# vfmatzkin/ct-unet

Measured on AMD Instinct MI355X. Metric: voxels/sec fwd+bwd, 128^3 fp32 patch, higher is better.
Workload: dtype f32; 1 GPU; UNet() default (1 in, 2 out, i_size 8, 4 blocks), 128^3 patch, batch 1 per GPU, train step = fwd + Dice/CE loss + bwd + grad all-reduce + Adam(amsgrad); patch=128, per_gpu_batch=1, parallelism=dp1, launch=hipgraph

## Files before the change

### ct-unet_amd/csrc/upconv_fused.hip

```cpp
#include <type_traits>
#include "common.h"
#include "bn_tail.h"
#include "channel_sum.h"

namespace {

typedef float v2f __attribute__((ext_vector_type(2)));

struct UpP {
    const float* in;
    const float* in_scale;
    const float* in_shift;
    const float* wp;
    const float* beff;
    float* out;
    float* stats;
    int in_cs, rin_p, in_relu, out_cs, nout_p;
    int N, D, H, W;
    int tiles_d, tiles_h, tiles_w;
    ctu_bn_tail tail;
};

template <int PB, int NTP, bool PW = false>
__global__ __launch_bounds__(256, 2) void upconv_fused_fwd_kernel(UpP p, int ntiles, int tiles_per_block) {
    static_assert(PW ? (PB == 4 && NTP == 1) : ((PB * NTP == 8 || (PB == 4 && NTP == 1)) && (PB == 8 || PB == 4 || PB == 2)), "tile-parities per block");
    constexpr int NTW = PW ? 3 : 2, TAPS = 4 * NTW;
    constexpr int MT = 4, TD = 4, TH = 4, TW = 16;
    constexpr int HD = TD + 2, HH = TH + 2, HW = TW + 2, HV = HD * HH * HW;
    constexpr int NTHR = 256;
    constexpr int NTPT = NTP;
    constexpr int WFL = PB * TAPS * NTP * 128;
    constexpr int AITEMS = HV * 2, AITER = (AITEMS + NTHR - 1) / NTHR;
    constexpr int WITER = (WFL / 4 + NTHR - 1) / NTHR;
    constexpr int VS2 = 6;
    static_assert(WFL / 4 % NTHR == 0, "weight staging covers the stage exactly");

    __shared__ __attribute__((aligned(16))) v2f sA2[HV * VS2];
    __shared__ __attribute__((aligned(16))) v2f sW2[WFL / 2];
    typedef const volatile __attribute__((address_space(3))) v2f* lds_v2f_ptr;
    __shared__ float sRed[4 * NTP * 16 * 2];

    const int tid = threadIdx.x, lane = tid & 63, wave = tid >> 6;
    const int m = lane & 15, kq = lane >> 4;
    const int by = blockIdx.y;
    const int nchunk = p.rin_p >> 3;
    const int half = tid & 1;
    const bool has_xf = p.in_scale != nullptr;
    const int pd0 = PW ? 0 : ((by * PB) >> 2) & 1, ph0 = PW ? 0 : ((by * PB) >> 1) & 1;

    lds_v2f_ptr vA = (lds_v2f_ptr)sA2 + (((wave + pd0) * HH + ph0) * HW + m) * VS2 + kq;
    lds_v2f_ptr vW = (lds_v2f_ptr)sW2 + (kq * 16 + m);

    unsigned hoff[AITER];
    constexpr int FPW = 5, NFW = (AITER + FPW - 1) / FPW;
    unsigned fw[NFW];
#pragma unroll
    for (int q = 0; q < NFW; ++q) fw[q] = 0;
#pragma unroll
    for (int it = 0; it < AITER; ++it) {
        const int i = tid + it * NTHR;
        const int v = (i < AITEMS) ? (i >> 1) : 0;
        const int pw = v % HW, t2 = v / HW, ph = t2 % HH, pd = t2 / HH;
        hoff[it] = (unsigned)(((pd * p.H + ph) * p.W + pw) * p.in_cs + half * 4) * 4u;
        const unsigned face = (pd == 0 ? 1u : 0u) | (pd == HD - 1 ? 2u : 0u) | (ph == 0 ? 4u : 0u) | (ph == HH - 1 ? 8u : 0u) |
                              (pw == 0 ? 16u : 0u) | (pw == HW - 1 ? 32u : 0u);
        fw[it / FPW] |= face << (6 * (it % FPW));
    }
    const unsigned safe_off = (unsigned)(((p.H + 1) * p.W + 1) * p.in_cs + half * 4) * 4u;

    f32x4 acc[PB][MT][NTP];
    float s1[NTP][4], s2[NTP][4];
#pragma unroll
    for (int nt = 0; nt < NTP; ++nt) {
#pragma unroll
        for (int pi = 0; pi < PB; ++pi)
#pragma unroll
            for (int mt = 0; mt < MT; ++mt) acc[pi][mt][nt] = f32x4{0.f, 0.f, 0.f, 0.f};
#pragma unroll
        for (int r = 0; r < 4; ++r) { s1[nt][r] = 0.f; s2[nt][r] = 0.f; }
    }

    int tile = blockIdx.x * tiles_per_block;
    const int tile_end = min(ntiles, tile + tiles_per_block);
    int c = 0;
    float4 va[AITER];
    typedef typename std::conditional<PW, f32x4, float4>::type wv_t;
    wv_t vw[WITER];
    float4 sc = make_float4(1.f, 1.f, 1.f, 1.f), sh = make_float4(0.f, 0.f, 0.f, 0.f);
    unsigned vmask = 0;

    struct Box { int tx, ty, tz, n; };
    Box box;
    {
        int t = tile;
        box.tx = t % p.tiles_w; t /= p.tiles_w;
        box.ty = t % p.tiles_h; t /= p.tiles_h;
        box.tz = t % p.tiles_d; box.n = t / p.tiles_d;
    }
    auto box_next = [&](Box b) {
        if (++b.tx == p.tiles_w) { b.tx = 0; if (++b.ty == p.tiles_h) { b.ty = 0; if (++b.tz == p.tiles_d) { b.tz = 0; ++b.n; } } }
        return b;
    };
    bool a_interior = false;
    auto load_a = [&](Box b, int cc) {
        const int d0 = b.tz * TD, h0 = b.ty * TH, w0 = b.tx * TW;
        if (has_xf) {
            sc = *reinterpret_cast<const float4*>(p.in_scale + cc * 8 + half * 4);
            sh = *reinterpret_cast<const float4*>(p.in_shift + cc * 8 + half * 4);
        }
        const long long org = (((long long)b.n * p.D + d0) * p.H + h0) * p.W + w0 - ((long long)p.H * p.W + p.W + 1);
        const char* base = reinterpret_cast<const char*>(p.in + org * p.in_cs + cc * 8);
        a_interior = d0 >= 1 && h0 >= 1 && w0 >= 1 && d0 + TD < p.D && h0 + TH < p.H && w0 + TW < p.W;
        if (a_interior) {
#pragma unroll
            for (int it = 0; it < AITER; ++it) {
                if ((it + 1) * NTHR <= AITEMS || tid + it * NTHR < AITEMS)
                    va[it] = *reinterpret_cast<const float4*>(base + hoff[it]);
                else
                    va[it] = make_float4(0.f, 0.f, 0.f, 0.f);
            }
            return;
        }
        vmask = 0;
        if (d0 + TD <= p.D && h0 + TH <= p.H && w0 + TW <= p.W) {
            const unsigned bface = (d0 == 0 ? 1u : 0u) | (d0 + TD == p.D ? 2u : 0u) | (h0 == 0 ? 4u : 0u) |
                                   (h0 + TH == p.H ? 8u : 0u) | (w0 == 0 ? 16u : 0u) | (w0 + TW == p.W ? 32u : 0u);
#pragma unroll
            for (int it = 0; it < AITER; ++it) {
                const bool ok = (fw[it / FPW] & (bface << (6 * (it % FPW)))) == 0u;
                va[it] = *reinterpret_cast<const float4*>(base + (ok ? hoff[it] : safe_off));
                vmask |= ok ? (1u << it) : 0u;
            }
            return;
        }
#pragma unroll
        for (int it = 0; it < AITER; ++it) {
            const int i = tid + it * NTHR, v = i >> 1;
            const int pw = v % HW, t2 = v / HW, ph = t2 % HH, pd = t2 / HH;
            const int gd = d0 + pd - 1, gh = h0 + ph - 1, gw = w0 + pw - 1;
            const bool ok = i < AITEMS && (unsigned)gd < (unsigned)p.D && (unsigned)gh < (unsigned)p.H && (unsigned)gw < (unsigned)p.W;
            float4 val = make_float4(0.f, 0.f, 0.f, 0.f);
            if (ok) {
                val = *reinterpret_cast<const float4*>(base + hoff[it]);
                vmask |= 1u << it;
            }
            va[it] = val;
        }
    };
    auto load_w = [&](int cc) {
        const char* wsrc = reinterpret_cast<const char*>(PW ? p.wp + (size_t)cc * 4 * TAPS * 128
                                                            : p.wp + ((size_t)cc * 8 + (size_t)by * PB) * 8 * NTPT * 128);
#pragma unroll
        for (int it = 0; it < WITER; ++it) vw[it] = *reinterpret_cast<const wv_t*>(wsrc + (unsigned)(tid + it * NTHR) * 16u);
    };
    if (tile >= tile_end) return;
    load_a(box, 0);
    load_w(0);

    while (true) {
        CTU_SETPRIO(CTU_PRIO_STAGE);
        __syncthreads();
        {
            auto put = [&](int it, float4 val) {
                const int i = tid + it * NTHR;
                if ((it + 1) * NTHR <= AITEMS || i < AITEMS) *reinterpret_cast<float4*>(&sA2[(i >> 1) * VS2 + half * 2]) = val;
            };
            if (a_interior) {
#pragma unroll
                for (int it = 0; it < AITER; ++it) put(it, has_xf ? xform4(va[it], sc, sh, p.in_relu) : va[it]);
            } else {
#pragma unroll
                for (int it = 0; it < AITER; ++it) {
                    const float4 t = has_xf ? xform4(va[it], sc, sh, p.in_relu) : va[it];
                    const bool ok = (vmask >> it) & 1u;
                    put(it, make_float4(ok ? t.x : 0.f, ok ? t.y : 0.f, ok ? t.z : 0.f, ok ? t.w : 0.f));
                }
            }
#pragma unroll
            for (int it = 0; it < WITER; ++it) *reinterpret_cast<wv_t*>(&sW2[(tid + it * NTHR) * 2]) = vw[it];
        }
        __syncthreads();
        int ntile = tile, nc = c + 1;
        Box nbox = box;
        if (nc == nchunk) { nc = 0; ntile = tile + 1; nbox = box_next(box); }
        const bool has_next = ntile < tile_end;
        if (has_next) {
            load_a(nbox, nc);
            load_w(nc);
        }
        CTU_SETPRIO(0);
        {
            constexpr int NG = PB * 2 * NTW;
            v2f ar[2][5], br[2][2][NTP];
            auto load_group = [&](int g, v2f (&aa)[5], v2f (&bb)[2][NTP]) {
                const int pi = g / (2 * NTW), dz = (g / NTW) & 1, dx = g % NTW;
                const int pid = PW ? (pi >> 1) : ((PB == 8) ? (pi >> 2) : 0), pih = PW ? (pi & 1) : ((PB >= 4) ? ((pi >> 1) & 1) : 0),
                          piw = PW ? 0 : (pi & 1);
#pragma unroll
                for (int r = 0; r < 5; ++r) aa[r] = vA[(((pid + dz) * HH + r + pih) * HW + piw + dx) * VS2];
#pragma unroll
                for (int dy = 0; dy < 2; ++dy)
#pragma unroll
                    for (int nt = 0; nt < NTP; ++nt) bb[dy][nt] = vW[((pi * TAPS + (dz * 2 + dy) * NTW + dx) * NTP + nt) * 64];
            };
            load_group(0, ar[0], br[0]);
            constexpr bool PIN = CTU_PIN_FWD && PB * NTP <= 4;
            if constexpr (PIN) __builtin_amdgcn_sched_barrier(0);
#pragma unroll
            for (int g = 0; g < NG; ++g) {
                if (g + 1 < NG) load_group(g + 1, ar[(g + 1) & 1], br[(g + 1) & 1]);
                const int pi = g / (2 * NTW);
                v2f (&aa)[5] = ar[g & 1];
                v2f (&bb)[2][NTP] = br[g & 1];
#pragma unroll
                for (int dy = 0; dy < 2; ++dy) {
#pragma unroll
                    for (int nt = 0; nt < NTP; ++nt)
#pragma unroll
                        for (int mt = 0; mt < MT; ++mt)
                            acc[pi][mt][nt] = __builtin_amdgcn_mfma_f32_16x16x4f32(bb[dy][nt].x, aa[mt + dy].x, acc[pi][mt][nt], 0, 0, 0);
#pragma unroll
                    for (int nt = 0; nt < NTP; ++nt)
#pragma unroll
                        for (int mt = 0; mt < MT; ++mt)
                            acc[pi][mt][nt] = __builtin_amdgcn_mfma_f32_16x16x4f32(bb[dy][nt].y, aa[mt + dy].y, acc[pi][mt][nt], 0, 0, 0);
                }
                if constexpr (PIN) {
#pragma unroll
                    for (int q = 0; q < 4 * MT * NTP; ++q) {
                        __builtin_amdgcn_sched_group_barrier(0x008, 1, 0);
                        if (g + 1 < NG && q < 5 + 2 * NTP) __builtin_amdgcn_sched_group_barrier(0x100, 1, 0);
                    }
                }
            }
        }
        CTU_SETPRIO(CTU_PRIO_STAGE);
        if (c == nchunk - 1) {
            const int d0 = box.tz * TD, h0 = box.ty * TH, w0 = box.tx * TW;
            const int Df = 2 * p.D, Hf = 2 * p.H, Wf = 2 * p.W;
            const int cd = d0 + wave, cw = w0 + m;
            const bool touches = d0 == 0 || h0 == 0 || w0 == 0 || d0 + TD >= p.D || h0 + TH >= p.H || w0 + TW >= p.W;
#pragma unroll
            for (int nt = 0; nt < NTP; ++nt) {
                const int co = PW ? (kq & 1) * 4 : nt * 16 + kq * 4;
                const bool cok = co < p.nout_p;
                float4 b0 = make_float4(0.f, 0.f, 0.f, 0.f);
                if (cok) b0 = *reinterpret_cast<const float4*>(p.beff + co);
#pragma unroll
                for (int pi = 0; pi < PB; ++pi) {
                    const int pd = PW ? (pi >> 1) : pd0 + ((PB == 8) ? (pi >> 2) : 0), ph = PW ? (pi & 1) : ph0 + ((PB >= 4) ? ((pi >> 1) & 1) : 0),
                              pw = PW ? (kq >> 1) : (pi & 1);
                    const int fz = 2 * cd + pd, fx = 2 * cw + pw;
#pragma unroll
                    for (int mt = 0; mt < MT; ++mt) {
                        const int ch = h0 + mt, fy = 2 * ch + ph;
                        if (cok && cd < p.D && ch < p.H && cw < p.W) {
                            float4 bv = b0;
                            if (touches) {
                                const int cz = fz == 0 ? 1 : (fz == Df - 1 ? 2 : 0), cy = fy == 0 ? 1 : (fy == Hf - 1 ? 2 : 0),
                                          cx = fx == 0 ? 1 : (fx == Wf - 1 ? 2 : 0);
                                bv = *reinterpret_cast<const float4*>(p.beff + (size_t)((cz * 3 + cy) * 3 + cx) * p.nout_p + co);
                            }
                            float4 o;
                            o.x = acc[pi][mt][nt][0] + bv.x; o.y = acc[pi][mt][nt][1] + bv.y;
                            o.z = acc[pi][mt][nt][2] + bv.z; o.w = acc[pi][mt][nt][3] + bv.w;
                            const size_t fv = (((size_t)box.n * Df + fz) * Hf + fy) * Wf + fx;
                            *reinterpret_cast<float4*>(p.out + fv * p.out_cs + co) = o;
                            s1[nt][0] += o.x; s1[nt][1] += o.y; s1[nt][2] += o.z; s1[nt][3] += o.w;
                            s2[nt][0] += o.x * o.x; s2[nt][1] += o.y * o.y; s2[nt][2] += o.z * o.z; s2[nt][3] += o.w * o.w;
                        }
                        acc[pi][mt][nt] = f32x4{0.f, 0.f, 0.f, 0.f};
                    }
                }
            }
        }
        if (!has_next) break;
        tile = ntile; c = nc; box = nbox;
    }
    if (p.stats) {
        __syncthreads();
#pragma unroll
        for (int nt = 0; nt < NTP; ++nt)
#pragma unroll
            for (int r = 0; r < 4; ++r) {
                float a1 = s1[nt][r], a2 = s2[nt][r];
#pragma unroll
                for (int o = 1; o < 16; o <<= 1) { a1 += __shfl_xor(a1, o); a2 += __shfl_xor(a2, o); }
                if (PW) { a1 += __shfl_xor(a1, 32); a2 += __shfl_xor(a2, 32); }
                const int ch = PW ? (kq & 1) * 4 + r : nt * 16 + kq * 4 + r;
                if (m == 0 && (!PW || kq < 2)) {
                    sRed[(wave * NTP * 16 + ch) * 2 + 0] = a1;
                    sRed[(wave * NTP * 16 + ch) * 2 + 1] = a2;
                }
            }
        __syncthreads();
        float* row = p.stats + ((size_t)blockIdx.y * gridDim.x + blockIdx.x) * 2 * p.nout_p;
        for (int ch = tid; ch < p.nout_p; ch += NTHR) {
            float a1 = 0.f, a2 = 0.f;
#pragma unroll
            for (int w = 0; w < 4; ++w) {
                a1 += sRed[(w * NTP * 16 + ch) * 2 + 0];
                a2 += sRed[(w * NTP * 16 + ch) * 2 + 1];
            }
            st_row(p.tail.counter != nullptr, row + ch, a1);
            st_row(p.tail.counter != nullptr, row + p.nout_p + ch, a2);
        }
        if (p.tail.counter) bn_fwd_tail(p.tail, p.stats, gridDim.x * gridDim.y, p.nout_p, gridDim.x * gridDim.y);
    }
}

struct UpDP {
    const float* g;
    const float* wp;
    float* out;
    int g_cs, nout_p, out_cs, cin_p;
    int N, D, H, W;
    int tiles_d, tiles_h, tiles_w, n16;
};

template <int NT>
__global__ __launch_bounds__(256, 2) void upconv_fused_bwd_data_kernel(UpDP p, int ntiles, int tiles_per_block) {
    constexpr int MT = 4, TD = 4, TH = 4, TW = 16;
    constexpr int HD = TD + 2, HH = TH + 2, HW = TW + 2, HV = HD * HH * HW;
    constexpr int NTHR = 256;
    constexpr int WFL = 8 * NT * 128;
    constexpr int AITEMS = HV * 2, AITER = (AITEMS + NTHR - 1) / NTHR;
    constexpr int WITER = (WFL / 4 + NTHR - 1) / NTHR;
    constexpr int VS2 = 6;
    static_assert(WFL / 4 % NTHR == 0, "weight staging covers the stage exactly");

    __shared__ __attribute__((aligned(16))) v2f sA2[HV * VS2];
    __shared__ __attribute__((aligned(16))) v2f sW2[WFL / 2];
    typedef const volatile __attribute__((address_space(3))) v2f* lds_v2f_ptr;

    const int tid = threadIdx.x, lane = tid & 63, wave = tid >> 6;
    const int m = lane & 15, kq = lane >> 4;
    const int by = blockIdx.y;
    const int qc = p.nout_p >> 3;
    const int nchunk = 8 * qc;
    const int half = tid & 1;
    const int Hf = 2 * p.H, Wf = 2 * p.W;

    lds_v2f_ptr vA0 = (lds_v2f_ptr)sA2 + ((wave * HH) * HW + m) * VS2 + kq;
    lds_v2f_ptr vW = (lds_v2f_ptr)sW2 + (kq * 16 + m);

    unsigned hoff[AITER];
    constexpr int FPW = 5, NFW = (AITER + FPW - 1) / FPW;
    unsigned fw[NFW];
#pragma unroll
    for (int q = 0; q < NFW; ++q) fw[q] = 0;
#pragma unroll
    for (int it = 0; it < AITER; ++it) {
        const int i = tid + it * NTHR;
        const int v = (i < AITEMS) ? (i >> 1) : 0;
        const int pw = v % HW, t2 = v / HW, ph = t2 % HH, pd = t2 / HH;
        hoff[it] = (unsigned)(((2 * pd * Hf + 2 * ph) * Wf + 2 * pw) * p.g_cs + half * 4) * 4u;
        const unsigned face = (pd == 0 ? 1u : 0u) | (pd == HD - 1 ? 2u : 0u) | (ph == 0 ? 4u : 0u) | (ph == HH - 1 ? 8u : 0u) |
                              (pw == 0 ? 16u : 0u) | (pw == HW - 1 ? 32u : 0u);
        fw[it / FPW] |= face << (6 * (it % FPW));
    }
    const unsigned safe_off = (unsigned)(((2 * Hf + 2) * Wf + 2) * p.g_cs + half * 4) * 4u;

    f32x4 acc[MT][NT];
#pragma unroll
    for (int nt = 0; nt < NT; ++nt)
#pragma unroll
        for (int mt = 0; mt < MT; ++mt) acc[mt][nt] = f32x4{0.f, 0.f, 0.f, 0.f};

    int tile = blockIdx.x * tiles_per_block;
    const int tile_end = min(ntiles, tile + tiles_per_block);
    if (tile >= tile_end) return;
    int c = 0;
    float4 va[AITER], vw[WITER];
    unsigned vmask = 0;

    struct Box { int tx, ty, tz, n; };
    Box box;
    {
        int t = tile;
        box.tx = t % p.tiles_w; t /= p.tiles_w;
        box.ty = t % p.tiles_h; t /= p.tiles_h;
        box.tz = t % p.tiles_d; box.n = t / p.tiles_d;
    }
    auto box_next = [&](Box b) {
        if (++b.tx == p.tiles_w) { b.tx = 0; if (++b.ty == p.tiles_h) { b.ty = 0; if (++b.tz == p.tiles_d) { b.tz = 0; ++b.n; } } }
        return b;
    };
    bool a_interior = false;
    auto load_a = [&](Box b, int cc) {
        const int d0 = b.tz * TD, h0 = b.ty * TH, w0 = b.tx * TW;
        const int par = cc / qc, q = cc % qc;
        const int pz = (par >> 2) & 1, py = (par >> 1) & 1, px = par & 1;
        const long long org = (((long long)b.n * 2 * p.D + 2 * (d0 - 1) + pz) * Hf + 2 * (h0 - 1) + py) * Wf + 2 * (w0 - 1) + px;
        const char* base = reinterpret_cast<const char*>(p.g + org * p.g_cs + q * 8);
        a_interior = d0 >= 1 && h0 >= 1 && w0 >= 1 && d0 + TD < p.D && h0 + TH < p.H && w0 + TW < p.W;
        if (a_interior) {
#pragma unroll
            for (int it = 0; it < AITER; ++it) {
                if ((it + 1) * NTHR <= AITEMS || tid + it * NTHR < AITEMS)
                    va[it] = *reinterpret_cast<const float4*>(base + hoff[it]);
                else
                    va[it] = make_float4(0.f, 0.f, 0.f, 0.f);
            }
            return;
        }
        vmask = 0;
        if (d0 + TD <= p.D && h0 + TH <= p.H && w0 + TW <= p.W) {
            const unsigned bface = (d0 == 0 ? 1u : 0u) | (d0 + TD == p.D ? 2u : 0u) | (h0 == 0 ? 4u : 0u) |
                                   (h0 + TH == p.H ? 8u : 0u) | (w0 == 0 ? 16u : 0u) | (w0 + TW == p.W ? 32u : 0u);
#pragma unroll
            for (int it = 0; it < AITER; ++it) {
                const bool ok = (fw[it / FPW] & (bface << (6 * (it % FPW)))) == 0u;
                va[it] = *reinterpret_cast<const float4*>(base + (ok ? hoff[it] : safe_off));
                vmask |= ok ? (1u << it) : 0u;
            }
            return;
        }
#pragma unroll
        for (int it = 0; it < AITER; ++it) {
            const int i = tid + it * NTHR, v = i >> 1;
            const int pw = v % HW, t2 = v / HW, ph = t2 % HH, pd = t2 / HH;
            const int gd = d0 + pd - 1, gh = h0 + ph - 1, gw = w0 + pw - 1;
            const bool ok = i < AITEMS && (unsigned)gd < (unsigned)p.D && (unsigned)gh < (unsigned)p.H && (unsigned)gw < (unsigned)p.W;
            float4 val = make_float4(0.f, 0.f, 0.f, 0.f);
            if (ok) {
                val = *reinterpret_cast<const float4*>(base + hoff[it]);
                vmask |= 1u << it;
            }
            va[it] = val;
        }
    };
    const bool w_full = (by + 1) * NT <= p.n16;
    auto load_w = [&](int cc) {
        const float* wsrc = p.wp + ((size_t)cc * 8 * p.n16 + (size_t)by * NT) * 128;
#pragma unroll
        for (int it = 0; it < WITER; ++it) {
            const int i = (tid + it * NTHR) * 4;
            const int ts = i / (NT * 128), r = i % (NT * 128);
            float4 v = make_float4(0.f, 0.f, 0.f, 0.f);
            if (w_full || by * NT * 128 + r < p.n16 * 128)
                v = *reinterpret_cast<const float4*>(reinterpret_cast<const char*>(wsrc) + (unsigned)(ts * p.n16 * 128 + r) * 4u);
            vw[it] = v;
        }
    };
    load_a(box, 0);
    load_w(0);

    while (true) {
        CTU_SETPRIO(CTU_PRIO_STAGE);
        __syncthreads();
        {
            auto put = [&](int it, float4 val) {
                const int i = tid + it * NTHR;
                if ((it + 1) * NTHR <= AITEMS || i < AITEMS) *reinterpret_cast<float4*>(&sA2[(i >> 1) * VS2 + half * 2]) = val;
            };
            if (a_interior) {
#pragma unroll
                for (int it = 0; it < AITER; ++it) put(it, va[it]);
            } else {
#pragma unroll
                for (int it = 0; it < AITER; ++it) {
                    const bool ok = (vmask >> it) & 1u;
                    put(it, make_float4(ok ? va[it].x : 0.f, ok ? va[it].y : 0.f, ok ? va[it].z : 0.f, ok ? va[it].w : 0.f));
                }
            }
#pragma unroll
            for (int it = 0; it < WITER; ++it) *reinterpret_cast<float4*>(&sW2[(tid + it * NTHR) * 2]) = vw[it];
        }
        __syncthreads();
        const int par = c / qc;
        lds_v2f_ptr vA = vA0 + (((1 - ((par >> 2) & 1)) * HH + (1 - ((par >> 1) & 1))) * HW + (1 - (par & 1))) * VS2;
        int ntile = tile, nc = c + 1;
        Box nbox = box;
        if (nc == nchunk) { nc = 0; ntile = tile + 1; nbox = box_next(box); }
        const bool has_next = ntile < tile_end;
        if (has_next) {
            load_a(nbox, nc);
            load_w(nc);
        }
        CTU_SETPRIO(0);
        {
            v2f ar[2][5], br[2][2][NT];
            auto load_group = [&](int g, v2f (&aa)[5], v2f (&bb)[2][NT]) {
                const int ez = (g >> 1) & 1, ex = g & 1;
#pragma unroll
                for (int r = 0; r < 5; ++r) aa[r] = vA[((ez * HH + r) * HW + ex) * VS2];
#pragma unroll
                for (int ey = 0; ey < 2; ++ey)
#pragma unroll
                    for (int nt = 0; nt < NT; ++nt) bb[ey][nt] = vW[(((ez * 2 + ey) * 2 + ex) * NT + nt) * 64];
            };
            load_group(0, ar[0], br[0]);
#if CTU_PIN_FWD
            __builtin_amdgcn_sched_barrier(0);
#endif
#pragma unroll
            for (int g = 0; g < 4; ++g) {
                if (g + 1 < 4) load_group(g + 1, ar[(g + 1) & 1], br[(g + 1) & 1]);
                v2f (&aa)[5] = ar[g & 1];
                v2f (&bb)[2][NT] = br[g & 1];
#pragma unroll
                for (int ey = 0; ey < 2; ++ey) {
#pragma unroll
                    for (int nt = 0; nt < NT; ++nt)
#pragma unroll
                        for (int mt = 0; mt < MT; ++mt)
                            acc[mt][nt] = __builtin_amdgcn_mfma_f32_16x16x4f32(bb[ey][nt].x, aa[mt + ey].x, acc[mt][nt], 0, 0, 0);
#pragma unroll
                    for (int nt = 0; nt < NT; ++nt)
#pragma unroll
                        for (int mt = 0; mt < MT; ++mt)
                            acc[mt][nt] = __builtin_amdgcn_mfma_f32_16x16x4f32(bb[ey][nt].y, aa[mt + ey].y, acc[mt][nt], 0, 0, 0);
                }
#if CTU_PIN_FWD
#pragma unroll
                for (int q = 0; q < 4 * MT * NT; ++q) {
                    __builtin_amdgcn_sched_group_barrier(0x008, 1, 0);
                    if (g + 1 < 4 && q < 5 + 2 * NT) __builtin_amdgcn_sched_group_barrier(0x100, 1, 0);
                }
#endif
            }
        }
        CTU_SETPRIO(CTU_PRIO_STAGE);
        if (c == nchunk - 1) {
            const int d0 = box.tz * TD, h0 = box.ty * TH, w0 = box.tx * TW;
            const int gw = w0 + m;
            float* obase = p.out + ((((size_t)box.n * p.D + d0 + wave) * p.H + h0) * p.W + gw) * p.out_cs;
            const int orow = p.W * p.out_cs;
#pragma unroll
            for (int nt = 0; nt < NT; ++nt) {
                const int co = (by * NT + nt) * 16 + kq * 4;
#pragma unroll
                for (int mt = 0; mt < MT; ++mt) {
                    if (co < p.cin_p && d0 + wave < p.D && h0 + mt < p.H && gw < p.W) {
                        float4 o;
                        o.x = acc[mt][nt][0]; o.y = acc[mt][nt][1]; o.z = acc[mt][nt][2]; o.w = acc[mt][nt][3];
                        *reinterpret_cast<float4*>(obase + mt * orow + co) = o;
                    }
                    acc[mt][nt] = f32x4{0.f, 0.f, 0.f, 0.f};
                }
            }
        }
        if (!has_next) break;
        tile = ntile; c = nc; box = nbox;
    }
}

__device__ __forceinline__ float upconv_pack_bwd_value(const float* __restrict__ wp, int idx, int cin_p, int nout_p) {
    const int n16 = (cin_p + 15) >> 4, qc = nout_p >> 3, ntpt = (nout_p + 15) >> 4;
    int r = idx;
    const int j = r & 1; r >>= 1;
    const int n = r & 15; r >>= 4;
    const int kq = r & 3; r >>= 2;
    const int nt = r % n16; r /= n16;
    const int e = r & 7; r >>= 3;
    const int q = r % qc;
    const int par = r / qc;
    const int pos = nt * 16 + n, co = q * 8 + kq * 2 + j;
    float v = 0.f;
    if (pos < cin_p) {
        const int cf = pos >> 3, kqf = (pos & 7) >> 1, jf = pos & 1;
        v = wp[((((size_t)cf * 8 + par) * 8 + (e ^ 7)) * ntpt + (co >> 4)) * 128 + kqf * 32 + (co & 15) * 2 + jf];
    }
    return v;
}

__device__ __forceinline__ int axis_pairs(int pbit, int jbit, int (&t)[2], int (&a)[2]) {
    if (pbit == 0) {
        if (jbit == 0) { t[0] = 0; a[0] = 1; return 1; }
        t[0] = 1; a[0] = 0; t[1] = 2; a[1] = 1; return 2;
    }
    if (jbit == 0) { t[0] = 0; a[0] = 0; t[1] = 1; a[1] = 1; return 2; }
    t[0] = 2; a[0] = 0; return 1;
}

__global__ void upconv_transpose_kernel(const float* __restrict__ wt, const float* __restrict__ w3, float* __restrict__ wtt,
                                        float* __restrict__ w3t, int C, int Co, int nout_p) {
    const int idx = blockIdx.x * blockDim.x + threadIdx.x;
    const int n3 = 27 * C * nout_p, nt = 8 * C * C;
    if (idx < n3) {
        const int co = idx % nout_p, cm = (idx / nout_p) % C, t = idx / (nout_p * C);
        w3t[idx] = co < Co ? w3[((size_t)co * C + cm) * 27 + t] : 0.f;
    } else if (idx < n3 + nt) {
        const int k = idx - n3;
        const int cm = k % C, ci = (k / C) % C, a = k / (C * C);
        wtt[k] = wt[((size_t)ci * C + cm) * 8 + a];
    }
}

constexpr int WS_WAVES = 8, WS_BLOCK = WS_WAVES * 64;
__device__ __forceinline__ void upconv_pack_block(const float* __restrict__ wtt, const float* __restrict__ w3t, float* __restrict__ wp,
                                                  int C, int nout_p, const int32_t* __restrict__ cinv, int nchunk, int ntpt,
                                                  int bid, float4 (*part)[64]) {
    const int pr = threadIdx.x >> 6, lane = threadIdx.x & 63, sub = lane & 7;
    const int idx = bid * 8 + (lane >> 3);
    const int ncol4 = ntpt * 4;
    const bool valid = idx < nchunk * 8 * 8 * 8 * ncol4;
    int r = valid ? idx : 0;
    const int co = (r % ncol4) * 4; r /= ncol4;
    const int r8 = r & 7; r >>= 3;
    const int tap = r & 7; r >>= 3;
    const int par = r & 7; r >>= 3;
    const int c = r;
    const int rp = c * 8 + r8;
    const int ci = cinv ? cinv[rp] : (rp < C ? rp : -1);
    int np = 0;
    float4 s = make_float4(0.f, 0.f, 0.f, 0.f);
    if (valid && ci >= 0 && co < nout_p) {
        int tz[2], az[2], ty[2], ay[2], tx[2], ax[2];
        const int nz = axis_pairs((par >> 2) & 1, (tap >> 2) & 1, tz, az);
        const int ny = axis_pairs((par >> 1) & 1, (tap >> 1) & 1, ty, ay);
        const int nx = axis_pairs(par & 1, tap & 1, tx, ax);
        np = nz * ny * nx;
        const int ix = pr % nx, iy = (pr / nx) % ny, iz = pr / (nx * ny);
        if (iz < nz) {
            const float* a = wtt + ((size_t)((az[iz] * 2 + ay[iy]) * 2 + ax[ix]) * C + ci) * C;
            const float* b = w3t + (size_t)((tz[iz] * 3 + ty[iy]) * 3 + tx[ix]) * C * nout_p + co;
#pragma unroll 4
            for (int cm = sub; cm < C; cm += 8) {
                const float av = a[cm];
                const float4 bv = *reinterpret_cast<const float4*>(b + (size_t)cm * nout_p);
                s.x = fmaf(av, bv.x, s.x); s.y = fmaf(av, bv.y, s.y); s.z = fmaf(av, bv.z, s.z); s.w = fmaf(av, bv.w, s.w);
            }
        }
    }
    part[pr][lane] = s;
    __syncthreads();
    if (pr != 0) return;
    float4 v = make_float4(0.f, 0.f, 0.f, 0.f);
    for (int p = 0; p < np; ++p) {
        const float4 t = part[p][lane];
        v.x += t.x; v.y += t.y; v.z += t.z; v.w += t.w;
    }
    float vv[4] = {v.x, v.y, v.z, v.w};
#pragma unroll
    for (int q = 0; q < 4; ++q) { vv[q] += __shfl_xor(vv[q], 1); vv[q] += __shfl_xor(vv[q], 2); vv[q] += __shfl_xor(vv[q], 4); }
    if (valid && sub == 0) {
        const int nt = co >> 4, n = co & 15, kq = r8 >> 1, j = r8 & 1;
        float* dst = wp + ((((size_t)c * 8 + par) * 8 + tap) * ntpt + nt) * 128 + kq * 32 + n * 2 + j;
#pragma unroll
        for (int q = 0; q < 4; ++q) dst[q * 2] = vv[q];
    }
}

__device__ __forceinline__ float upconv_pack_pw_value(const float* __restrict__ wp, int idx) {
    int r = idx;
    const int j = r & 1; r >>= 1;
    const int n = r & 15; r >>= 4;
    const int kq = r & 3; r >>= 2;
    const int tap = r % 12; r /= 12;
    const int par4 = r & 3;
    const int c = r >> 2;
    const int px = n >> 3, co = n & 7, dxx = tap % 3, dzy = tap / 3, jx = dxx - px;
    float v = 0.f;
    if (jx == 0 || jx == 1) v = wp[((size_t)(c * 8 + par4 * 2 + px) * 8 + dzy * 2 + jx) * 128 + kq * 32 + co * 2 + j];
    return v;
}

__global__ void upconv_pack_gather_kernel(const float* __restrict__ wp, float* __restrict__ wpw, int npw, float* __restrict__ wpd,
                                          int nwpd, int cin_p, int nout_p) {
    const int idx = blockIdx.x * blockDim.x + threadIdx.x;
    if (idx < npw) wpw[idx] = upconv_pack_pw_value(wp, idx);
    else if (idx - npw < nwpd) wpd[idx - npw] = upconv_pack_bwd_value(wp, idx - npw, cin_p, nout_p);
}

constexpr int BEFF_CO = 8;
__device__ __forceinline__ void upconv_beff_block(const float* __restrict__ bt, const float* __restrict__ w3t, float* __restrict__ beff,
                                                  int C, int nout_p, int co0, float* S) {
    for (int i = threadIdx.x; i < 27 * BEFF_CO; i += blockDim.x) {
        const int co = co0 + i % BEFF_CO, t = i / BEFF_CO;
        const float* b = w3t + (size_t)t * C * nout_p + co;
        float s = 0.f;
#pragma unroll 16
        for (int cm = 0; cm < C; ++cm) s = fmaf(bt[cm], b[(size_t)cm * nout_p], s);
        S[i] = s;
    }
    __syncthreads();
    for (int i = threadIdx.x; i < 27 * BEFF_CO; i += blockDim.x) {
        const int col = i % BEFF_CO, cls = i / BEFF_CO;
        const int cz = cls / 9, cy = (cls / 3) % 3, cx = cls % 3;
        float v = 0.f;
        for (int t = 0; t < 27; ++t) {
            const int tz = t / 9, ty = (t / 3) % 3, tx = t % 3;
            if ((cz == 1 && tz == 0) || (cz == 2 && tz == 2) || (cy == 1 && ty == 0) || (cy == 2 && ty == 2) ||
                (cx == 1 && tx == 0) || (cx == 2 && tx == 2))
                continue;
            v += S[t * BEFF_CO + col];
        }
        beff[cls * nout_p + co0 + col] = v;
    }
}

__global__ __launch_bounds__(WS_BLOCK) void upconv_pack_beff_kernel(const float* __restrict__ wtt, const float* __restrict__ w3t,
                                                                    float* __restrict__ wp, int C, int nout_p,
                                                                    const int32_t* __restrict__ cinv, int nchunk, int ntpt,
                                                                    const float* __restrict__ bt, float* __restrict__ beff) {
    __shared__ float4 part[WS_WAVES][64];
    static_assert(27 * BEFF_CO <= WS_WAVES * 64 * 4, "b_eff's S fits the pack's LDS");
    const int nbeff = nout_p / BEFF_CO;
    if ((int)blockIdx.x < nbeff) {
        upconv_beff_block(bt, w3t, beff, C, nout_p, (int)blockIdx.x * BEFF_CO, reinterpret_cast<float*>(part));
        return;
    }
    upconv_pack_block(wtt, w3t, wp, C, nout_p, cinv, nchunk, ntpt, (int)blockIdx.x - nbeff, part);
}

constexpr int FS_SPLIT = 16;

template <class T>
__device__ __forceinline__ void upconv_face_sums_block(const T* __restrict__ dy, int cs, int cp, int N, int Df, int Hf, int Wf,
                                                       float* __restrict__ tpart, int sel, int split, float4* red) {
    const int sz = sel / 9, sy = (sel / 3) % 3, sx = sel % 3;
    const int nz = sz ? 1 : Df, ny = sy ? 1 : Hf, nx = sx ? 1 : Wf;
    const int z0 = sz == 2 ? Df - 1 : 0, y0 = sy == 2 ? Hf - 1 : 0, x0 = sx == 2 ? Wf - 1 : 0;
    const int nq = cp >> 2;
    const int qd = threadIdx.x % nq;
    const int64_t nvox = (int64_t)N * nz * ny * nx;
    float4 acc = make_float4(0.f, 0.f, 0.f, 0.f);
    for (int64_t v = (int64_t)split * (256 / nq) + threadIdx.x / nq; v < nvox; v += (int64_t)FS_SPLIT * (256 / nq)) {
        int64_t r = v;
        const int x = x0 + (int)(r % nx); r /= nx;
        const int y = y0 + (int)(r % ny); r /= ny;
        const int z = z0 + (int)(r % nz);
        const int n = (int)(r / nz);
        const float4 g = ld4<T>(dy + ((((size_t)n * Df + z) * Hf + y) * Wf + x) * cs + qd * 4);
        acc.x += g.x; acc.y += g.y; acc.z += g.z; acc.w += g.w;
    }
    red[threadIdx.x] = acc;
    __syncthreads();
    for (int o = 128; o >= nq; o >>= 1) {
        if (threadIdx.x < o) {
            float4 b = red[threadIdx.x + o];
            float4& a = red[threadIdx.x];
            a.x += b.x; a.y += b.y; a.z += b.z; a.w += b.w;
        }
        __syncthreads();
    }
    if (threadIdx.x < nq)
        *reinterpret_cast<float4*>(tpart + ((size_t)sel * FS_SPLIT + split) * cp + threadIdx.x * 4) = red[threadIdx.x];
}

template <class T>
__global__ __launch_bounds__(256) void upconv_sums_kernel(const T* __restrict__ dy, int cs, int cp, int N, int Df, int Hf, int Wf,
                                                          int64_t fvox, float* __restrict__ csp, int nb, float* __restrict__ tpart) {
    static_assert(CSUM_BLOCK == 256, "one block size for both ranges");
    __shared__ float4 red[256];
    if ((int)blockIdx.x < nb) {
        channel_sum_partial_block<T>(dy, cs, cp, fvox, csp, blockIdx.x, nb, reinterpret_cast<float*>(red));
        return;
    }
    const int b = (int)blockIdx.x - nb;
    upconv_face_sums_block<T>(dy, cs, cp, N, Df, Hf, Wf, tpart, b / FS_SPLIT + 1, b % FS_SPLIT, red);
}

__global__ __launch_bounds__(256) void upconv_tall_v_kernel(const float* __restrict__ csp, int nb, const float* __restrict__ tpart,
                                                            int cp, float* __restrict__ tall, float* __restrict__ V) {
    __shared__ double r[CSUM_BLOCK];
    const int co = blockIdx.x;
    const float ta = channel_sum_final_block(csp, nb, cp, co, r);
    if (threadIdx.x == 0) tall[co] = ta;
    if (threadIdx.x >= 27) return;
    const int t = threadIdx.x, idx = t * cp + co;
    const int tz = t / 9, ty = (t / 3) % 3, tx = t % 3;
    float v = 0.f;
    for (int iz = 0; iz < (tz == 1 ? 1 : 2); ++iz)
        for (int iy = 0; iy < (ty == 1 ? 1 : 2); ++iy)
            for (int ix = 0; ix < (tx == 1 ? 1 : 2); ++ix) {
                const int sz = iz == 0 ? 0 : (tz == 0 ? 1 : 2), sy = iy == 0 ? 0 : (ty == 0 ? 1 : 2), sx = ix == 0 ? 0 : (tx == 0 ? 1 : 2);
                const float sign = ((iz + iy + ix) & 1) ? -1.f : 1.f;
                const int sel = (sz * 3 + sy) * 3 + sx;
                float s = 0.f;
                if (sel == 0) {
                    s = ta;
                } else {
                    const float* src = tpart + (size_t)sel * FS_SPLIT * cp + co;
                    for (int b = 0; b < FS_SPLIT; ++b) s += src[(size_t)b * cp];
                }
                v += sign * s;
            }
    V[idx] = v;
}

__device__ __forceinline__ void axis_pd(int t, int a, int& pbit, int& jbit) {
    if (a == 1) { pbit = (t == 1) ? 1 : 0; jbit = (t == 2) ? 1 : 0; }
    else { pbit = (t == 1) ? 0 : 1; jbit = (t == 0) ? 0 : 1; }
}
__device__ __forceinline__ int weff_index(int t, int a) {
    int pz, jz, py, jy, px, jx;
    axis_pd(t / 9, (a >> 2) & 1, pz, jz);
    axis_pd((t / 3) % 3, (a >> 1) & 1, py, jy);
    axis_pd(t % 3, a & 1, px, jx);
    return ((pz * 4 + py * 2 + px) * 8) + (jz * 4 + jy * 2 + jx);
}

__global__ __launch_bounds__(WS_BLOCK) void upconv_project_kernel(const float* __restrict__ dweff, const float* __restrict__ V,
                                                                  const float* __restrict__ wtt, const float* __restrict__ w3t,
                                                                  const float* __restrict__ bt, const int32_t* __restrict__ imap,
                                                                  int C, int Co, int cin_p, int nout_p, int nb1,
                                                                  float* __restrict__ dwt, float* __restrict__ dw3,
                                                                  float* __restrict__ dbt) {
    const int coq = (Co + 3) >> 2;
    const int n1 = C * C * 8, n2 = coq * C * 27, n3 = C;
    if ((int)blockIdx.x >= nb1) {
        __shared__ float4 part[WS_WAVES][64];
        const int a = threadIdx.x >> 6, lane = threadIdx.x & 63, sub = lane & 7;
        const int k = ((int)blockIdx.x - nb1) * 8 + (lane >> 3);
        const bool valid = k < n2;
        const int kk = valid ? k : 0;
        const int co = (kk % coq) * 4, cm = (kk / coq) % C, t = kk / (coq * C);
        float4 s = make_float4(0.f, 0.f, 0.f, 0.f);
        if (valid) {
            const float* g = dweff + (size_t)weff_index(t, a) * cin_p * nout_p + co;
            const float* w = wtt + (size_t)a * C * C + cm;
#pragma unroll 4
            for (int ci = sub; ci < C; ci += 8) {
                const float4 gv = *reinterpret_cast<const float4*>(g + (size_t)(imap ? imap[ci] : ci) * nout_p);
                const float wv = w[(size_t)ci * C];
                s.x = fmaf(gv.x, wv, s.x); s.y = fmaf(gv.y, wv, s.y); s.z = fmaf(gv.z, wv, s.z); s.w = fmaf(gv.w, wv, s.w);
            }
        }
        part[a][lane] = s;
        __syncthreads();
        if (a != 0) return;
        float4 acc = make_float4(0.f, 0.f, 0.f, 0.f);
#pragma unroll
        for (int aa = 0; aa < 8; ++aa) {
            const float4 p = part[aa][lane];
            acc.x += p.x; acc.y += p.y; acc.z += p.z; acc.w += p.w;
        }
        float av[4] = {acc.x, acc.y, acc.z, acc.w};
#pragma unroll
        for (int q = 0; q < 4; ++q) {
            if (sub == 0 && co + q < Co) av[q] = fmaf(V[t * nout_p + co + q], bt[cm], av[q]);
            av[q] += __shfl_xor(av[q], 1); av[q] += __shfl_xor(av[q], 2); av[q] += __shfl_xor(av[q], 4);
            if (valid && sub == 0 && co + q < Co) dw3[((size_t)(co + q) * C + cm) * 27 + t] = av[q];
        }
        return;
    }
    const int gidx = blockIdx.x * blockDim.x + threadIdx.x;
    const int sub = gidx & 7;
    const int idx = gidx >> 3;
    if (idx >= n1 + n3) return;
    float v = 0.f;
    float* dst;
    if (idx < n1) {
        const int a = idx & 7, cm = (idx >> 3) % C, ci = idx / (8 * C);
        const int pos = imap ? imap[ci] : ci;
#pragma unroll
        for (int k = 0; k < 4; ++k) {
            const int t = sub + 8 * k;
            if (t < 27) {
                const float4* g = reinterpret_cast<const float4*>(dweff + ((size_t)weff_index(t, a) * cin_p + pos) * nout_p);
                const float4* w = reinterpret_cast<const float4*>(w3t + ((size_t)t * C + cm) * nout_p);
                float s = 0.f;
                for (int c4 = 0; c4 * 4 < Co; ++c4) {
                    const float4 gv = g[c4], wv = w[c4];
                    const int co = c4 * 4;
                    s = fmaf(gv.x, wv.x, s);
                    if (co + 1 < Co) s = fmaf(gv.y, wv.y, s);
                    if (co + 2 < Co) s = fmaf(gv.z, wv.z, s);
                    if (co + 3 < Co) s = fmaf(gv.w, wv.w, s);
                }
                v += s;
            }
        }
        dst = dwt + idx;
    } else {
        const int cm = idx - n1;
        for (int t = sub; t < 27; t += 8) {
            const float* w = w3t + ((size_t)t * C + cm) * nout_p;
#pragma unroll 8
            for (int co = 0; co < Co; ++co) v = fmaf(V[t * nout_p + co], w[co], v);
        }
        dst = dbt + cm;
    }
    v += __shfl_xor(v, 1); v += __shfl_xor(v, 2); v += __shfl_xor(v, 4);
    if (sub == 0) *dst = v;
}

struct UpPlan { int tiles_d, tiles_h, tiles_w, ntiles, nt, ny; Grid grid; };
static UpPlan up_plan(int N, int D, int H, int W, int nout_p, int bwd_n16) {
    UpPlan r;
    r.tiles_d = ceil_div(D, 4); r.tiles_h = ceil_div(H, 4); r.tiles_w = ceil_div(W, 16);
    r.ntiles = N * r.tiles_d * r.tiles_h * r.tiles_w;
    if (bwd_n16) {
        r.nt = bwd_n16 >= 4 ? 4 : (bwd_n16 >= 2 ? 2 : 1);
        while (r.nt > 1 && (long)r.ntiles * ceil_div(bwd_n16, r.nt) < 256) r.nt >>= 1;
        r.ny = ceil_div(bwd_n16, r.nt);
    } else {
        r.nt = 0;
        r.ny = (nout_p == 16 && r.ntiles < 256) ? 2 : (nout_p <= 16 ? 1 : (nout_p <= 32 ? 2 : 4));
    }
    r.grid = persist_grid(r.ntiles, 512 / r.ny);
    return r;
}

}

extern "C" int ctu_upconv_fused_supported(int k, int D, int H, int W, int cin_p, int nout_p) {
    return k == 3 && W >= 16 && D >= 1 && H >= 1 && cin_p % 8 == 0 && cin_p >= 8 && nout_p % 8 == 0 && nout_p >= 8 && nout_p <= 64;
}

static size_t up_std_packed(int cin_p, int nout_p) { return (size_t)(cin_p / 8) * 8 * 8 * ceil_div(nout_p, 16) * 128; }

extern "C" size_t ctu_upconv_fused_packed_floats(int cin_p, int nout_p) {
    return up_std_packed(cin_p, nout_p) + (nout_p == 8 ? (size_t)(cin_p / 8) * 4 * 12 * 128 : 0);
}

extern "C" int ctu_upconv_fused_num_blocks(int N, int D, int H, int W, int nout_p) {
    const UpPlan r = up_plan(N, D, H, W, nout_p, 0);
    return r.grid.gx * r.ny;
}

extern "C" size_t ctu_upconv_fused_pack_ws_floats(int C, int nout_p) { return (size_t)27 * C * nout_p + (size_t)8 * C * C; }

static int upconv_pack_gather(const float* wp, int cin_p, int nout_p, float* wpw, float* wpd, hipStream_t st) {
    const int npw = wpw ? (cin_p / 8) * 4 * 12 * 128 : 0;
    const int nwpd = wpd ? (int)ctu_upconv_fused_bwd_packed_floats(cin_p, nout_p) : 0;
    if (npw + nwpd == 0) return CTU_OK;
    upconv_pack_gather_kernel<<<ceil_div(npw + nwpd, 256), 256, 0, st>>>(wp, wpw, npw, wpd, nwpd, cin_p, nout_p);
    CTU_CHECK_LAUNCH("upconv_fused_pack_gather");
    return CTU_OK;
}

extern "C" int ctu_upconv_fused_pack_all(const float* wt, const float* bt, const float* w3, int C, int Co, const int32_t* cinv,
                                         int cin_p, int nout_p, float* wp, float* beff, float* ws, float* wpd, void* stream) {
    CTU_REQUIRE(wt && bt && w3 && wp && beff && ws, "upconv_fused_pack: null pointer");
    CTU_REQUIRE(C > 0 && Co > 0 && Co <= nout_p && cin_p % 8 == 0 && nout_p % 8 == 0 && (cinv || C <= cin_p),
                "upconv_fused_pack: C=%d Co=%d cin_p=%d nout_p=%d", C, Co, cin_p, nout_p);
    hipStream_t st = (hipStream_t)stream;
    const int ntpt = ceil_div(nout_p, 16);
    CTU_REQUIRE(((uintptr_t)ws & 15) == 0, "upconv_fused_pack: ws must be 16-byte aligned");
    float* w3t = ws;
    float* wtt = ws + (size_t)27 * C * nout_p;
    const int ntr = 27 * C * nout_p + 8 * C * C;
    upconv_transpose_kernel<<<ceil_div(ntr, 256), 256, 0, st>>>(wt, w3, wtt, w3t, C, Co, nout_p);
    CTU_CHECK_LAUNCH("upconv_fused_transpose");
    const int quads = (cin_p / 8) * 8 * 8 * 8 * ntpt * 4;
    upconv_pack_beff_kernel<<<nout_p / BEFF_CO + ceil_div(quads, 8), WS_BLOCK, 0, st>>>(wtt, w3t, wp, C, nout_p, cinv, cin_p / 8,
                                                                                         ntpt, bt, beff);
    CTU_CHECK_LAUNCH("upconv_fused_pack");
    return upconv_pack_gather(wp, cin_p, nout_p, nout_p == 8 ? wp + up_std_packed(cin_p, nout_p) : nullptr, wpd, st);
}

extern "C" int ctu_upconv_fused_pack(const float* wt, const float* bt, const float* w3, int C, int Co, const int32_t* cinv,
                                     int cin_p, int nout_p, float* wp, float* beff, float* ws, void* stream) {
    return ctu_upconv_fused_pack_all(wt, bt, w3, C, Co, cinv, cin_p, nout_p, wp, beff, ws, nullptr, stream);
}

extern "C" int ctu_upconv_fused_fwd(const float* in, int in_cs, int cin_p, const float* in_scale, const float* in_shift,
                                    int in_relu, const float* wp, const float* beff, float* out, int out_cs, int nout_p,
                                    float* stats, int N, int D, int H, int W, const ctu_bn_tail* tail, void* stream) {
    CTU_REQUIRE(in && wp && beff && out, "upconv_fused_fwd: null pointer");
    CTU_REQUIRE(ctu_upconv_fused_supported(3, D, H, W, cin_p, nout_p), "upconv_fused_fwd: unsupported geometry (W=%d cin_p=%d nout_p=%d)",
                W, cin_p, nout_p);
    CTU_REQUIRE(in_cs >= cin_p && in_cs % 4 == 0 && out_cs >= nout_p && out_cs % 4 == 0, "upconv_fused_fwd: bad stride");
    CTU_REQUIRE((in_scale == nullptr) == (in_shift == nullptr), "upconv_fused_fwd: scale/shift must come together");
    CTU_REQUIRE(((uintptr_t)in & 15) == 0 && ((uintptr_t)out & 15) == 0 && ((uintptr_t)wp & 15) == 0 && ((uintptr_t)beff & 15) == 0,
                "upconv_fused_fwd: 16-byte alignment");
    CTU_REQUIRE((int64_t)N * D * H * W * 8 < (int64_t)1 << 31 && (int64_t)(2 * H * W + 2 * W + 2) * in_cs * 4 < (int64_t)1 << 31,
                "upconv_fused_fwd: volume too large for 32-bit offsets");
    UpP p;
    p.in = in; p.in_scale = in_scale; p.in_shift = in_shift; p.wp = wp; p.beff = beff; p.out = out; p.stats = stats;
    CTU_REQUIRE(!tail || (stats && tail->counter && tail->gamma && tail->beta && tail->scale && tail->shift && tail->mean &&
                          tail->invstd && tail->C > 0 && tail->C <= nout_p && tail->count > 0),
                "upconv_fused_fwd: incomplete BatchNorm tail");
    p.tail = tail_or_off(tail);
    p.in_cs = in_cs; p.rin_p = cin_p; p.in_relu = in_relu; p.out_cs = out_cs; p.nout_p = nout_p;
    p.N = N; p.D = D; p.H = H; p.W = W;
    const UpPlan r = up_plan(N, D, H, W, nout_p, 0);
    p.tiles_d = r.tiles_d; p.tiles_h = r.tiles_h; p.tiles_w = r.tiles_w;
    const int ny = r.ny, gx = r.grid.gx, tpb = r.grid.tpb, ntiles = r.ntiles;
    hipStream_t st = (hipStream_t)stream;
    if (nout_p == 16 && ny == 2) {
        upconv_fused_fwd_kernel<4, 1><<<dim3(gx, 2), 256, 0, st>>>(p, ntiles, tpb);
    } else if (nout_p == 8) {
        p.wp = wp + up_std_packed(cin_p, nout_p);
        upconv_fused_fwd_kernel<4, 1, true><<<dim3(gx, 1), 256, 0, st>>>(p, ntiles, tpb);
    } else if (ny == 1) upconv_fused_fwd_kernel<8, 1><<<dim3(gx, 1), 256, 0, st>>>(p, ntiles, tpb);
    else if (ny == 2) upconv_fused_fwd_kernel<4, 2><<<dim3(gx, 2), 256, 0, st>>>(p, ntiles, tpb);
    else upconv_fused_fwd_kernel<2, 4><<<dim3(gx, 4), 256, 0, st>>>(p, ntiles, tpb);
    CTU_CHECK_LAUNCH("upconv_fused_fwd");
    return CTU_OK;
}

extern "C" int ctu_channel_sum_num_blocks(int64_t nvox);

extern "C" size_t ctu_upconv_fused_project_ws_floats(int nout_p, int64_t fine_nvox) {
    return (size_t)27 * FS_SPLIT * nout_p + (size_t)27 * nout_p + nout_p + (size_t)ctu_channel_sum_num_blocks(fine_nvox) * nout_p;
}

static int upconv_project_impl(int dtype, const float* dweff, const void* gout, int g_cs, int nout_p, int N, int D, int H, int W,
                               const float* bt, const float* pack_ws, const int32_t* imap, int C, int Co, int cin_p,
                               float* dwt, float* dbt, float* dw3, float* ws, void* stream) {
    CTU_REQUIRE(dweff && gout && bt && pack_ws && dwt && dbt && dw3 && ws, "upconv_fused_project: null pointer");
    CTU_REQUIRE(nout_p == 8 || nout_p == 16 || nout_p == 32 || nout_p == 64, "upconv_fused_project: nout_p=%d", nout_p);
    CTU_REQUIRE(C > 0 && Co > 0 && Co <= nout_p && g_cs >= nout_p && g_cs % 4 == 0, "upconv_fused_project: bad channels");
    CTU_REQUIRE(((uintptr_t)dweff & 15) == 0 && ((uintptr_t)pack_ws & 15) == 0, "upconv_fused_project: dweff / pack_ws must be 16-byte aligned");
    hipStream_t st = (hipStream_t)stream;
    float* tpart = ws;
    float* V = ws + (size_t)27 * FS_SPLIT * nout_p;
    float* tall = V + (size_t)27 * nout_p;
    float* csp = tall + nout_p;
    const int64_t fvox = (int64_t)N * 8 * D * H * W;
    const int nb = ctu_channel_sum_num_blocks(fvox);
    const int nsum = nb + 26 * FS_SPLIT;
    if (dtype == 0) {
        upconv_sums_kernel<float><<<nsum, 256, 0, st>>>((const float*)gout, g_cs, nout_p, N, 2 * D, 2 * H, 2 * W, fvox, csp, nb, tpart);
    } else {
        CTU_DISPATCH_LP(dtype, upconv_sums_kernel<T><<<nsum, 256, 0, st>>>((const T*)gout, g_cs, nout_p, N, 2 * D, 2 * H, 2 * W, fvox, csp, nb, tpart));
    }
    CTU_CHECK_LAUNCH("upconv_sums");
    upconv_tall_v_kernel<<<nout_p, 256, 0, st>>>(csp, nb, tpart, nout_p, tall, V);
    CTU_CHECK_LAUNCH("upconv_tall_v");
    const float* w3t = pack_ws;
    const float* wtt = pack_ws + (size_t)27 * C * nout_p;
    const int nb1 = ceil_div((C * C * 8 + C) * 8, WS_BLOCK);
    const int nb2 = ceil_div(((Co + 3) / 4) * C * 27, 8);
    upconv_project_kernel<<<nb1 + nb2, WS_BLOCK, 0, st>>>(dweff, V, wtt, w3t, bt, imap, C, Co, cin_p, nout_p, nb1, dwt, dw3, dbt);
    CTU_CHECK_LAUNCH("upconv_project");
    return CTU_OK;
}

extern "C" int ctu_upconv_fused_project(const float* dweff, const float* gout, int g_cs, int nout_p, int N, int D, int H, int W,
                                        const float* bt, const float* pack_ws, const int32_t* imap, int C, int Co, int cin_p,
                                        float* dwt, float* dbt, float* dw3, float* ws, void* stream) {
    return upconv_project_impl(0, dweff, gout, g_cs, nout_p, N, D, H, W, bt, pack_ws, imap, C, Co, cin_p, dwt, dbt, dw3, ws, stream);
}
extern "C" int ctu_lp_upconv_fused_project(int dtype, const float* dweff, const void* gout, int g_cs, int nout_p, int N, int D, int H,
                                           int W, const float* bt, const float* pack_ws, const int32_t* imap, int C, int Co, int cin_p,
                                           float* dwt, float* dbt, float* dw3, float* ws, void* stream) {
    CTU_REQUIRE(dtype == CTU_BF16 || dtype == CTU_F16, "lp_upconv_fused_project: dtype %d", dtype);
    return upconv_project_impl(dtype, dweff, gout, g_cs, nout_p, N, D, H, W, bt, pack_ws, imap, C, Co, cin_p, dwt, dbt, dw3, ws, stream);
}

extern "C" size_t ctu_upconv_fused_bwd_packed_floats(int cin_p, int nout_p) {
    return (size_t)8 * (nout_p / 8) * 8 * ceil_div(cin_p, 16) * 128;
}

extern "C" int ctu_upconv_fused_pack_bwd(const float* wp, int cin_p, int nout_p, float* wpd, void* stream) {
    CTU_REQUIRE(wp && wpd && cin_p % 8 == 0 && nout_p % 8 == 0, "upconv_fused_pack_bwd: bad argument");
    return upconv_pack_gather(wp, cin_p, nout_p, nullptr, wpd, (hipStream_t)stream);
}

extern "C" int ctu_upconv_fused_bwd_data(const float* gout, int g_cs, int nout_p, const float* wpd, float* gin, int gin_cs,
                                         int cin_p, int N, int D, int H, int W, void* stream) {
    CTU_REQUIRE(gout && wpd && gin, "upconv_fused_bwd_data: null pointer");
    CTU_REQUIRE(ctu_upconv_fused_supported(3, D, H, W, cin_p, nout_p), "upconv_fused_bwd_data: unsupported geometry");
    CTU_REQUIRE(g_cs >= nout_p && g_cs % 4 == 0 && gin_cs >= cin_p && gin_cs % 4 == 0, "upconv_fused_bwd_data: bad stride");
    CTU_REQUIRE(((uintptr_t)gout & 15) == 0 && ((uintptr_t)gin & 15) == 0 && ((uintptr_t)wpd & 15) == 0, "upconv_fused_bwd_data: alignment");
    CTU_REQUIRE((int64_t)(12 * 2 * H + 12) * 2 * W * g_cs * 4 + 64 < (int64_t)1 << 31, "upconv_fused_bwd_data: volume too large for 32-bit offsets");
    UpDP p;
    p.g = gout; p.wp = wpd; p.out = gin; p.g_cs = g_cs; p.nout_p = nout_p; p.out_cs = gin_cs; p.cin_p = cin_p;
    p.N = N; p.D = D; p.H = H; p.W = W;
    p.n16 = ceil_div(cin_p, 16);
    const UpPlan r = up_plan(N, D, H, W, nout_p, p.n16);
    p.tiles_d = r.tiles_d; p.tiles_h = r.tiles_h; p.tiles_w = r.tiles_w;
    const int NT = r.nt, ny = r.ny, gx = r.grid.gx, tpb = r.grid.tpb, ntiles = r.ntiles;
    hipStream_t st = (hipStream_t)stream;
    if (NT == 4) upconv_fused_bwd_data_kernel<4><<<dim3(gx, ny), 256, 0, st>>>(p, ntiles, tpb);
    else if (NT == 2) upconv_fused_bwd_data_kernel<2><<<dim3(gx, ny), 256, 0, st>>>(p, ntiles, tpb);
    else upconv_fused_bwd_data_kernel<1><<<dim3(gx, ny), 256, 0, st>>>(p, ntiles, tpb);
    CTU_CHECK_LAUNCH("upconv_fused_bwd_data");
    return CTU_OK;
}
```

### ct-unet_amd/ctunet_amd/_lib.py

```python
from __future__ import annotations

import ctypes as C
import os

import torch

_HERE = os.path.dirname(os.path.abspath(__file__))
LIB_PATH = os.environ.get("CTUNET_HIP_LIB") or os.path.join(_HERE, "libctunet_hip.so")

P = C.c_void_p
I = C.c_int
L = C.c_int64
F = C.c_float
D = C.c_double
Z = C.c_size_t
U = C.c_uint64

class PackJob(C.Structure):
    _fields_ = [("w", C.c_void_p), ("wp", C.c_void_p), ("cinv", C.c_void_p), ("kind", C.c_int), ("Co", C.c_int),
                ("Ci", C.c_int), ("k", C.c_int), ("rin_p", C.c_int), ("nout_p", C.c_int), ("mode", C.c_int),
                ("layout", C.c_int)]


class BnTail(C.Structure):
    _fields_ = [("gamma", C.c_void_p), ("beta", C.c_void_p), ("running_mean", C.c_void_p), ("running_var", C.c_void_p),
                ("scale", C.c_void_p), ("shift", C.c_void_p), ("mean", C.c_void_p), ("invstd", C.c_void_p),
                ("num_batches_tracked", C.c_void_p), ("counter", C.c_void_p), ("count", C.c_double),
                ("momentum", C.c_float), ("eps", C.c_float), ("C", C.c_int), ("n_updates", C.c_int)]


class BnBwdTail(C.Structure):
    _fields_ = [("gamma", C.c_void_p), ("invstd", C.c_void_p), ("dgamma", C.c_void_p), ("dbeta", C.c_void_p),
                ("coef", C.c_void_p), ("mean", C.c_void_p), ("running_mean", C.c_void_p), ("running_var", C.c_void_p),
                ("num_batches_tracked", C.c_void_p), ("counter", C.c_void_p), ("count", C.c_double),
                ("momentum", C.c_float), ("eps", C.c_float), ("C", C.c_int)]


class WgradJob(C.Structure):
    _fields_ = [("ws", C.c_void_p), ("dw", C.c_void_p), ("db", C.c_void_p), ("cinv", C.c_void_p), ("kind", C.c_int),
                ("Co", C.c_int), ("Ci", C.c_int), ("cin_p", C.c_int), ("n_ci_g", C.c_int), ("gx", C.c_int),
                ("pairs", C.c_int), ("nmf", C.c_int)]


WGRAD_JOBS_MAX = 4

SIGNATURES = {
    "ctu_last_error": (C.c_char_p, []),
    "ctu_abi_version": (I, []),
    "ctu_arch": (C.c_char_p, []),
    "ctu_ncdhw_to_ndhwc": (I, [P, P, I, I, I, I, I, I, I, P]),
    "ctu_ndhwc_to_ncdhw": (I, [P, P, I, I, I, I, I, I, P]),
    "ctu_conv3d_layout": (I, [I, I, I]),
    "ctu_conv3d_fwd_kernel_name": (C.c_char_p, [I, I, I, I, I, I, I]),
    "ctu_conv3d_wgrad_kernel_name": (C.c_char_p, [I, I, I, I]),
    "ctu_conv3d_packed_floats": (Z, [I, I, I, I]),
    "ctu_conv3d_num_blocks": (I, [I, I, I, I, I, I, I]),
    "ctu_pack_conv3d_weight": (I, [P, P, I, I, I, P, I, I, I, I, P]),
    "ctu_pack_batch": (I, [P, I, P]),
    "ctu_conv3d_fwd": (I, [P, I, I, P, P, I, P, P, I, P, I, I, P, I, I, I, I, I, I, P, P]),
    "ctu_conv3d_wgrad_ws_floats": (Z, [I, I, I, I, I, I, I]),
    "ctu_conv3d_wgrad": (I, [P, I, I, P, P, I, P, I, I, P, P, I, I, P, P, I, I, I, I, I, P]),
    "ctu_conv3d_wgrad_bn_supported": (I, [I, I, I, I, I, I, I]),
    "ctu_conv3d_wgrad_bn": (I, [P, I, I, P, P, I, P, I, I, P, P, P, P, P, P, I, I, P, P, I, I, I, I, I, P]),
    "ctu_conv3d_first_supported": (I, [I, I, I, I]),
    "ctu_conv3d_first_num_blocks": (I, [I, I, I, I]),
    "ctu_conv3d_first_fwd": (I, [P, I, P, P, I, P, I, I, P, I, I, I, I, P, P]),
    "ctu_conv3d_first_bwd_data": (I, [P, I, P, I, I, P, I, I, I, I, P]),
    "ctu_conv3d_first_wgrad_ws_floats": (Z, [I, I, I, I, I]),
    "ctu_conv3d_first_wgrad": (I, [P, I, P, I, P, I, P, I, I, I, I, P]),
    "ctu_conv3d_first_wgrad_bn": (I, [P, I, P, I, P, P, P, P, P, P, I, P, I, I, I, I, P]),
    "ctu_bn_finalize": (I, [P, I, I, I, D, P, P, P, P, F, F, I, P, P, P, P, P, P]),
    "ctu_bn_eval_affine": (I, [P, P, P, P, F, I, I, P, P, P]),
    "ctu_bn_bwd_num_blocks": (I, [L]),
    "ctu_bn_relu_bwd_reduce": (I, [P, I, P, I, I, P, P, P, P, L, P, P, P]),
    "ctu_bn_bwd_finalize": (I, [P, I, I, I, D, P, P, P, P, P, P, P, P, F, F, P, P]),
    "ctu_bn_relu_bwd_apply": (I, [P, I, P, I, I, P, P, P, P, P, L, P]),
    "ctu_conv3d_wgrad_slabs": (I, [P, I, I, P, P, I, P, I, I, P, P, I, I, P, P, I, I, I, I, I, P, P]),
    "ctu_conv3d_wgrad_bn_slabs": (I, [P, I, I, P, P, I, P, I, I, P, P, P, P, P, P, I, I, P, P, I, I, I, I, I, P, P]),
    "ctu_conv3d_first_wgrad_slabs": (I, [P, I, P, I, P, I, P, I, I, I, I, P, P]),
    "ctu_conv3d_first_wgrad_bn_slabs": (I, [P, I, P, I, P, P, P, P, P, P, I, P, I, I, I, I, P, P]),
    "ctu_convt2_wgrad_slabs": (I, [P, I, I, P, P, I, P, I, I, P, P, I, I, P, P, I, I, I, I, P, P]),
    "ctu_bn_bwd_finalize_jobs": (I, [P, I, I, I, D, P, P, P, P, P, P, P, P, F, F, P, P, I, P]),
    "ctu_wgrad_reduce_jobs": (I, [P, I, P]),
    "ctu_maxpool2_fwd": (I, [P, I, I, P, P, I, P, I, I, I, I, I, P]),
    "ctu_maxpool2_bwd": (I, [P, I, I, P, P, I, P, I, P, I, I, I, I, I, I, P]),
    "ctu_maxpool2_bwd_bn_num_blocks": (I, [I, I, I, I, I]),
    "ctu_maxpool2_bwd_bn": (I, [P, I, I, P, P, P, P, P, I, P, I, I, I, I, I, I, P, P, P]),
    "ctu_convt_packed_floats": (Z, [I, I]),
    "ctu_pack_convt_weight": (I, [P, P, I, I, P, I, I, I, P]),
    "ctu_convt2_fwd": (I, [P, I, I, P, P, I, P, P, I, P, I, I, I, I, I, I, P]),
    "ctu_convt2_bwd_data": (I, [P, I, I, P, P, I, I, I, I, I, I, P]),
    "ctu_convt2_wgrad_ws_floats": (Z, [I, I, I, I, I, I]),
    "ctu_convt2_wgrad": (I, [P, I, I, P, P, I, P, I, I, P, P, I, I, P, P, I, I, I, I, P]),
    "ctu_convt2_plan": (C.c_char_p, [I, I, I, I, I, I, I, P]),
    "ctu_convt2_wgrad_plan": (C.c_char_p, [I, I, I, I, I, I, P]),
    "ctu_head_fwd": (I, [P, I, I, P, P, I, P, P, P, I, I, I, I, P, P, I, L, P]),
    "ctu_head_bwd_ws_floats": (Z, [I, L, I, I]),
    "ctu_head_bwd": (I, [P, I, I, P, P, I, P, P, P, I, I, I, I, P, P, P, I, P, P, P, I, L, P]),
    "ctu_head_bwd_num_blocks": (I, [I, L]),
    "ctu_head_bwd_bn": (I, [P, I, I, P, P, I, P, P, P, I, I, I, I, P, P, P, I, P, P, P, I, L, P, P, I, P, P, P]),
    "ctu_loss_ws_floats": (Z, [I, L]),
    "ctu_loss_fwd": (I, [P, P, I, L, F, F, I, P, P, P]),
    "ctu_loss_bwd": (I, [P, P, I, L, F, F, I, P, P, P, P, I, P]),
    "ctu_skip_add": (I, [P, I, P, P, I, P, I, P, P, I, P, I, I, L, P]),
    "ctu_upconv_fused_supported": (I, [I, I, I, I, I, I]),
    "ctu_upconv_fused_packed_floats": (Z, [I, I]),
    "ctu_upconv_fused_num_blocks": (I, [I, I, I, I, I]),
    "ctu_upconv_fused_pack_ws_floats": (Z, [I, I]),
    "ctu_upconv_fused_pack": (I, [P, P, P, I, I, P, I, I, P, P, P, P]),
    "ctu_upconv_fused_pack_all": (I, [P, P, P, I, I, P, I, I, P, P, P, P, P]),
    "ctu_upconv_fused_fwd": (I, [P, I, I, P, P, I, P, P, P, I, I, P, I, I, I, I, P, P]),
    "ctu_upconv_fused_wgrad_ws_floats": (Z, [I, I, I, I, I, I]),
    "ctu_upconv_fused_wgrad": (I, [P, I, I, P, P, I, P, I, I, P, P, I, I, I, I, P]),
    "ctu_upconv_fused_wgrad_bn_supported": (I, [I, I, I, I, I, I]),
    "ctu_upconv_fused_wgrad_bn": (I, [P, I, I, P, P, I, P, I, I, P, P, P, P, P, P, P, I, I, I, I, P]),
    "ctu_upconv_fused_project_ws_floats": (Z, [I, L]),
    "ctu_upconv_fused_project": (I, [P, P, I, I, I, I, I, I, P, P, P, I, I, I, P, P, P, P, P]),
    "ctu_upconv_fused_bwd_packed_floats": (Z, [I, I]),
    "ctu_upconv_fused_pack_bwd": (I, [P, I, I, P, P]),
    "ctu_upconv_fused_bwd_data": (I, [P, I, I, P, P, I, I, I, I, I, I, P]),
    "ctu_hard_segm": (I, [P, I, I, L, P, P]),
    "ctu_one_hot": (I, [P, I, I, L, P, P]),
    "ctu_hard_dice_ws_doubles": (Z, [I]),
    "ctu_hard_dice_counts": (I, [P, P, I, I, L, P, P, P]),
    "ctu_hausdorff_ws_bytes": (Z, [I, I, I, I, I]),
    "ctu_hausdorff": (I, [P, P, I, I, I, I, I, P, P, P]),
    "ctu_surface_ws_bytes": (Z, [I, I, I, I, I]),
    "ctu_surface_metrics": (I, [P, I, I, P, I, I, I, I, I, I, I, I, I, P, P, D, P, P, P]),
    "ctu_components_ws_bytes": (Z, [I, I, I, I]),
    "ctu_label_components": (I, [P, I, I, I, I, I, I, P, I, P, P, P, P]),
    "ctu_filter_components": (I, [P, I, I, I, I, I, I, P, I, I, I, P, P, P]),
    "ctu_morphology_ws_bytes": (Z, [I, I, I, I, I]),
    "ctu_binary_morphology": (I, [P, I, I, I, I, I, I, C.c_uint32, I, I, I, L, P, P, P]),
    "ctu_fill_holes": (I, [P, I, I, I, I, I, I, I, L, P, P, P]),
    "ctu_implant_mask": (I, [P, I, P, I, I, I, I, I, C.c_uint32, I, I, I, I, P, P, P]),
    "ctu_distance_ws_bytes": (Z, [I, I, I, I, I, I]),
    "ctu_distance_transform": (I, [P, I, I, I, I, I, I, L, I, I, P, I, P, P, F, P, P]),
    "ctu_resample": (I, [P, I, I, I, L, I, I, I, I, I, I, P, P, P, P, P]),
    "ctu_affine_resample": (I, [P, I, I, I, L, I, I, I, I, I, I, P, P, P, P, P, D, P, P]),
    "ctu_registration_ws_bytes": (Z, [L]),
    "ctu_registration_init": (I, [P, L, P, P, P]),
    "ctu_registration_accumulate": (I, [P, L, P, I, I, I, P, P, D, P, P]),
    "ctu_registration_update": (I, [L, I, P, P, P, I, P, P]),
    "ctu_mesh_ws_bytes": (Z, [I, I, I]),
    "ctu_mesh_count": (I, [P, I, I, I, I, I, L, F, P, P]),
    "ctu_mesh_emit": (I, [P, I, I, I, I, F, F, P, P, L, L, P, P, P, P]),
    "ctu_mesh_measure": (I, [P, L, P, L, P, P, P, P]),
    "ctu_mesh_adjacency_ws_bytes": (Z, [L, L]),
    "ctu_mesh_adjacency_build": (I, [P, L, L, P, P, P]),
    "ctu_mesh_adjacency_emit": (I, [L, L, L, P, P, P, P]),
    "ctu_mesh_smooth_ws_bytes": (Z, [L]),
    "ctu_mesh_smooth": (I, [P, L, P, P, L, P, I, F, I, F, P, P, P]),
    "ctu_mesh_voxelize_ws_bytes": (Z, [I, I, I]),
    "ctu_mesh_voxelize": (I, [P, L, P, L, I, I, I, P, P, I, P, P, P]),
    "ctu_mesh_grid_ws_bytes": (Z, [L, L]),
    "ctu_mesh_grid_build": (I, [P, L, P, L, F, L, P, P, P]),
    "ctu_mesh_grid_emit": (I, [P, L, L, L, L, P, P, P, P]),
    "ctu_mesh_distance": (I, [P, L, P, P, L, P, I, I, I, P, L, I, I, I, P, P, F, F, P, P, P, P]),
    "ctu_mesh_decimate_ws_bytes": (Z, [L, L, L]),
    "ctu_mesh_decimate_bounds": (I, [P, L, P, L, P, P]),
    "ctu_mesh_decimate_build": (I, [P, L, P, L, P, P, P, L, I, P, P]),
    "ctu_mesh_decimate_emit": (I, [P, L, L, L, L, P, P, P, P, P, P, P]),
    "ctu_gaussian_ws_bytes": (Z, [L, I, I, I, I]),
    "ctu_gaussian_filter": (I, [P, I, L, I, I, I, P, P, I, F, P, P, P]),
    "ctu_minmax_ws_bytes": (Z, [L]),
    "ctu_finite_minmax": (I, [P, I, L, P, P, P]),
    "ctu_histogram": (I, [P, I, L, I, P, D, D, P, P]),
    "ctu_threshold_otsu": (I, [P, I, P, D, D, P, P, P]),
    "ctu_binarize": (I, [P, I, L, P, D, P, D, P, P]),
    "ctu_extract_patches": (I, [P, P, I, I, I, I, I, I, I, I, P, P]),
    "ctu_stitch_patches": (I, [P, P, I, I, I, I, I, I, I, I, P, P]),
    "ctu_window_accumulate": (I, [P, P, P, P, I, I, I, I, I, I, I, I, P, P, P, F, I, I, I, P, P, P]),
    "ctu_window_finalize": (I, [P, P, I, L, P, P, P]),
    "ctu_flap_count": (I, [P, I, I, L, P, P]),
    "ctu_flap_draw": (I, [P, I, I, I, I, I, P, I, P, U, F, I, I, I, P, P, U, F, F, I, P, P]),
    "ctu_flap_apply": (I, [P, I, P, I, I, I, I, P, I, P, P, P, U, I, P, I, P, P, P]),
    "ctu_spatial_draw": (I, [I, I, I, I, P, P, U, I, D, D, D, P, I, I, I, I, P, P, P]),
    "ctu_spatial_warp": (I, [P, I, I, I, I, I, I, P, I, I, I, P, P, P, P, P]),
    "ctu_lp_upconv_fused_supported": (I, [I, I, I, I, I, I]),
    "ctu_lp_upconv_fused_packed_elems": (Z, [I]),
    "ctu_lp_upconv_fused_num_blocks": (I, [I, I, I, I]),
    "ctu_lp_upconv_fused_pack": (I, [I, P, I, P, P]),
    "ctu_lp_upconv_fused_fwd": (I, [I, P, I, I, P, P, I, P, P, P, I, P, I, I, I, I, P]),
    "ctu_lp_upconv_fused_wgrad_ws_floats": (Z, [I, I, I, I, I]),
    "ctu_lp_upconv_fused_wgrad": (I, [I, P, I, I, P, P, I, P, I, P, P, I, I, I, I, P]),
    "ctu_lp_upconv_fused_wgrad_bn_supported": (I, [I, I, I, I, I]),
    "ctu_lp_upconv_fused_wgrad_bn": (I, [I, P, I, I, P, P, I, P, I, P, P, P, P, P, P, P, I, I, I, I, P]),
    "ctu_lp_conv3d_wgrad_bn_supported": (I, [I, I, I, I, I, I, I]),
    "ctu_lp_conv3d_wgrad_bn": (I, [I, P, I, I, P, P, I, P, I, I, P, P, P, P, P, P, I, I, P, P, I, I, I, I, I, P]),
    "ctu_lp_upconv_fused_project": (I, [I, P, P, I, I, I, I, I, I, P, P, P, I, I, I, P, P, P, P, P]),
    "ctu_lp_upconv_fused_bwd_data": (I, [I, P, I, P, P, I, I, I, I, I, I, P]),
    "ctu_lp_conv3d_layout": (I, [I, I, I, I]),
    "ctu_lp_conv3d_packed_elems": (Z, [I, I, I]),
    "ctu_lp_conv3d_num_blocks": (I, [I, I, I, I, I, I, I, I]),
    "ctu_lp_pack_conv3d_weight": (I, [I, P, P, I, I, I, P, I, I, I, I, P]),
    "ctu_lp_pack_batch": (I, [I, P, I, P]),
    "ctu_lp_conv3d_fwd": (I, [I, P, I, I, P, P, I, P, P, I, P, I, I, P, I, I, I, I, I, I, P, P]),
    "ctu_lp_conv3d_wgrad_ws_floats": (Z, [I, I, I, I, I, I, I]),
    "ctu_lp_conv3d_wgrad": (I, [I, P, I, I, P, P, I, P, I, I, P, I, I, P, P, I, I, I, I, I, P]),
    "ctu_lp_conv3d_first_fwd": (I, [I, P, I, P, P, I, P, I, I, P, I, I, I, I, P, P]),
    "ctu_lp_conv3d_first_bwd_data": (I, [I, P, I, P, I, I, P, I, I, I, I, P]),
    "ctu_lp_conv3d_first_bwd_data_pair_supported": (I, [I, I]),
    "ctu_lp_conv3d_fwd_kernel_name": (C.c_char_p, [I, I, I, I, I, I, I, I]),
    "ctu_lp_conv3d_wgrad_kernel_name": (C.c_char_p, [I, I, I, I, I, I]),
    "ctu_lp_conv3d_first_bwd_data_pair": (I, [I, P, I, P, I, P, I, I, I, I, P]),
    "ctu_lp_conv3d_first_wgrad": (I, [I, P, I, P, I, P, I, P, I, I, I, I, P]),
    "ctu_lp_convt_packed_elems": (Z, [I, I, I]),
    "ctu_lp_pack_convt_weight": (I, [I, P, P, I, I, P, I, I, I, P]),
    "ctu_lp_convt2_fwd": (I, [I, P, I, I, P, P, I, P, P, I, P, I, I, I, I, I, I, P]),
    "ctu_lp_convt2_bwd_data": (I, [I, P, I, I, P, P, I, I, I, I, I, I, P]),
    "ctu_lp_convt2_wgrad_ws_floats": (Z, [I, I, I, I, I, I]),
    "ctu_lp_convt2_wgrad": (I, [I, P, I, I, P, P, I, P, I, I, P, I, I, P, P, I, I, I, I, P]),
    "ctu_lp_convt2_plan": (C.c_char_p, [I, I, I, I, I, I, I, P]),
    "ctu_lp_convt2_wgrad_plan": (C.c_char_p, [I, I, I, I, I, I, P]),
    "ctu_lp_ncdhw_to_ndhwc": (I, [I, P, P, I, I, I, I, I, I, I, P]),
    "ctu_lp_ndhwc_to_ncdhw": (I, [I, P, P, I, I, I, I, I, I, P]),
    "ctu_lp_bn_relu_bwd_reduce": (I, [I, P, I, P, I, I, P, P, P, P, L, P, P, P]),
    "ctu_lp_bn_relu_bwd_apply": (I, [I, P, I, P, I, I, P, P, P, P, P, L, P]),
    "ctu_lp_maxpool2_fwd": (I, [I, P, I, I, P, P, I, P, I, I, I, I, I, P]),
    "ctu_lp_maxpool2_bwd": (I, [I, P, I, I, P, P, I, P, I, P, I, I, I, I, I, I, P]),
    "ctu_lp_maxpool2_bwd_bn": (I, [I, P, I, I, P, P, P, P, P, I, P, I, I, I, I, I, I, P, P, P]),
    "ctu_lp_skip_add": (I, [I, P, I, P, P, I, P, I, P, P, I, P, I, I, L, P]),
    "ctu_lp_channel_sum": (I, [I, P, I, I, L, P, P, I, P]),
    "ctu_lp_head_fwd": (I, [I, P, I, I, P, P, I, P, P, P, I, I, I, I, P, P, I, L, P]),
    "ctu_lp_head_bwd_bn": (I, [I, P, I, I, P, P, I, P, P, P, I, I, I, I, P, P, P, I, P, P, P, I, L, P, P, I, P, P, F, P]),
    "ctu_lp_head_bwd_bn_dscale": (I, [I, P, I, I, P, P, I, P, P, P, I, I, I, I, P, P, P, I, P, P, P, I, L, P, P, I, P, P, P, P]),
    "ctu_scale_tensors": (I, [P, P, I, F, P, P]),
    "ctu_unscale_tensors": (I, [P, P, I, P, P, P]),
    "ctu_loss_scale_update": (I, [P, P, P, P, F, F, I, P]),
    "ctu_comm_available": (I, []),
    "ctu_comm_unique_id": (I, [P]),
    "ctu_comm_init": (I, [C.POINTER(C.c_void_p), I, I, P]),
    "ctu_comm_allreduce_f32": (I, [P, P, P, Z, I, P]),
    "ctu_comm_destroy": (I, [P]),
    "ctu_channel_sum_num_blocks": (I, [L]),
    "ctu_channel_sum": (I, [P, I, I, L, P, P, I, P]),
    "ctu_adam_amsgrad": (I, [P, P, I, P, D, D, D, D, D, I, P, P]),
    "ctu_adam_amsgrad_dev": (I, [P, P, I, P, P, D, D, D, D, I, P, P, P]),
    "ctu_grad_norm_num_blocks": (I, [P, I]),
    "ctu_grad_clip_coef": (I, [P, P, I, F, P, P, P, P]),
    "ctu_plateau_update": (I, [P, P, P, P, I, I, D, I, D, I, D, D, P]),
    "ctu_sgd": (I, [P, P, I, P, P, D, D, D, D, I, I, P, P, P]),
    "ctu_rmsprop": (I, [P, P, I, P, P, D, D, D, D, D, I, I, P, P, P]),
}

_lib = None
ABI_VERSION = 8


class CtuError(RuntimeError):
    """A libctunet_hip.so entry point returned a non-zero status."""


def load() -> C.CDLL:
    global _lib
    if _lib is not None:
        return _lib
    if not os.path.exists(LIB_PATH):
        raise ImportError(
            f"{LIB_PATH} not found: the MI355X kernels are not built. Run `python __graft_entry__.py` "
            "(or `make -C ct-unet_amd/csrc`). There is no CPU fallback for this path.")
    lib = C.CDLL(LIB_PATH)
    for name, (res, args) in SIGNATURES.items():
        try:
            fn = getattr(lib, name)
        except AttributeError as e:
            raise ImportError(f"{LIB_PATH} does not export {name}; rebuild the library") from e
        fn.restype = res
        fn.argtypes = args
    if lib.ctu_abi_version() != ABI_VERSION:
        raise ImportError(f"{LIB_PATH} is ABI v{lib.ctu_abi_version()}, this package binds v{ABI_VERSION}: "
                          "a stale build -- run `python __graft_entry__.py` (or `make -C ct-unet_amd/csrc`)")
    _lib = lib
# ... 53 lines not shown
```

### ct-unet_amd/ctunet_amd/engine.py

```python
from __future__ import annotations

import os
from dataclasses import dataclass
from typing import Dict, List, Optional, Tuple

import torch

from . import ops
from .ops import CL, pad8

BN_EPS = 1e-5
FUSE_UP = os.environ.get("CTUNET_FUSE_UP", "1") != "0"
FUSE_UP_MAX_CO = int(os.environ.get("CTUNET_FUSE_UP_MAXCO", "16"))
POOL_BN = os.environ.get("CTUNET_POOL_BN", "1") != "0"
LP_FUSE_UP = os.environ.get("CTUNET_LP_FUSE_UP", "1") != "0"
BN_MOMENTUM = 0.1
LAZY_BN = os.environ.get("CTUNET_LAZY_BN", "1") != "0"
LAZY_BN_LP = os.environ.get("CTUNET_LAZY_BN_LP", "0") != "0"
BN_TAIL = os.environ.get("CTUNET_BN_TAIL", "0") != "0"
DEFER_WGRAD_REDUCE = os.environ.get("CTUNET_DEFER_WGRAD_REDUCE", "1") != "0"


@dataclass
class BlockPlan:
    prefix: str
    first: int
    cin: int
    cout: int


@dataclass
class NetPlan:
    k: int
    conv_bias: bool
    in_ch: int
    out_ch: int
    enc: List[BlockPlan]
    center: BlockPlan
    center_live: bool
    dec: List[BlockPlan]
    head: str
    act: int
    head_mode: int
    skip: str = "cat"


@dataclass(slots=True)
class _ConvRec:
    x: Optional[CL]
    y: CL
    vec: torch.Tensor
    stats: Optional[torch.Tensor]
    nblk: int
    conv: str
    bn: str
    cin: int
    cout: int
    imap: Optional[torch.Tensor]
    bias: bool
    first: Optional[torch.Tensor] = None


class _WgradWs:

    def __init__(self, floats: int, device, defer: bool):
        self.jobs = ops.WgradJobs() if defer else None
        self.bufs = [torch.empty(floats, dtype=torch.float32, device=device) for _ in range(2 if defer else 1)]
        self.i = 0

    def take(self) -> torch.Tensor:
        self.i = (self.i + 1) % len(self.bufs)
        ws = self.bufs[self.i]
        if self.jobs is not None:
            if self.jobs.uses(ws):
                self.jobs.flush()
            assert not self.jobs.uses(ws)
        return ws

    def flush(self) -> None:
        if self.jobs is not None:
            self.jobs.flush()


class UNetEngine:
    def __init__(self, plan: NetPlan, dtype: torch.dtype = torch.float32, loss_scale: Optional[float] = None):
        if dtype not in ops.ACT_DTYPES:
            raise ValueError(f"ctunet_amd: activation dtype {dtype} not supported (float32, bfloat16, float16)")
        self.plan = plan
        self.dtype = dtype
        self.loss_scale = loss_scale
        self.scaler = None
        self._pack_cache: Dict[Tuple, Tuple[int, torch.Tensor]] = {}
        self._replay_stats = False
        self._up_cache: Dict[str, Tuple] = {}
        self._imaps: Dict[Tuple, torch.Tensor] = {}
        self._tail_words: Dict[str, torch.Tensor] = {}
        self._tail_slots: Dict[Tuple[str, str], int] = {}
        self._overflow: Dict[str, torch.Tensor] = {}
        self._gy_bufs: Dict[int, Tuple[torch.Tensor, torch.Tensor]] = {}

    def overflow_flag(self, device) -> torch.Tensor:
        f = self._overflow.get(str(device))
        if f is None:
            f = self._overflow[str(device)] = torch.zeros(1, dtype=torch.float32, device=device)
        return f

    def _counter(self, layer: str, direction: str, device) -> Optional[torch.Tensor]:
        if not BN_TAIL:
            return None
        words = self._tail_words.get(str(device))
        if words is None:
            words = self._tail_words[str(device)] = torch.zeros(1024, dtype=torch.int32, device=device)
        slot = self._tail_slots.setdefault((layer, direction), len(self._tail_slots))
        if slot >= words.numel():
            raise RuntimeError("ctunet_amd: more than 1024 BatchNorm tails in one engine")
        return words[slot:slot + 1]

    def _maps(self, segs: Tuple[Tuple[int, int], ...], cp: int, device):
        idx: List[int] = []
        for n, start in segs:
            idx += list(range(start, start + n))
        if idx == list(range(len(idx))):
            return None, None
        key = (segs, cp, str(device))
        t = self._imaps.get(key)
        if t is None:
            inv = [-1] * cp
            for logical, pos in enumerate(idx):
                inv[pos] = logical
            t = (torch.tensor(idx, dtype=torch.int32, device=device), torch.tensor(inv, dtype=torch.int32, device=device))
            self._imaps[key] = t
        return t

    def _packed(self, name: str, w: torch.Tensor, kind: str, imap, rin_p: int, nout_p: int, mode: int,
                layout: int = 0) -> torch.Tensor:
        key = (name, kind, mode, rin_p, nout_p, layout, self.dtype)
        hit = self._pack_cache.get(key)
        ver = (w._version, w.data_ptr())
        if hit is not None and hit[0] == ver:
            return hit[1]
        wd = w.detach()
        if self.dtype != torch.float32:
            wp = self._pack_lp(kind, wd, imap, rin_p, nout_p, mode, hit[1] if hit is not None else None, layout)
        else:
            wp = hit[1] if hit is not None else torch.empty(ops.packed_floats(kind, w.shape[2], rin_p, nout_p, layout),
                                                            dtype=torch.float32, device=w.device)
            ops.pack_batch([(kind, wd.contiguous(), wp, imap, rin_p, nout_p, mode, layout)], self.dtype)
        self._pack_cache[key] = (ver, wp, imap)
        return wp

    def _pack_lp(self, kind, wd, imap, rin_p, nout_p, mode, into, layout=0):
        if kind == "conv":
            return ops.pack_conv_w_lp(wd, imap, rin_p, nout_p, mode, self.dtype, into, layout)
        return ops.pack_convt_w_lp(wd, imap, rin_p, nout_p, mode, self.dtype, into)

    def refresh_packs(self, P: Dict[str, torch.Tensor]) -> None:
        force = P and next(iter(P.values())).is_cuda and torch.cuda.is_current_stream_capturing()
        jobs = []
        for key, ent in self._pack_cache.items():
            name, kind, mode, rin_p, nout_p, layout, dt = key
            w = P.get(name + ".weight")
            if w is None or w.device != ent[1].device or dt != self.dtype:
                continue
            ver = (w._version, w.data_ptr())
            if force or ent[0] != ver:
                jobs.append((kind, w.detach().contiguous(), ent[1], ent[2], rin_p, nout_p, mode, layout))
                self._pack_cache[key] = (ver, ent[1], ent[2])
        ops.pack_batch(jobs, self.dtype)

    def invalidate_packs(self) -> None:
        for key, ent in self._pack_cache.items():
            self._pack_cache[key] = (None,) + tuple(ent[1:])
        for prefix, hit in self._up_cache.items():
            self._up_cache[prefix] = (None,) + tuple(hit[1:])

    def _fwd_tail(self, P, bn: str, c: int, nvox: int, n_upd: int, vec4: torch.Tensor, device):
        counter = self._counter(bn, "fwd", device)
        if counter is None:
            return None
        return ops.make_bn_tail(c, nvox, P[bn + ".weight"], P[bn + ".bias"], P[bn + ".running_mean"], P[bn + ".running_var"],
                                BN_MOMENTUM, BN_EPS, n_upd, vec4, P.get(bn + ".num_batches_tracked") if n_upd else None,
                                counter)

    def _bn_stage(self, P, bn: str, out: CL, vec4: torch.Tensor, nvox: int, c: int, training: bool, n_upd: int, nblk: int,
                  launch, tail_ok: bool = True) -> Tuple[CL, Optional[torch.Tensor]]:
        wb = (P[bn + ".weight"], P[bn + ".bias"], P[bn + ".running_mean"], P[bn + ".running_var"])
        if training:
            stats = torch.empty((nblk, 2, out.cp), dtype=torch.float32, device=out.buf.device)
            tail = self._fwd_tail(P, bn, c, nvox, n_upd, vec4, out.buf.device) if tail_ok else None
            launch(stats, tail)
            if tail is None:
                ops.bn_finalize_into(stats, nblk, c, out.cp, nvox, *wb, BN_MOMENTUM, BN_EPS, n_upd, vec4,
                                     P.get(bn + ".num_batches_tracked") if n_upd else None)
        else:
            stats = None
            launch(None, None)
            ops.bn_eval_affine_into(*wb, BN_EPS, c, out.cp, vec4)
        return out.with_xf(vec4[0], vec4[1], True), stats

    def _conv_bn(self, P, x: CL, conv: str, bn: str, cin: int, cout: int, imap, out: CL, vec4: torch.Tensor,
                 training: bool, n_upd: int, save: bool) -> Tuple[CL, Optional[_ConvRec]]:
        k = self.plan.k
        w = P[conv + ".weight"]
        bias = P.get(conv + ".bias")
        lay = ops.conv_layout(k, out.cp, x.dims[3], self.dtype, x.cp)
        if bias is not None and self.dtype != torch.float32:
            lay = 0
        wp = self._packed(conv, w, "conv", imap, x.cp, out.cp, 0, lay)
        bias_p = None if bias is None else bias.detach()
        nblk = ops.conv_num_blocks(x.dims, out.cp, lay, k, self.dtype, x.cp) if training else 0
        y, stats = self._bn_stage(P, bn, out, vec4, x.nvox, cout, training, n_upd, nblk,
                                  lambda stats, tail: ops.conv3d_fwd(x, wp, bias_p, out, k, stats, (cin, cout), lay, tail))
        rec = _ConvRec(x, out.raw(), vec4, stats, nblk, conv, bn, cin, cout, imap, bias is not None) if save else None
        return y, rec

    def _fuse_up(self, x: CL, nout_p: int) -> bool:
        if not (self.plan.k == 3 and not self.plan.conv_bias and nout_p <= FUSE_UP_MAX_CO and FUSE_UP):
            return False
        if self.dtype == torch.float32:
            return ops.upconv_fused_supported(x.dims, 3, x.cp, nout_p)
        return LP_FUSE_UP and ops.lp_upconv_fused_supported(x.dims, 3, x.cp, nout_p)

    def _upconv_bn(self, P, x: CL, prefix: str, ct: int, cout: int, cinv, out: CL, vec4: torch.Tensor, training: bool,
                   n_upd: int, save: bool) -> Tuple[CL, Optional[_ConvRec]]:
        conv, bn = f"{prefix}.1", f"{prefix}.2"
        wt, bt, w3 = P[f"{prefix}.0.weight"], P[f"{prefix}.0.bias"], P[conv + ".weight"]
        lp = bool(x.lp)
        ver = tuple((t._version, t.data_ptr()) for t in (wt, bt, w3))
        hit = self._up_cache.get(prefix)
        if hit is None or hit[0] != ver or hit[3] != (x.cp, out.cp, self.dtype) or torch.cuda.is_current_stream_capturing():
            same = hit is not None and hit[3] == (x.cp, out.cp, self.dtype)
            if lp:
                wp, beff, pws = ops.upconv_fused_pack(wt, bt, w3, cinv, x.cp, out.cp, (hit[1], hit[2], hit[4]) if same else None)
                wpd = ops.lp_upconv_fused_pack(wp, x.cp, self.dtype, hit[5] if same else None)
            else:
                wp, beff, pws, wpd = ops.upconv_fused_pack_all(wt, bt, w3, cinv, x.cp, out.cp,
                                                               (hit[1], hit[2], hit[4], hit[5]) if same else None)
            self._up_cache[prefix] = (ver, wp, beff, (x.cp, out.cp, self.dtype), pws, wpd)
        else:
            wp, beff, wpd = hit[1], hit[2], hit[5]
        if lp:
            nblk = ops.lp_upconv_fused_num_blocks(x.dims) if training else 0
            launch = lambda stats, tail: ops.lp_upconv_fused_fwd(x, wpd, beff, out, stats, (ct, cout))
        else:
            nblk = ops.upconv_fused_num_blocks(x.dims, out.cp) if training else 0
            launch = lambda stats, tail: ops.upconv_fused_fwd(x, wp, beff, out, stats, (ct, cout), tail)
        y, stats = self._bn_stage(P, bn, out, vec4, 8 * x.nvox, cout, training, n_upd, nblk, launch, tail_ok=not lp)
        rec = _ConvRec(None, out.raw(), vec4, stats, nblk, conv, bn, ct, cout, None, False) if save else None
        return y, rec

    def _first_conv_bn(self, P, x: torch.Tensor, conv: str, bn: str, cin: int, cout: int, out: CL, vec4: torch.Tensor,
                       training: bool, n_upd: int, save: bool):
        w = P[conv + ".weight"].detach()
        bias = P.get(conv + ".bias")
        bias_p = None if bias is None else bias.detach()
        nblk = ops.conv_first_num_blocks(out.dims) if training else 0
        y, stats = self._bn_stage(P, bn, out, vec4, out.nvox, cout, training, n_upd, nblk,
                                  lambda stats, tail: ops.conv_first_fwd(x, w, bias_p, out, stats, tail))
        rec = _ConvRec(None, out.raw(), vec4, stats, nblk, conv, bn, cin, cout, None, bias is not None, x) if save else None
        return y, rec

    def forward(self, P: Dict[str, torch.Tensor], x: torch.Tensor, training: bool, save: bool, chk: bool):
        plan = self.plan
        dev = x.device
        n, cin, d, h, w = x.shape
        nlev = len(plan.enc)
        if cin != plan.in_ch:
            raise RuntimeError(f"ctunet_amd: expected {plan.in_ch} input channels, got {cin}")
        if any(s % (1 << nlev) for s in (d, h, w)):
            raise RuntimeError(f"ctunet_amd: spatial size {(d, h, w)} must be divisible by {1 << nlev}")
        if training and n * (d >> nlev) * (h >> nlev) * (w >> nlev) <= 1:
            raise ValueError("Expected more than 1 value per channel when training (centre block)")
        ctx = {"recs": {}, "levels": [], "training": training, "chk": chk} if save else None
        n_upd = 1 if training else 0
        self.refresh_packs(P)

        x = x.contiguous()
        e0 = plan.enc[0]
        first_direct = plan.conv_bias is False and ops.conv_first_supported(plan.k, cin, pad8(e0.cout), w)
        adt = self.dtype
        cur = None if first_direct else ops.ncdhw_to_cl(x, dtype=adt)
        x_cl = cur
        cat: List[torch.Tensor] = []
        xf: List[torch.Tensor] = []
        pooled: List[CL] = []
        dskip: List[CL] = []
        dd, hh, ww = d, h, w
        recs = {}
        xf_sizes = [8 * pad8(blk.cout) for blk in plan.enc]
        xf_all = torch.zeros(sum(xf_sizes), dtype=torch.float32, device=dev)
        xf_off = 0
        for i, blk in enumerate(plan.enc):
            cp = pad8(blk.cout)
            cat.append(torch.empty((n, dd, hh, ww, 2 * cp), dtype=adt, device=dev))
            xf.append(xf_all[xf_off:xf_off + 8 * cp].view(4, 2 * cp))
            xf_off += 8 * cp
            t1 = CL(torch.empty((n, dd, hh, ww, cp), dtype=adt, device=dev), 0, cp)
            v1 = torch.empty((4, cp), dtype=torch.float32, device=dev)
            imap = None
            if i == 0 and first_direct:
                a1, recs[(blk.prefix, 1)] = self._first_conv_bn(P, x, f"{blk.prefix}.{blk.first}",
                                                                f"{blk.prefix}.{blk.first + 1}", blk.cin, blk.cout, t1,
                                                                v1, training, n_upd, save)
            else:
                a1, recs[(blk.prefix, 1)] = self._conv_bn(P, cur, f"{blk.prefix}.{blk.first}",
                                                          f"{blk.prefix}.{blk.first + 1}", blk.cin, blk.cout, imap, t1,
                                                          v1, training, n_upd, save)
            a2, recs[(blk.prefix, 2)] = self._conv_bn(P, a1, f"{blk.prefix}.{blk.first + 3}", f"{blk.prefix}.{blk.first + 4}",
                                                      blk.cout, blk.cout, None, CL(cat[i], cp, cp), xf[i][:, cp:],
                                                      training, n_upd, save)
            dskip.append(a2)
            dd, hh, ww = dd // 2, hh // 2, ww // 2
            pl = CL(torch.empty((n, dd, hh, ww, cp), dtype=adt, device=dev), 0, cp)
            ops.maxpool_fwd(a2, pl)
            pooled.append(pl)
            cur = pl
        cb = plan.center
        cpc = pad8(cb.cout)
        center_out = None
        if plan.center_live or training:
            live = plan.center_live
            c1 = CL(torch.empty((n, dd, hh, ww, cpc), dtype=adt, device=dev), 0, cpc)
            c2 = CL(torch.empty((n, dd, hh, ww, cpc), dtype=adt, device=dev), 0, cpc)
            v1 = torch.empty((4, cpc), dtype=torch.float32, device=dev)
            v2 = torch.empty((4, cpc), dtype=torch.float32, device=dev)
            a1, r1 = self._conv_bn(P, cur, f"{cb.prefix}.{cb.first}", f"{cb.prefix}.{cb.first + 1}", cb.cin, cb.cout,
                                   None, c1, v1, training, n_upd, save and live)
            a2, r2 = self._conv_bn(P, a1, f"{cb.prefix}.{cb.first + 3}", f"{cb.prefix}.{cb.first + 4}", cb.cout, cb.cout,
                                   None, c2, v2, training, n_upd, save and live)
            if live:
                recs[(cb.prefix, 1)], recs[(cb.prefix, 2)] = r1, r2
                center_out = a2
        cur = center_out if plan.center_live else pooled[-1]
        cur_segs = ((cb.cout if plan.center_live else plan.enc[-1].cout, 0),)
        dec_in: List[CL] = []
        ups: List[CL] = []
        for j, blk in enumerate(plan.dec):
            i = nlev - 1 - j
            cp = pad8(blk.cout)
            dd, hh, ww = dd * 2, hh * 2, ww * 2
            ct = blk.cin
            ctp = pad8(ct)
            imap_t, cinv_t = self._maps(cur_segs, cur.cp, dev)
            wt = P[f"{blk.prefix}.0.weight"]
            dec_in.append(cur)
            t1 = CL(torch.empty((n, dd, hh, ww, cp), dtype=adt, device=dev), 0, cp)
            v1 = torch.empty((4, cp), dtype=torch.float32, device=dev)
            if self._fuse_up(cur, cp):
                ups.append(None)
                a1, recs[(blk.prefix, 1)] = self._upconv_bn(P, cur, blk.prefix, ct, blk.cout, cinv_t, t1, v1, training,
                                                            n_upd, save)
            else:
                up = CL(torch.empty((n, dd, hh, ww, ctp), dtype=adt, device=dev), 0, ctp)
                wpt = self._packed(f"{blk.prefix}.0", wt, "convt", cinv_t, cur.cp, ctp, 0)
                ops.convt_fwd(cur, wpt, P[f"{blk.prefix}.0.bias"].detach(), up)
                ups.append(up)
                a1, recs[(blk.prefix, 1)] = self._conv_bn(P, up, f"{blk.prefix}.1", f"{blk.prefix}.2", ct, blk.cout, None,
                                                          t1, v1, training, n_upd, save)
            a2, recs[(blk.prefix, 2)] = self._conv_bn(P, a1, f"{blk.prefix}.4", f"{blk.prefix}.5", blk.cout, blk.cout, None,
                                                      CL(cat[i], 0, cp), xf[i][:, :cp], training, n_upd, save)
            if plan.skip == "cat":
                cur = CL(cat[i], 0, 2 * cp, xf[i][0], xf[i][1], True)
                cur_segs = ((blk.cout, 0), (blk.cout, cp))
            elif plan.skip == "none":
                cur = CL(cat[i], 0, cp, xf[i][0][:cp], xf[i][1][:cp], True)
                cur_segs = ((blk.cout, 0),)
            else:
                cur = CL(torch.empty((n, dd, hh, ww, cp), dtype=adt, device=dev), 0, cp)
                ops.skip_add(CL(cat[i], 0, cp, xf[i][0][:cp], xf[i][1][:cp], True),
                             CL(cat[i], cp, cp, xf[i][0][cp:], xf[i][1][cp:], True), cur)
                cur_segs = ((blk.cout, 0),)
        imap_h, _ = self._maps(cur_segs, cur.cp, dev)
        wl, bl = P[plan.head + ".weight"], P[plan.head + ".bias"]
        w2 = wl.detach().reshape(wl.shape[0], wl.shape[1])
        out0, out1 = ops.head_fwd(cur, w2, bl.detach(), imap_h, plan.act, plan.head_mode)
        if save:
            ctx.update(recs=recs, x_cl=x_cl, cat=cat, xf=xf, pooled=pooled, dskip=dskip, dec_in=dec_in, ups=ups,
                       head_in=cur, imap_h=imap_h, center_out=center_out, dims=(n, d, h, w))
        return out0, out1, ctx

    def _replay(self, P, rec: _ConvRec):
        return ((P[rec.bn + ".running_mean"], P[rec.bn + ".running_var"], BN_MOMENTUM, BN_EPS,
                 P.get(rec.bn + ".num_batches_tracked")) if self._replay_stats else None)

    def _bwd_fin(self, P, rec: _ConvRec, device):
        counter = self._counter(rec.bn, "bwd", device)
        return None if counter is None else (P[rec.bn + ".weight"].detach(), rec.cout, self._replay(P, rec), counter)

    def _gy_like(self, ga: CL) -> CL:
        ent = self._gy_bufs.get(id(ga.buf))
        if ent is None:
            ent = self._gy_bufs[id(ga.buf)] = (ga.buf, torch.empty_like(ga.buf))
        return CL(ent[1], ga.c0, ga.cp)

    def _conv_bn_bwd(self, P, rec: _ConvRec, ga: CL, gin: Optional[CL], grads: Dict[str, torch.Tensor], ws: _WgradWs, part,
                     pre_reduced: Optional[int] = None, finalized=None, up_in: Optional[CL] = None):
        k = self.plan.k
        can = LAZY_BN and ga.cs == rec.y.cs and (not ga.lp or LAZY_BN_LP)
        if up_in is not None:
            lazy = can and (ops.lp_upconv_fused_wgrad_bn_supported(up_in.dims, up_in.cp) if ga.lp else
# ... 6 lines not shown
        res = ops.bn_relu_bwd(rec.y, ga, rec.vec, P[rec.bn + ".weight"].detach(), rec.cout, part, self._replay(P, rec),
                              pre_reduced, self._counter(rec.bn, "bwd", ga.buf.device), finalized, lazy, jobs)
        grads[rec.bn + ".weight"], grads[rec.bn + ".bias"] = res[0], res[1]
        if up_in is not None:
            return (rec.y, rec.vec, res[2], self._gy_like(ga)) if lazy else None
        if rec.first is not None:
            if lazy:
                gy = self._gy_like(ga)
                grads[rec.conv + ".weight"] = ops.conv_first_wgrad_bn(rec.first, ga, rec.y, rec.vec, res[2], gy, rec.cout,
                                                                      ws.take(), jobs)
                ga = gy
            else:
                grads[rec.conv + ".weight"] = ops.conv_first_wgrad(rec.first, ga, rec.cout, ws.take(), jobs)
            return ops.conv_first_bwd_data(ga, P[rec.conv + ".weight"].detach(), rec.cin) if gin is not None else None
        if lazy:
            gy = self._gy_like(ga)
            grads[rec.conv + ".weight"] = ops.conv3d_wgrad_bn(rec.x, ga, rec.y, rec.vec, res[2], gy, rec.cout, rec.cin, k,
                                                             rec.imap, ws.take(), jobs)
            ga = gy
        elif rec.x is not None:
            dw, dbias = ops.conv3d_wgrad(rec.x, ga, rec.cout, rec.cin, k, rec.imap, ws.take(), rec.bias, jobs)
            grads[rec.conv + ".weight"] = dw
            if rec.bias:
                grads[rec.conv + ".bias"] = dbias
        if gin is not None:
            lay = ops.conv_layout(k, gin.cp, ga.dims[3], self.dtype, ga.cp)
            wpd = self._packed(rec.conv, P[rec.conv + ".weight"], "conv", rec.imap, ga.cp, gin.cp, 1, lay)
            ops.conv3d_fwd(ga, wpd, None, gin, k, None, (rec.cout, rec.cin), lay)

    def backward(self, P: Dict[str, torch.Tensor], ctx, g0: torch.Tensor, g1: Optional[torch.Tensor],
                 need_dx: bool, sync=None):
        plan = self.plan
        recs = ctx["recs"]
        n, d, h, w = ctx["dims"]
        dev = g0.device
        nlev = len(plan.enc)
        gs = 1.0
        flag = None
        dyn = self.scaler if self.dtype == torch.float16 else None
        if dyn is not None:
            dyn.prepare(dev, n * d * h * w)
            flag = dyn.found_inf
        elif self.dtype == torch.float16:
            gs = self.loss_scale if self.loss_scale else float(2 ** max(0, (n * d * h * w).bit_length() - 5))
            flag = self.overflow_flag(dev)
            flag.zero_()
        grads: Dict[str, torch.Tensor] = {}
        emitted: set = set()
        self._gy_bufs = {}

        def unscale(tensors):
            if dyn is not None:
                ops.unscale_tensors(tensors, dyn.scale, flag)
            elif gs != 1.0:
                ops.scale_tensors(tensors, 1.0 / gs, flag)

        def emit():
            new = [(nm, g) for nm, g in grads.items() if nm not in emitted and g is not None]
            emitted.update(nm for nm, _ in new)
            if sync is not None or dyn is not None or gs != 1.0:
                ws.flush()
            unscale([g for _, g in new])
            if sync is not None:
                sync.push(new)
        k = plan.k
        ws_n, part_n = 1, 1
        for r in recs.values():
            if r is None:
                continue
            if r.first is not None:
                ws_n = max(ws_n, ops.conv_first_wgrad_ws(r.y.dims, r.cin))
                part_n = max(part_n, ops.bn_bwd_partials_floats(r.y.nvox, r.y.cp))
                continue
            ws_n = max(ws_n, ops.conv3d_wgrad_ws(r.y.dims, k, r.x.cp if r.x is not None else pad8(r.cin), r.y.cp, self.dtype))
            part_n = max(part_n, ops.bn_bwd_partials_floats(r.y.nvox, r.y.cp))
        for x_in, blk in zip(ctx["dec_in"], plan.dec):
            ws_n = max(ws_n, ops.convt_wgrad_ws(x_in.dims, x_in.cp, pad8(blk.cin), self.dtype))
        for dsk in ctx["dskip"]:
            part_n = max(part_n, ops.maxpool_bwd_bn_blocks(dsk.dims, dsk.cp) * 2 * dsk.cp)
        part_n = max(part_n, ops.head_bwd_blocks(ctx["head_in"].dims) * 2 * pad8(plan.dec[-1].cout))
        ws = _WgradWs(ws_n, dev, DEFER_WGRAD_REDUCE and self.dtype == torch.float32 and ops.TIMER is None)
        part = torch.empty(part_n, dtype=torch.float32, device=dev)

        self._replay_stats = bool(ctx["training"] and ctx["chk"])

        cat, head_in = ctx["cat"], ctx["head_in"]
        gcat = [torch.empty_like(c) for c in cat]
        wl, bl = P[plan.head + ".weight"], P[plan.head + ".bias"]
        w2 = wl.detach().reshape(wl.shape[0], wl.shape[1])
        gsd = None if dyn is None else dyn.scale
        def g_skip_target(level: int) -> CL:
            full = gcat[level].shape[-1]
            return CL(gcat[level], 0, full if plan.skip == "cat" else full // 2)

        def g_skip_fanout(level: int):
            if plan.skip == "add":
                half = gcat[level].shape[-1] // 2
                ops.skip_add(CL(gcat[level], 0, half), None, CL(gcat[level], half, half))

        r_last = recs[(plan.dec[-1].prefix, 2)]
        head_rows, head_fin = None, None
        if (POOL_BN and head_in.scale is not None and head_in.relu and head_in.scale.data_ptr() == r_last.vec[0].data_ptr()
                and head_in.c0 == r_last.y.c0 and head_in.buf is r_last.y.buf):
            fin = self._bwd_fin(P, r_last, head_in.buf.device)
            res = ops.head_bwd(head_in, w2, bl.detach(), ctx["imap_h"], plan.act, plan.head_mode, g0.contiguous(),
                               None if g1 is None else g1.contiguous(), g_skip_target(0), (r_last.vec, part), fin, gscale=gs,
                               gscale_dev=gsd)
            dwl, dbl, head_rows = res[:3]
            head_fin = res[3] if fin is not None else None
        else:
            dwl, dbl = ops.head_bwd(head_in, w2, bl.detach(), ctx["imap_h"], plan.act, plan.head_mode, g0.contiguous(),
                                    None if g1 is None else g1.contiguous(), g_skip_target(0), gscale=gs,
                                    gscale_dev=gsd)
        g_skip_fanout(0)
        grads[plan.head + ".weight"], grads[plan.head + ".bias"] = dwl.reshape(wl.shape), dbl
        emit()

        g_deep: Optional[CL] = None
        for j in range(nlev - 1, -1, -1):
            blk = plan.dec[j]
            i = nlev - 1 - j
            cp = pad8(blk.cout)
            r1, r2 = recs[(blk.prefix, 1)], recs[(blk.prefix, 2)]
            g_u2 = CL(gcat[i], 0, cp)
            g_u1 = CL(torch.empty_like(r1.y.buf), 0, cp)
            self._conv_bn_bwd(P, r2, g_u2, g_u1, grads, ws, part, head_rows if j == nlev - 1 else None,
                              head_fin if j == nlev - 1 else None)
            x_in = ctx["dec_in"][j]
            ct = blk.cin
            if j > 0 and plan.skip == "cat":
                segs = ((plan.dec[j - 1].cout, 0), (plan.dec[j - 1].cout, pad8(plan.dec[j - 1].cout)))
            else:
                segs = ((ct, 0),)
            imap_t, cinv_t = self._maps(segs, x_in.cp, dev)
            wt = P[f"{blk.prefix}.0.weight"]
            up = ctx["ups"][j]
            if j > 0:
                gin = g_skip_target(i + 1)
            else:
                gin = CL(torch.empty_like(x_in.buf), 0, x_in.cp)
                g_deep = gin
            if up is None:
                lz = self._conv_bn_bwd(P, r1, g_u1, None, grads, ws, part, up_in=x_in)
                gq = g_u1
                up_wgrad = ops.lp_upconv_fused_wgrad if g_u1.lp else ops.upconv_fused_wgrad
                dwt, dbt, dw3 = up_wgrad(x_in, gq, ct, blk.cout, P[f"{blk.prefix}.0.bias"], self._up_cache[blk.prefix][4], imap_t, lz)
                if lz is not None:
                    gq = lz[3]
                grads[f"{blk.prefix}.1.weight"] = dw3
                grads[f"{blk.prefix}.0.weight"], grads[f"{blk.prefix}.0.bias"] = dwt, dbt
                if g_u1.lp:
                    ops.lp_upconv_fused_bwd_data(gq, self._up_cache[blk.prefix][5], gin, (ct, blk.cout))
                else:
                    ops.upconv_fused_bwd_data(gq, self._up_cache[blk.prefix][5], gin, (ct, blk.cout))
            else:
                g_up = CL(torch.empty_like(up.buf), 0, up.cp)
                self._conv_bn_bwd(P, r1, g_u1, g_up, grads, ws, part)
                dwt, dbt = ops.convt_wgrad(x_in, g_up, ct, ct, imap_t, ws.take(), ws.jobs)
                grads[f"{blk.prefix}.0.weight"], grads[f"{blk.prefix}.0.bias"] = dwt, dbt
                wpd = self._packed(f"{blk.prefix}.0", wt, "convt", cinv_t, g_up.cp, x_in.cp, 1)
                ops.convt_bwd_data(g_up, wpd, gin)
            if j > 0:
                g_skip_fanout(i + 1)
            emit()
        g_pool = g_deep
        if plan.center_live:
            cb = plan.center
            r1, r2 = recs[(cb.prefix, 1)], recs[(cb.prefix, 2)]
            g_c1 = CL(torch.empty_like(r1.y.buf), 0, r1.y.cp)
            self._conv_bn_bwd(P, r2, g_deep, g_c1, grads, ws, part)
            g_pool = CL(torch.empty_like(ctx["pooled"][-1].buf), 0, ctx["pooled"][-1].cp)
            self._conv_bn_bwd(P, r1, g_c1, g_pool, grads, ws, part)
            emit()
        dx = None
        for i in range(nlev - 1, -1, -1):
            blk = plan.enc[i]
            cp = pad8(blk.cout)
            r1, r2 = recs[(blk.prefix, 1)], recs[(blk.prefix, 2)]
            g_d2 = CL(gcat[i], cp, cp)
            dsk = ctx["dskip"][i]
            fuse = (POOL_BN and dsk.scale is not None and dsk.relu and dsk.scale.data_ptr() == r2.vec[0].data_ptr()
                    and ops.maxpool_bwd_bn_blocks(dsk.dims, dsk.cp) > 0)
            fin = self._bwd_fin(P, r2, dsk.buf.device) if fuse else None
            nb = ops.maxpool_bwd(dsk, g_pool, g_d2, plan.skip != "none", (r2.vec, part) if fuse else None, fin)
            nb, done = nb if fin is not None else (nb, None)
            g_d1 = CL(torch.empty_like(r1.y.buf), 0, cp)
            self._conv_bn_bwd(P, r2, g_d2, g_d1, grads, ws, part, nb, done)
            if i > 0:
                g_pool = CL(torch.empty_like(ctx["pooled"][i - 1].buf), 0, ctx["pooled"][i - 1].cp)
                self._conv_bn_bwd(P, r1, g_d1, g_pool, grads, ws, part)
            elif need_dx and r1.first is not None:
                dx = self._conv_bn_bwd(P, r1, g_d1, True, grads, ws, part)
            elif need_dx:
                g_x = CL(torch.empty_like(ctx["x_cl"].buf), 0, ctx["x_cl"].cp)
                self._conv_bn_bwd(P, r1, g_d1, g_x, grads, ws, part)
                dx = ops.cl_to_ncdhw(g_x, plan.in_ch)
            else:
                self._conv_bn_bwd(P, r1, g_d1, None, grads, ws, part)
            emit()
        ws.flush()
        emit()
        unscale([dx])
        if sync is not None:
            if flag is not None:
                sync.push([("__overflow__", flag.clone())])
            grads.update(sync.finish())
            red = grads.pop("__overflow__", None)
            if red is not None:
                flag.copy_(red.reshape(1))
        self._gy_bufs = {}
        return grads, dx


class _UNetFn(torch.autograd.Function):
    @staticmethod
    def forward(fctx, module, engine, names, x_req, x, *params):
        P = _tensor_dict(module)
        out0, out1, ctx = engine.forward(P, x, module.training, True, bool(getattr(module, "chk", False)))
        fctx.engine, fctx.module, fctx.names, fctx.ctx = engine, module, names, ctx
        fctx.two = out1 is not None
        fctx.x_req = x_req
        fctx.versions = _versions(P, names)
        if out1 is None:
            return out0
        return out0, out1

    @staticmethod
    def backward(fctx, *gouts):
        if fctx.ctx is None:
            raise RuntimeError("ctunet_amd: backward through the same forward twice is not supported")
        g0 = gouts[0]
        g1 = gouts[1] if fctx.two else None
        ctx = fctx.ctx
        if g0 is None:
            g0 = torch.zeros(_out_shape(ctx, fctx, 0), device=ctx["cat"][0].device)
        if fctx.two and g1 is None:
            g1 = torch.zeros_like(g0)
        P = _tensor_dict(fctx.module)
        for nm, then, now in zip(fctx.names, fctx.versions, _versions(P, fctx.names)):
            if then != now:
                raise RuntimeError(f"ctunet_amd: parameter {nm} needed for gradient computation has been modified since the "
                                   f"forward pass (version {then[0]} then, {now[0]} now): run backward before changing weights")
        from .parallel import make_sync
        with torch.no_grad():
            grads, dx = fctx.engine.backward(P, ctx, g0, g1, fctx.x_req, make_sync(fctx.module))
        fctx.ctx = None
        return (None, None, None, None, dx) + tuple(grads.get(nm) for nm in fctx.names)


def _out_shape(ctx, fctx, idx):
    n, d, h, w = ctx["dims"]
    c = 2 if fctx.two else fctx.engine.plan.out_ch
    return (n, c, d, h, w)


def _versions(P: Dict[str, torch.Tensor], names) -> Tuple[Tuple[int, int], ...]:
    return tuple((P[nm]._version, P[nm].data_ptr()) for nm in names)


def _tensor_dict(module) -> Dict[str, torch.Tensor]:
    P = dict(module.named_parameters())
    P.update(dict(module.named_buffers()))
    return P


def check_input(module, x: torch.Tensor) -> None:
    if not isinstance(x, torch.Tensor) or x.dim() != 5:
        raise RuntimeError("ctunet_amd: expected a [N, C, D, H, W] tensor")
    if not x.is_cuda:
        raise RuntimeError("ctunet_amd: this model runs on the MI355X only (input is on %s); there is no CPU path"
                           % x.device)
    if x.dtype != torch.float32:
        raise RuntimeError(f"ctunet_amd: fp32 input expected, got {x.dtype}")
    for p in module.parameters():
        if p.device != x.device:
            raise RuntimeError("ctunet_amd: module parameters and input must be on the same GPU (call .to(device))")


def run_network(module, engine: UNetEngine, x: torch.Tensor):
    check_input(module, x)
    names, params = zip(*module.named_parameters())
    need_grad = torch.is_grad_enabled() and (x.requires_grad or any(p.requires_grad for p in params))
    if not need_grad:
        with torch.no_grad():
            out0, out1, _ = engine.forward(_tensor_dict(module), x, module.training, False, False)
        return out0 if out1 is None else (out0, out1)
    return _UNetFn.apply(module, engine, names, x.requires_grad, x, *params)
```

### ct-unet_amd/ctunet_amd/ops.py

```python
from __future__ import annotations

import contextlib
import ctypes
import gc
import os

from dataclasses import dataclass
from typing import Optional, Tuple

import torch

from . import _lib


def pad8(c: int) -> int:
    return (c + 7) // 8 * 8


LP_CODE = {torch.bfloat16: 1, torch.float16: 2}
ACT_DTYPES = (torch.float32, torch.bfloat16, torch.float16)


def _need_cuda(t: torch.Tensor, name: str) -> None:
    if not t.is_cuda:
# ... 693 lines not shown
    return dw, db


def convt_wgrad_ws(dims, cin_p, cout_p, dtype=torch.float32) -> int:
    n, d, h, w = dims
    return _query(lp(dtype), "convt2_wgrad_ws_floats", n, d, h, w, cin_p, cout_p)


def head_fwd(x: CL, w: torch.Tensor, b: torch.Tensor, imap, act: int, head_mode: int):
    n, d, h, w_ = x.dims
    co, ci = w.shape[0], w.shape[1]
    v = d * h * w_
    dev = x.buf.device
    if head_mode == 0:
        out0 = torch.empty((n, co, d, h, w_), dtype=torch.float32, device=dev)
        out1 = None
    else:
        out0 = torch.empty((n, 2, d, h, w_), dtype=torch.float32, device=dev)
        out1 = torch.empty((n, 2, d, h, w_), dtype=torch.float32, device=dev)
    _dual(x.lp, "head_fwd", x.ptr, x.cs, x.cp, _ptr(x.scale), _ptr(x.shift), int(x.relu), w.data_ptr(), b.data_ptr(),
          _ptr(imap), ci, co, act, head_mode, out0.data_ptr(), _ptr(out1), n, v, _stream())
    return out0, out1


def head_bwd(x: CL, w: torch.Tensor, b: torch.Tensor, imap, act: int, head_mode: int, g0: torch.Tensor,
             g1: Optional[torch.Tensor], gin: CL, bn=None, fin=None, gscale: float = 1.0,
             gscale_dev: Optional[torch.Tensor] = None):
    assert gscale == 1.0 or x.lp, "gscale is the 16-bit path's loss scale"
    assert gscale_dev is None or (x.lp and gscale_dev.is_cuda and gscale_dev.dtype == torch.float32), \
        "gscale_dev is the 16-bit path's device loss scale"
    n, d, h, w_ = x.dims
    co, ci = w.shape[0], w.shape[1]
    v = d * h * w_
    dev = x.buf.device
    lib = _lib.load()
    ws = torch.empty(lib.ctu_head_bwd_ws_floats(n, v, x.cp, co), dtype=torch.float32, device=dev)
    dw = torch.empty_like(w)
    db = torch.empty_like(b)
    bn_args, tail, done = (None, None, 0, None), None, None
    if bn is not None:
        vec, partials = bn
        bn_cp = vec.shape[1]
        rows = lib.ctu_head_bwd_num_blocks(n, v)
        assert x.scale is not None and x.relu and vec[0].data_ptr() == x.scale.data_ptr() and partials.numel() >= rows * 2 * bn_cp
        bn_args = (vec[2].data_ptr(), vec[3].data_ptr(), bn_cp, partials.data_ptr())
        if fin is not None:
            gamma, c, replay = fin[:3]
            tail, done = _bn_bwd_outputs(c, bn_cp, n * v, gamma, vec, replay, None, dev)
    entry, scale = "head_bwd_bn", ((float(gscale),) if x.lp else ())
    if gscale_dev is not None:
        entry, scale = "head_bwd_bn_dscale", (gscale_dev.data_ptr(),)
    _dual(x.lp, entry, x.ptr, x.cs, x.cp, _ptr(x.scale), _ptr(x.shift), int(x.relu), w.data_ptr(), b.data_ptr(), _ptr(imap),
          ci, co, act, head_mode, g0.data_ptr(), _ptr(g1), gin.ptr, gin.cs, dw.data_ptr(), db.data_ptr(), ws.data_ptr(), n, v,
          *bn_args, _tail_arg(tail), *scale, _stream())
    if bn is None:
        return dw, db
    return (dw, db, rows) if fin is None else (dw, db, rows, done)


def head_bwd_blocks(dims) -> int:
    n, d, h, w_ = dims
    return _lib.load().ctu_head_bwd_num_blocks(n, d * h * w_)


def loss_fwd(pred: torch.Tensor, target: torch.Tensor, ce_lambda: float, dice_lambda: float, dice_softmax: bool):
    _need_cuda(pred, "prediction")
    _need_cuda(target, "target")
    assert pred.shape == target.shape and pred.shape[1] == 2, "loss kernel handles 2-channel maps"
    pred, target = pred.contiguous(), target.contiguous()
    n = pred.shape[0]
    v = pred[0, 0].numel()
    lib = _lib.load()
    ws = torch.empty(lib.ctu_loss_ws_floats(n, v), dtype=torch.float32, device=pred.device)
    terms = torch.empty(2, dtype=torch.float32, device=pred.device)
    _lib.check(lib.ctu_loss_fwd(pred.data_ptr(), target.data_ptr(), n, v, ce_lambda, dice_lambda, int(dice_softmax),
                                terms.data_ptr(), ws.data_ptr(), _stream()), "loss_fwd")
    return terms, ws


def loss_bwd(pred, target, ce_lambda, dice_lambda, dice_softmax, ws, g_ce: Optional[torch.Tensor],
             g_dice: Optional[torch.Tensor], out: Optional[torch.Tensor] = None, accumulate: bool = False) -> torch.Tensor:
    pred, target = pred.contiguous(), target.contiguous()
    for g_ in (g_ce, g_dice):
        assert g_ is None or (g_.is_cuda and g_.dtype == torch.float32 and g_.numel() == 1)
    n = pred.shape[0]
    v = pred[0, 0].numel()
    g = out if out is not None else torch.empty_like(pred)
    lib = _lib.load()
    _lib.check(lib.ctu_loss_bwd(pred.data_ptr(), target.data_ptr(), n, v, ce_lambda, dice_lambda, int(dice_softmax),
                                ws.data_ptr(), _ptr(g_ce), _ptr(g_dice), g.data_ptr(), int(accumulate), _stream()),
               "loss_bwd")
    return g



def skip_add(a: CL, b: Optional[CL], out: CL) -> None:
    assert out.dims == a.dims and out.cp == a.cp and (b is None or (b.dims == a.dims and b.cp == a.cp))
    assert out.dtype == a.dtype and (b is None or b.dtype == a.dtype)
    _dual(a.lp, "skip_add", a.ptr, a.cs, _ptr(a.scale), _ptr(a.shift), int(a.relu), 0 if b is None else b.ptr,
          0 if b is None else b.cs, _ptr(b.scale) if b is not None else 0, _ptr(b.shift) if b is not None else 0,
          int(b.relu) if b is not None else 0, out.ptr, out.cs, out.cp, a.nvox, _stream())


def channel_sum(x: CL, c: int) -> torch.Tensor:
    lib = _lib.load()
    nb = lib.ctu_channel_sum_num_blocks(x.nvox)
    part = torch.empty(nb * x.cp, dtype=torch.float32, device=x.buf.device)
    out = torch.empty(c, dtype=torch.float32, device=x.buf.device)
    _dual(x.lp, "channel_sum", x.ptr, x.cs, x.cp, x.nvox, part.data_ptr(), out.data_ptr(), c, _stream())
    return out


def upconv_fused_supported(dims, k: int, cin_p: int, nout_p: int) -> bool:
    n, d, h, w = dims
    return bool(_lib.load().ctu_upconv_fused_supported(k, d, h, w, cin_p, nout_p))


def upconv_fused_pack(wt: torch.Tensor, bt: torch.Tensor, w3: torch.Tensor, cinv, cin_p: int, nout_p: int,
                      into=None):
    return _upconv_pack(wt, bt, w3, cinv, cin_p, nout_p, into, False)


def upconv_fused_pack_all(wt: torch.Tensor, bt: torch.Tensor, w3: torch.Tensor, cinv, cin_p: int, nout_p: int,
                          into=None):
    return _upconv_pack(wt, bt, w3, cinv, cin_p, nout_p, into, True)


def _upconv_pack(wt, bt, w3, cinv, cin_p, nout_p, into, with_wpd: bool):
    lib = _lib.load()
    c, co = wt.shape[0], w3.shape[0]
    assert wt.shape == (c, c, 2, 2, 2) and w3.shape == (co, c, 3, 3, 3) and bt.shape == (c,)
    if into is not None:
        bufs = tuple(into)
        assert len(bufs) == 3 + with_wpd
    else:
        new = lambda n: torch.empty(n, dtype=torch.float32, device=wt.device)
        bufs = (new(lib.ctu_upconv_fused_packed_floats(cin_p, nout_p)), new((27, nout_p)),
                new(lib.ctu_upconv_fused_pack_ws_floats(c, nout_p)))
        if with_wpd:
            bufs += (new(lib.ctu_upconv_fused_bwd_packed_floats(cin_p, nout_p)),)
    wp, beff, ws = bufs[:3]
    _lib.check(lib.ctu_upconv_fused_pack_all(wt.detach().contiguous().data_ptr(), bt.detach().contiguous().data_ptr(),
                                             w3.detach().contiguous().data_ptr(), c, co, _ptr(cinv), cin_p, nout_p, wp.data_ptr(),
                                             beff.data_ptr(), ws.data_ptr(), bufs[3].data_ptr() if with_wpd else None, _stream()),
               "upconv_fused_pack")
    return bufs


def upconv_fused_num_blocks(dims, nout_p: int) -> int:
    n, d, h, w = dims
    return _lib.load().ctu_upconv_fused_num_blocks(n, d, h, w, nout_p)


def upconv_fused_fwd(x: CL, wp: torch.Tensor, beff: torch.Tensor, out: CL, stats: Optional[torch.Tensor],
                     algo_ch: Optional[Tuple[int, int]] = None, tail=None) -> None:
    n, d, h, w = x.dims
    assert out.dims == (n, 2 * d, 2 * h, 2 * w)
    ci, co = algo_ch if algo_ch is not None else (x.cp, out.cp)
    vox = n * d * h * w
    with _timed(lambda: (f"upconv_fused_fwd_kernel<{out.cp}>", vox * (16.0 * ci * ci + 8 * 54.0 * ci * co),
                         4.0 * vox * (ci + 8 * co), (w, x.cp, out.cp))):
        _lib.check(_lib.load().ctu_upconv_fused_fwd(x.ptr, x.cs, x.cp, _ptr(x.scale), _ptr(x.shift), int(x.relu),
                                                    wp.data_ptr(), beff.data_ptr(), out.ptr, out.cs, out.cp, _ptr(stats),
                                                    n, d, h, w, _tail_arg(tail), _stream()), "upconv_fused_fwd")


def upconv_fused_wgrad_bn_supported(dims, cin_p: int, nout_p: int, dtype=torch.float32) -> bool:
    n, d, h, w = dims
    return dtype == torch.float32 and bool(_lib.load().ctu_upconv_fused_wgrad_bn_supported(n, d, h, w, cin_p, nout_p))


def upconv_fused_wgrad(x: CL, g: CL, c: int, co: int, bt: torch.Tensor, pack_ws: torch.Tensor, imap, lazy=None):
    n, d, h, w = x.dims
    assert g.dims == (n, 2 * d, 2 * h, 2 * w) and not x.lp
    return _upconv_wgrad(x, g, c, co, bt, pack_ws, imap, lazy,
                         lambda: (f"upconv_fused_wgrad_kernel<{g.cp}> (+slab reduce)", 4.0 * (n * d * h * w) * (c + 8 * co)))


def _upconv_wgrad(x: CL, g: CL, c: int, co: int, bt, pack_ws, imap, lazy, tag_bytes):
    n, d, h, w = x.dims
    dev = x.buf.device
    gcp = () if x.lp else (g.cp,)
    dweff = torch.empty((8, 8, x.cp, g.cp), dtype=torch.float32, device=dev)
    ws = torch.empty(_query(x.lp, "upconv_fused_wgrad_ws_floats", n, d, h, w, x.cp, *gcp), dtype=torch.float32, device=dev)
    act = (x.ptr, x.cs, x.cp, _ptr(x.scale), _ptr(x.shift), int(x.relu), g.ptr, g.cs, *gcp)
    detail = (w, x.cp, g.cp)

    def record():
        tag, nbytes = tag_bytes()
        return tag, (n * d * h * w) * (16.0 * c * c + 8 * 54.0 * c * co), nbytes, detail
    with _timed(record):
        if lazy is not None:
            y, vec, coef, gy = lazy
            assert y.dims == g.dims and gy.dims == g.dims and y.cs == g.cs == gy.cs and y.cp == g.cp == gy.cp
            assert gy.buf.data_ptr() != g.buf.data_ptr()
            _dual(x.lp, "upconv_fused_wgrad_bn", *act, y.ptr, vec[0].data_ptr(), vec[1].data_ptr(), coef.data_ptr(), gy.ptr,
                  dweff.data_ptr(), ws.data_ptr(), n, d, h, w, _stream())
            g = gy
        else:
            _dual(x.lp, "upconv_fused_wgrad", *act, dweff.data_ptr(), ws.data_ptr(), n, d, h, w, _stream())
    dwt = torch.empty((c, c, 2, 2, 2), dtype=torch.float32, device=dev)
    dbt = torch.empty(c, dtype=torch.float32, device=dev)
    dw3 = torch.empty((co, c, 3, 3, 3), dtype=torch.float32, device=dev)
    ws2 = torch.empty(_lib.load().ctu_upconv_fused_project_ws_floats(g.cp, g.nvox), dtype=torch.float32, device=dev)
    _dual(x.lp, "upconv_fused_project", dweff.data_ptr(), g.ptr, g.cs, g.cp, n, d, h, w, bt.detach().data_ptr(),
          pack_ws.data_ptr(), _ptr(imap), c, co, x.cp, dwt.data_ptr(), dbt.data_ptr(), dw3.data_ptr(), ws2.data_ptr(), _stream())
    return dwt, dbt, dw3


def lp_upconv_fused_supported(dims, k: int, cin_p: int, nout_p: int) -> bool:
    n, d, h, w = dims
    return bool(_lib.load().ctu_lp_upconv_fused_supported(k, d, h, w, cin_p, nout_p))


def lp_upconv_fused_pack(wp32: torch.Tensor, cin_p: int, dtype: torch.dtype, into: Optional[torch.Tensor] = None) -> torch.Tensor:
    lib = _lib.load()
    n = lib.ctu_lp_upconv_fused_packed_elems(cin_p)
    wp16 = into if into is not None else torch.empty(n, dtype=dtype, device=wp32.device)
    assert wp16.numel() == n and wp16.dtype == dtype
    _lib.check(lib.ctu_lp_upconv_fused_pack(LP_CODE[dtype], wp32.data_ptr(), cin_p, wp16.data_ptr(), _stream()), "lp_upconv_fused_pack")
    return wp16


def lp_upconv_fused_num_blocks(dims) -> int:
    n, d, h, w = dims
    return _lib.load().ctu_lp_upconv_fused_num_blocks(n, d, h, w)


def lp_upconv_fused_fwd(x: CL, wp16: torch.Tensor, beff: torch.Tensor, out: CL, stats: Optional[torch.Tensor],
                        algo_ch: Optional[Tuple[int, int]] = None) -> None:
    n, d, h, w = x.dims
    assert out.dims == (n, 2 * d, 2 * h, 2 * w) and x.lp and out.dtype == x.dtype and wp16.dtype == x.dtype and out.cp == 8
    ci, co = algo_ch if algo_ch is not None else (x.cp, out.cp)
    vox = n * d * h * w
    with _timed(lambda: (f"lp_upconv_fwd_kernel<{_lp_name(x.lp)}>", vox * (16.0 * ci * ci + 8 * 54.0 * ci * co),
                         2.0 * vox * (x.cp + 8 * out.cp), (w, x.cp, out.cp))):
        _lib.check(_lib.load().ctu_lp_upconv_fused_fwd(x.lp, x.ptr, x.cs, x.cp, _ptr(x.scale), _ptr(x.shift), int(x.relu),
                                                       wp16.data_ptr(), beff.data_ptr(), out.ptr, out.cs, _ptr(stats),
                                                       n, d, h, w, _stream()), "lp_upconv_fused_fwd")


def lp_upconv_fused_wgrad_bn_supported(dims, cin_p: int) -> bool:
    n, d, h, w = dims
    return bool(_lib.load().ctu_lp_upconv_fused_wgrad_bn_supported(n, d, h, w, cin_p))


def lp_upconv_fused_wgrad(x: CL, g: CL, c: int, co: int, bt: torch.Tensor, pack_ws: torch.Tensor, imap, lazy=None):
    n, d, h, w = x.dims
    assert g.dims == (n, 2 * d, 2 * h, 2 * w) and x.lp and g.dtype == x.dtype and g.cp == 8 and g.cs == 8
    return _upconv_wgrad(x, g, c, co, bt, pack_ws, imap, lazy,
                         lambda: (f"lp_upconv_wgrad_kernel<{_lp_name(x.lp)}> (+slab reduce)", 2.0 * (n * d * h * w) * (x.cp + 8 * g.cp)))


def lp_upconv_fused_bwd_data(g: CL, wp16: torch.Tensor, gin: CL, algo_ch: Optional[Tuple[int, int]] = None) -> None:
    n, d, h, w = gin.dims
    assert g.dims == (n, 2 * d, 2 * h, 2 * w) and g.lp and gin.dtype == g.dtype and wp16.dtype == g.dtype and g.cp == 8
    ci, co = algo_ch if algo_ch is not None else (gin.cp, g.cp)
    vox = n * d * h * w
    with _timed(lambda: (f"lp_upconv_bwd_data_kernel<{_lp_name(g.lp)}>", vox * (16.0 * ci * ci + 8 * 54.0 * ci * co),
                         2.0 * vox * (gin.cp + 8 * g.cp), (w, gin.cp, g.cp))):
        _lib.check(_lib.load().ctu_lp_upconv_fused_bwd_data(g.lp, g.ptr, g.cs, wp16.data_ptr(), gin.ptr, gin.cs, gin.cp,
                                                            n, d, h, w, _stream()), "lp_upconv_fused_bwd_data")


def upconv_fused_pack_bwd(wp: torch.Tensor, cin_p: int, nout_p: int, into: Optional[torch.Tensor] = None) -> torch.Tensor:
    lib = _lib.load()
    wpd = into if into is not None else torch.empty(lib.ctu_upconv_fused_bwd_packed_floats(cin_p, nout_p),
                                                     dtype=torch.float32, device=wp.device)
    _lib.check(lib.ctu_upconv_fused_pack_bwd(wp.data_ptr(), cin_p, nout_p, wpd.data_ptr(), _stream()), "upconv_fused_pack_bwd")
    return wpd


def upconv_fused_bwd_data(g: CL, wpd: torch.Tensor, gin: CL, algo_ch: Optional[Tuple[int, int]] = None) -> None:
    n, d, h, w = gin.dims
    assert g.dims == (n, 2 * d, 2 * h, 2 * w)
    ci, co = algo_ch if algo_ch is not None else (gin.cp, g.cp)
    vox = n * d * h * w
    with _timed(lambda: (f"upconv_fused_bwd_data_kernel<{g.cp}>", vox * (16.0 * ci * ci + 8 * 54.0 * ci * co),
                         4.0 * vox * (ci + 8 * co), (w, gin.cp, g.cp))):
        _lib.check(_lib.load().ctu_upconv_fused_bwd_data(g.ptr, g.cs, g.cp, wpd.data_ptr(), gin.ptr, gin.cs, gin.cp,
                                                         n, d, h, w, _stream()), "upconv_fused_bwd_data")


def _ncv(t: torch.Tensor):
    if t.dtype != torch.float32 or not t.is_cuda or not t.is_contiguous() or t.dim() not in (4, 5):
        raise RuntimeError("ctunet_amd: expected a contiguous float32 CUDA map [N,C,D,H,W] or [C,D,H,W]")
    n = t.shape[0] if t.dim() == 5 else 1
    c = t.shape[1] if t.dim() == 5 else t.shape[0]
    return n, c, t.numel() // (n * c)


def hard_segm(prob: torch.Tensor) -> torch.Tensor:
    n, c, v = _ncv(prob)
    out = torch.empty(prob.shape[:1] + prob.shape[2:] if prob.dim() == 5 else prob.shape[1:], dtype=torch.float32,
                      device=prob.device)
    _lib.check(_lib.load().ctu_hard_segm(prob.data_ptr(), n, c, v, out.data_ptr(), _stream()), "hard_segm")
    return out


def one_hot(label: torch.Tensor, num_classes: int) -> torch.Tensor:
    if label.dtype != torch.float32 or not label.is_cuda or not label.is_contiguous() or label.dim() != 4:
        raise RuntimeError("ctunet_amd: expected a contiguous float32 CUDA label volume [N,D,H,W]")
    n = label.shape[0]
    out = torch.empty((n, num_classes) + tuple(label.shape[1:]), dtype=torch.float32, device=label.device)
    _lib.check(_lib.load().ctu_one_hot(label.data_ptr(), n, num_classes, label.numel() // n, out.data_ptr(), _stream()),
               "one_hot")
    return out


def hard_dice_counts(pred: torch.Tensor, target: torch.Tensor) -> torch.Tensor:
    n, c, v = _ncv(pred)
    if target.shape != pred.shape or _ncv(target) != (n, c, v):
        raise RuntimeError("ctunet_amd: prediction and one-hot target must have the same shape")
    lib = _lib.load()
    ws = torch.empty(lib.ctu_hard_dice_ws_doubles(n), dtype=torch.float64, device=pred.device)
    counts = torch.empty((n, c, 3), dtype=torch.float64, device=pred.device)
    _lib.check(lib.ctu_hard_dice_counts(pred.data_ptr(), target.data_ptr(), n, c, v, counts.data_ptr(), ws.data_ptr(),
                                        _stream()), "hard_dice_counts")
    return counts


def hausdorff(pred: torch.Tensor, target: torch.Tensor) -> torch.Tensor:
    n, c, v = _ncv(pred)
    if pred.dim() != 5 or target.shape != pred.shape or _ncv(target) != (n, c, v):
        raise RuntimeError("ctunet_amd: hausdorff expects a [N,C,D,H,W] prediction and a one-hot target of the same shape")
    d, h, w = pred.shape[2:]
    lib = _lib.load()
    ws = torch.empty(lib.ctu_hausdorff_ws_bytes(n, c, d, h, w), dtype=torch.uint8, device=pred.device)
    out = torch.empty((n, c - 1), dtype=torch.float32, device=pred.device)
    _lib.check(lib.ctu_hausdorff(pred.data_ptr(), target.data_ptr(), n, c, d, h, w, out.data_ptr(), ws.data_ptr(), _stream()),
               "hausdorff")
    return out


def extract_patches(vol: torch.Tensor, coords: torch.Tensor, patch: Tuple[int, int, int]) -> torch.Tensor:
    _need_cuda(vol, "volume")
    _need_cuda(coords, "patch coordinates")
    if vol.dim() != 4 or coords.dim() != 2 or coords.shape[1] != 3 or coords.dtype != torch.int32:
        raise RuntimeError("ctunet_amd: extract_patches expects vol [C,D,H,W] and int32 coords [P,3]")
    vol, coords = vol.contiguous(), coords.contiguous()
    c, d, h, w = vol.shape
    p = coords.shape[0]
    out = torch.empty((p, c) + tuple(patch), dtype=torch.float32, device=vol.device)
    _lib.check(_lib.load().ctu_extract_patches(vol.data_ptr(), coords.data_ptr(), p, c, d, h, w, patch[0], patch[1], patch[2],
                                               out.data_ptr(), _stream()), "extract_patches")
    return out


def stitch_patches(patches: torch.Tensor, coords: torch.Tensor, shape: Tuple[int, int, int]) -> torch.Tensor:
    _need_cuda(patches, "patches")
    _need_cuda(coords, "patch coordinates")
    if patches.dim() != 5 or coords.shape != (patches.shape[0], 3) or coords.dtype != torch.int32:
        raise RuntimeError("ctunet_amd: stitch_patches expects patches [P,C,pd,ph,pw] and int32 coords [P,3]")
    patches, coords = patches.contiguous(), coords.contiguous()
    p, c, pd, ph, pw = patches.shape
    out = torch.empty((c,) + tuple(shape), dtype=torch.float32, device=patches.device)
    _lib.check(_lib.load().ctu_stitch_patches(patches.data_ptr(), coords.data_ptr(), p, c, shape[0], shape[1], shape[2], pd, ph,
                                              pw, out.data_ptr(), _stream()), "stitch_patches")
    return out


def window_accumulate(patches: torch.Tensor, coords: torch.Tensor, valid: torch.Tensor, box: torch.Tensor,
                      tables: Tuple[torch.Tensor, torch.Tensor, torch.Tensor], wmin: float, extent: Tuple[int, int, int],
                      num: torch.Tensor, wsum: Optional[torch.Tensor]) -> None:
    for t, nm in ((patches, "patches"), (coords, "coordinates"), (valid, "valid flags"), (box, "box origin"), (num, "num")):
        _need_cuda(t, nm)
        assert t.is_contiguous(), nm
    assert wsum is None or (wsum.is_cuda and wsum.dtype == torch.float32 and wsum.is_contiguous())
    b, k, pd, ph, pw = patches.shape
    _, d, h, w = num.shape
    wz, wy, wx = tables
    assert num.shape[0] == k and (wsum is None or wsum.shape == num.shape[1:]), "accumulator shapes"
    assert coords.shape == (b, 3) and valid.numel() == b and box.numel() == 3 and coords.dtype == torch.int32
    assert all(t.is_cuda and t.dtype == torch.float32 and t.is_contiguous() and t.numel() == n
               for t, n in zip(tables, (pd, ph, pw))), "weight tables"
    _lib.check(_lib.load().ctu_window_accumulate(patches.data_ptr(), coords.data_ptr(), valid.data_ptr(), box.data_ptr(), b,
                                                 k, d, h, w, pd, ph, pw, wz.data_ptr(), wy.data_ptr(), wx.data_ptr(),
                                                 float(wmin), extent[0], extent[1], extent[2], num.data_ptr(), _ptr(wsum),
                                                 _stream()), "window_accumulate")


def window_finalize(num: torch.Tensor, wsum: torch.Tensor, probs: torch.Tensor,
                    labels: Optional[torch.Tensor] = None) -> None:
    _need_cuda(num, "num")
    _need_cuda(wsum, "wsum")
    _need_cuda(probs, "probs")
    k = num.shape[0]
    v = wsum.numel()
    assert num.is_contiguous() and wsum.is_contiguous() and probs.is_contiguous() and num.numel() == k * v == probs.numel()
    assert labels is None or (labels.is_cuda and labels.dtype == torch.uint8 and labels.numel() == v and labels.is_contiguous())
    _lib.check(_lib.load().ctu_window_finalize(num.data_ptr(), wsum.data_ptr(), k, v, probs.data_ptr(), _ptr(labels),
                                               _stream()), "window_finalize")


def _tensor_table(tensors):
    ts = [t for t in tensors if t is not None]
    for t in ts:
        _need_cuda(t, "tensor")
        assert t.is_contiguous() and t.dtype == torch.float32
    return ((ctypes.c_void_p * len(ts))(*[t.data_ptr() for t in ts]), (ctypes.c_int64 * len(ts))(*[t.numel() for t in ts]),
            len(ts))


def scale_tensors(tensors, s: float, nonfinite: Optional[torch.Tensor] = None) -> None:
    pa, sa, n = _tensor_table(tensors)
    if not n:
        return
    assert nonfinite is None or (nonfinite.is_cuda and nonfinite.dtype == torch.float32 and nonfinite.numel() == 1)
    _lib.check(_lib.load().ctu_scale_tensors(pa, sa, n, float(s), _ptr(nonfinite), _stream()), "scale_tensors")


def unscale_tensors(tensors, scale: torch.Tensor, found_inf: torch.Tensor) -> None:
    pa, sa, n = _tensor_table(tensors)
    if not n:
        return
    for f in (scale, found_inf):
        assert f.is_cuda and f.dtype == torch.float32 and f.numel() == 1
    _lib.check(_lib.load().ctu_unscale_tensors(pa, sa, n, scale.data_ptr(), found_inf.data_ptr(), _stream()),
               "unscale_tensors")


FLAP_CHUNK = 8192
FLAP_RECORD = 16
FLAP_HOLE, FLAP_NOISE = 1, 2


def _skull_kind(t: torch.Tensor, name: str) -> int:
    if not t.is_cuda:
        raise RuntimeError(f"ctunet_amd: {name} must live on the GPU (MI355X); this path has no CPU fallback")
    if t.dtype not in (torch.float32, torch.uint8):
        raise RuntimeError(f"ctunet_amd: {name} must be float32 or uint8, got {t.dtype}")
    assert t.is_contiguous(), name
    return int(t.dtype == torch.uint8)

# ... 110 lines not shown
```

### include/ctunet_hip.h

```cpp
#ifndef CTUNET_HIP_H
#define CTUNET_HIP_H

#include <stddef.h>
#include <stdint.h>

#ifdef __cplusplus
extern "C" {
#endif

#define CTU_OK 0
#define CTU_EINVAL (-1)
#define CTU_ELAUNCH (-2)

#define CTU_F32 0
#define CTU_BF16 1
#define CTU_F16 2

typedef struct ctu_bn_tail {
    const float* gamma; const float* beta;
    float* running_mean; float* running_var;
    float* scale; float* shift; float* mean; float* invstd;
    long long* num_batches_tracked;
    unsigned int* counter;
    double count;
// ... 48 lines not shown
int ctu_conv3d_wgrad(const float* in, int in_cs, int cin_p,
                     const float* in_scale, const float* in_shift, int in_relu,
                     const float* gout, int g_cs, int cout_p,
                     float* dw, float* dbias, int Co, int Ci, const int32_t* cinv,
                     float* ws, int N, int D, int H, int W, int k, void* stream);
int ctu_conv3d_wgrad_bn_supported(int N, int D, int H, int W, int k, int cin_p, int cout_p);
int ctu_conv3d_wgrad_bn(const float* in, int in_cs, int cin_p,
                        const float* in_scale, const float* in_shift, int in_relu,
                        const float* ga, int g_cs, int cout_p, const float* y,
                        const float* bn_scale, const float* bn_shift, const float* coef, float* gy_out,
                        float* dw, int Co, int Ci, const int32_t* cinv,
                        float* ws, int N, int D, int H, int W, int k, void* stream);

int ctu_conv3d_first_supported(int k, int cin, int nout_p, int W);
int ctu_conv3d_first_num_blocks(int N, int D, int H, int W);
int ctu_conv3d_first_fwd(const float* x, int cin, const float* w, const float* bias, int nbias,
                         float* out, int out_cs, int Co, float* stats,
                         int N, int D, int H, int W, const ctu_bn_tail* tail, void* stream);
int ctu_conv3d_first_bwd_data(const float* g, int g_cs, const float* w, int cin, int Co, float* dx,
                              int N, int D, int H, int W, void* stream);
size_t ctu_conv3d_first_wgrad_ws_floats(int N, int D, int H, int W, int cin);
int ctu_conv3d_first_wgrad(const float* x, int cin, const float* g, int g_cs, float* dw, int Co,
                           float* ws, int N, int D, int H, int W, void* stream);
int ctu_conv3d_first_wgrad_bn(const float* x, int cin, const float* ga, int g_cs, const float* y, const float* bn_scale,
                              const float* bn_shift, const float* coef, float* gy_out, float* dw, int Co, float* ws,
                              int N, int D, int H, int W, void* stream);

int ctu_bn_finalize(const float* stats, int nblocks, int C, int cp, double count,
                    const float* gamma, const float* beta,
                    float* running_mean, float* running_var, float momentum, float eps,
                    int n_updates, float* scale, float* shift, float* mean_out,
                    float* invstd_out, long long* num_batches_tracked, void* stream);
int ctu_bn_eval_affine(const float* gamma, const float* beta, const float* running_mean,
                       const float* running_var, float eps, int C, int cp,
                       float* scale, float* shift, void* stream);

int ctu_bn_bwd_num_blocks(int64_t nvox);
int ctu_bn_relu_bwd_reduce(const float* y, int y_cs, const float* ga, int g_cs, int cp,
                           const float* scale, const float* shift, const float* mean,
                           const float* invstd, int64_t nvox, float* partials, const ctu_bn_bwd_tail* tail, void* stream);
int ctu_bn_bwd_finalize(const float* partials, int nb, int C, int cp, double count,
                        const float* gamma, const float* invstd,
                        float* dgamma, float* dbeta, float* coef, const float* mean,
                        float* running_mean, float* running_var, float momentum, float eps,
                        long long* num_batches_tracked, void* stream);
int ctu_bn_relu_bwd_apply(const float* y, int y_cs, float* ga, int g_cs, int cp,
                          const float* scale, const float* shift, const float* mean,
                          const float* invstd, const float* coef, int64_t nvox, void* stream);

#define CTU_WGRAD_JOBS_MAX 4
typedef struct ctu_wgrad_job {
    const float* ws;
    float* dw; float* db;
    const int32_t* cinv;
    int kind;
    int Co, Ci, cin_p, n_ci_g, gx, pairs, nmf;
} ctu_wgrad_job;
int ctu_conv3d_wgrad_slabs(const float* in, int in_cs, int cin_p,
                           const float* in_scale, const float* in_shift, int in_relu,
                           const float* gout, int g_cs, int cout_p,
                           float* dw, float* dbias, int Co, int Ci, const int32_t* cinv,
                           float* ws, int N, int D, int H, int W, int k, ctu_wgrad_job* job, void* stream);
int ctu_conv3d_wgrad_bn_slabs(const float* in, int in_cs, int cin_p,
                              const float* in_scale, const float* in_shift, int in_relu,
                              const float* ga, int g_cs, int cout_p, const float* y,
                              const float* bn_scale, const float* bn_shift, const float* coef, float* gy_out,
                              float* dw, int Co, int Ci, const int32_t* cinv,
                              float* ws, int N, int D, int H, int W, int k, ctu_wgrad_job* job, void* stream);
int ctu_conv3d_first_wgrad_slabs(const float* x, int cin, const float* g, int g_cs, float* dw, int Co,
                                 float* ws, int N, int D, int H, int W, ctu_wgrad_job* job, void* stream);
int ctu_conv3d_first_wgrad_bn_slabs(const float* x, int cin, const float* ga, int g_cs, const float* y, const float* bn_scale,
                                    const float* bn_shift, const float* coef, float* gy_out, float* dw, int Co, float* ws,
                                    int N, int D, int H, int W, ctu_wgrad_job* job, void* stream);
int ctu_convt2_wgrad_slabs(const float* in, int in_cs, int cin_p, const float* in_scale,
                           const float* in_shift, int in_relu, const float* gout, int g_cs,
                           int cout_p, float* dw, float* dbias, int Ci, int Co,
                           const int32_t* imap, float* ws, int N, int D, int H, int W, ctu_wgrad_job* job, void* stream);
int ctu_bn_bwd_finalize_jobs(const float* partials, int nb, int C, int cp, double count,
                             const float* gamma, const float* invstd,
                             float* dgamma, float* dbeta, float* coef, const float* mean,
                             float* running_mean, float* running_var, float momentum, float eps,
                             long long* num_batches_tracked, const ctu_wgrad_job* jobs, int njobs, void* stream);
int ctu_wgrad_reduce_jobs(const ctu_wgrad_job* jobs, int njobs, void* stream);

int ctu_maxpool2_fwd(const float* in, int in_cs, int cp, const float* in_scale,
                     const float* in_shift, int in_relu, float* out, int out_cs,
                     int N, int D, int H, int W, void* stream);
int ctu_maxpool2_bwd(const float* in, int in_cs, int cp, const float* in_scale,
                     const float* in_shift, int in_relu, const float* gout, int gout_cs,
                     float* gin, int gin_cs, int accumulate, int N, int D, int H, int W,
                     void* stream);
int ctu_maxpool2_bwd_bn_num_blocks(int N, int D, int H, int W, int cp);
int ctu_maxpool2_bwd_bn(const float* in, int in_cs, int cp, const float* in_scale, const float* in_shift,
                        const float* mean, const float* invstd, const float* gout, int gout_cs, float* gin,
                        int gin_cs, int accumulate, int N, int D, int H, int W, float* partials, const ctu_bn_bwd_tail* tail, void* stream);

size_t ctu_convt_packed_floats(int rin_p, int nout_p);
int ctu_pack_convt_weight(const float* w, float* wp, int Ci, int Co, const int32_t* cinv,
                          int rin_p, int nout_p, int mode, void* stream);
int ctu_convt2_fwd(const float* in, int in_cs, int rin_p, const float* in_scale,
                   const float* in_shift, int in_relu, const float* wp, const float* bias,
                   int nbias, float* out, int out_cs, int nout_p, int N, int D, int H, int W,
                   void* stream);
int ctu_convt2_bwd_data(const float* gout, int g_cs, int rout_p, const float* wp,
                        float* gin, int gin_cs, int nin_p, int N, int D, int H, int W,
                        void* stream);
size_t ctu_convt2_wgrad_ws_floats(int N, int D, int H, int W, int cin_p, int cout_p);
int ctu_convt2_wgrad(const float* in, int in_cs, int cin_p, const float* in_scale,
                     const float* in_shift, int in_relu, const float* gout, int g_cs,
                     int cout_p, float* dw, float* dbias, int Ci, int Co,
                     const int32_t* imap, float* ws, int N, int D, int H, int W, void* stream);
const char* ctu_convt2_plan(int mode, int rin_p, int nout_p, int N, int D, int H, int W, int* plan);
const char* ctu_convt2_wgrad_plan(int cin_p, int cout_p, int N, int D, int H, int W, int* plan);

int ctu_head_fwd(const float* in, int in_cs, int cin_p, const float* in_scale,
                 const float* in_shift, int in_relu, const float* w, const float* bias,
                 const int32_t* imap, int Ci, int Co, int act, int head_mode,
                 float* out0, float* out1, int N, int64_t nvox_per_item, void* stream);
size_t ctu_head_bwd_ws_floats(int N, int64_t nvox_per_item, int cin_p, int Co);
int ctu_head_bwd(const float* in, int in_cs, int cin_p, const float* in_scale,
                 const float* in_shift, int in_relu, const float* w, const float* bias,
                 const int32_t* imap, int Ci, int Co, int act, int head_mode,
                 const float* g0, const float* g1, float* gin, int gin_cs,
                 float* dw, float* db, float* ws, int N, int64_t nvox_per_item, void* stream);
int ctu_head_bwd_num_blocks(int N, int64_t nvox_per_item);
int ctu_head_bwd_bn(const float* in, int in_cs, int cin_p, const float* in_scale,
                    const float* in_shift, int in_relu, const float* w, const float* bias,
                    const int32_t* imap, int Ci, int Co, int act, int head_mode,
                    const float* g0, const float* g1, float* gin, int gin_cs,
                    float* dw, float* db, float* ws, int N, int64_t nvox_per_item,
                    const float* bn_mean, const float* bn_invstd, int bn_cp, float* bn_partials, const ctu_bn_bwd_tail* tail, void* stream);

size_t ctu_loss_ws_floats(int N, int64_t V);
int ctu_loss_fwd(const float* pred, const float* target, int N, int64_t V, float ce_lambda,
                 float dice_lambda, int dice_softmax, float* terms, float* ws, void* stream);
int ctu_loss_bwd(const float* pred, const float* target, int N, int64_t V, float ce_lambda,
                 float dice_lambda, int dice_softmax, const float* ws, const float* gscale_ce,
                 const float* gscale_dice, float* gpred, int accumulate, void* stream);

int ctu_skip_add(const float* a, int a_cs, const float* a_scale, const float* a_shift, int a_relu,
                 const float* b, int b_cs, const float* b_scale, const float* b_shift, int b_relu,
                 float* out, int out_cs, int cp, int64_t nvox, void* stream);
int ctu_upconv_fused_supported(int k, int D, int H, int W, int cin_p, int nout_p);
size_t ctu_upconv_fused_packed_floats(int cin_p, int nout_p);
int ctu_upconv_fused_num_blocks(int N, int D, int H, int W, int nout_p);
size_t ctu_upconv_fused_pack_ws_floats(int C, int nout_p);
int ctu_upconv_fused_pack(const float* wt, const float* bt, const float* w3, int C, int Co, const int32_t* cinv,
                          int cin_p, int nout_p, float* wp, float* beff, float* ws, void* stream);
int ctu_upconv_fused_pack_all(const float* wt, const float* bt, const float* w3, int C, int Co, const int32_t* cinv,
                              int cin_p, int nout_p, float* wp, float* beff, float* ws, float* wpd, void* stream);
int ctu_upconv_fused_fwd(const float* in, int in_cs, int cin_p, const float* in_scale, const float* in_shift,
                         int in_relu, const float* wp, const float* beff, float* out, int out_cs, int nout_p,
                         float* stats, int N, int D, int H, int W, const ctu_bn_tail* tail, void* stream);

size_t ctu_upconv_fused_wgrad_ws_floats(int N, int D, int H, int W, int cin_p, int nout_p);
int ctu_upconv_fused_wgrad(const float* in, int in_cs, int cin_p, const float* in_scale, const float* in_shift,
                           int in_relu, const float* gout, int g_cs, int nout_p, float* dweff, float* ws,
                           int N, int D, int H, int W, void* stream);
int ctu_upconv_fused_wgrad_bn_supported(int N, int D, int H, int W, int cin_p, int nout_p);
int ctu_upconv_fused_wgrad_bn(const float* in, int in_cs, int cin_p, const float* in_scale, const float* in_shift,
                              int in_relu, const float* ga, int g_cs, int nout_p, const float* y,
                              const float* bn_scale, const float* bn_shift, const float* coef, float* gy_out,
                              float* dweff, float* ws, int N, int D, int H, int W, void* stream);
size_t ctu_upconv_fused_project_ws_floats(int nout_p, int64_t fine_nvox);
int ctu_upconv_fused_project(const float* dweff, const float* gout, int g_cs, int nout_p, int N, int D, int H, int W,
                             const float* bt, const float* pack_ws, const int32_t* imap, int C, int Co, int cin_p,
                             float* dwt, float* dbt, float* dw3, float* ws, void* stream);

size_t ctu_upconv_fused_bwd_packed_floats(int cin_p, int nout_p);
int ctu_upconv_fused_pack_bwd(const float* wp, int cin_p, int nout_p, float* wpd, void* stream);
int ctu_upconv_fused_bwd_data(const float* gout, int g_cs, int nout_p, const float* wpd, float* gin, int gin_cs,
                              int cin_p, int N, int D, int H, int W, void* stream);

int ctu_hard_segm(const float* prob, int N, int C, int64_t nvox_per_item, float* seg, void* stream);
int ctu_one_hot(const float* label, int N, int C, int64_t nvox_per_item, float* out, void* stream);
size_t ctu_hard_dice_ws_doubles(int N);
int ctu_hard_dice_counts(const float* pred, const float* target, int N, int C, int64_t nvox_per_item,
                         double* counts, double* ws, void* stream);

size_t ctu_hausdorff_ws_bytes(int N, int C, int D, int H, int W);
int ctu_hausdorff(const float* pred, const float* target, int N, int C, int D, int H, int W, float* out, void* ws,
                  void* stream);

#define CTU_U8 3
#define CTU_I64 4
size_t ctu_surface_ws_bytes(int N, int Cs, int D, int H, int W);
int ctu_surface_metrics(const void* pred, int pred_dtype, int pred_onehot, const void* target, int target_dtype,
                        int target_onehot, int N, int C, int cls0, int Cs, int D, int H, int W, const float* spacing,
                        const double* tau, double percentile, float* out, void* ws, void* stream);

#define CTU_CC_LARGEST 0
#define CTU_CC_MIN_SIZE 1
size_t ctu_components_ws_bytes(int N, int D, int H, int W);
int ctu_label_components(const void* in, int dtype, int N, int D, int H, int W, int connectivity, const int64_t* applied,
                         int n_applied, int32_t* labels, int32_t* num, void* ws, void* stream);
int ctu_filter_components(const void* in, int dtype, int N, int D, int H, int W, int connectivity,
                          const int64_t* applied, int n_applied, int mode, int param, void* out, void* ws, void* stream);

#define CTU_MORPH_ERODE 0
#define CTU_MORPH_DILATE 1
#define CTU_MORPH_OPEN 2
#define CTU_MORPH_CLOSE 3
#define CTU_MORPH_WS_MORPH 0
#define CTU_MORPH_WS_FILL 1
#define CTU_MORPH_WS_IMPLANT 2
size_t ctu_morphology_ws_bytes(int N, int D, int H, int W, int kind);
int ctu_binary_morphology(const void* in, int dtype, int N, int D, int H, int W, int mode, uint32_t structure,
                          int iterations, int border, int has_label, int64_t label, uint8_t* out, void* ws, void* stream);
int ctu_fill_holes(const void* in, int dtype, int N, int D, int H, int W, int connectivity, int has_label, int64_t label,
                   uint8_t* out, void* ws, void* stream);
int ctu_implant_mask(const void* full, int full_dtype, const void* defective, int defective_dtype, int N, int D, int H,
                     int W, uint32_t structure, int opening_iterations, int fill_holes, int connectivity,
                     int num_components, uint8_t* out, void* ws, void* stream);

#define CTU_DIST_EDT 0
#define CTU_DIST_SQUARED 1
#define CTU_DIST_SIGNED 2
#define CTU_DIST_BALL 3
size_t ctu_distance_ws_bytes(int N, int D, int H, int W, int out_kind, int want_indices);
int ctu_distance_transform(const void* in, int dtype, int N, int D, int H, int W, int has_label, int64_t label, int invert,
                           int border_background, const float* spacing, int out_kind, void* out, int32_t* indices,
                           float ball_r2, void* ws, void* stream);

#define CTU_I16 5
#define CTU_I32 6
#define CTU_RESAMPLE_NEAREST 0
#define CTU_RESAMPLE_LINEAR 1
#define CTU_RESAMPLE_LABEL_LINEAR 2
int ctu_resample(const void* in, int dtype, int mode, int num_classes, int64_t N, int D, int H, int W, int d, int h, int w,
                 const int32_t* i0, const float* wt, const int32_t* near, void* out, void* stream);

int ctu_affine_resample(const void* in, int dtype, int mode, int num_classes, int64_t N, int D, int H, int W, int d, int h,
                        int w, const double* out_to_in, const double* spacing, const double* origin,
                        const double* out_spacing, const double* out_origin, double fill, void* out, void* stream);

#define CTU_REG_MAX_BLOCKS 1024
#define CTU_REG_MIN_INLIERS 6
size_t ctu_registration_ws_bytes(int64_t P);
int ctu_registration_init(const float* points, int64_t P, const double* init, void* ws, void* stream);
int ctu_registration_accumulate(const float* points, int64_t P, const float* field, int D, int H, int W,
                                const double* spacing, const double* origin, double max_distance, void* ws, void* stream);
int ctu_registration_update(int64_t P, int it, double* matrix, double* inverse, double* history, int history_rows, void* ws,
                            void* stream);

#define CTU_MESH_SCAN_BLOCK 1024
#define CTU_MESH_MEASURE_WS 16384
size_t ctu_mesh_ws_bytes(int D, int H, int W);
int ctu_mesh_count(const void* volume, int dtype, int D, int H, int W, int has_label, int64_t label, float level, void* ws,
                   void* stream);
int ctu_mesh_emit(const void* volume, int dtype, int D, int H, int W, float level, float fill_value, const float* spacing,
                  const float* origin, int64_t V, int64_t F, float* vertices, int32_t* faces, void* ws, void* stream);
int ctu_mesh_measure(const float* vertices, int64_t V, const int32_t* faces, int64_t F, double* out, float* normals, void* ws,
                     void* stream);

#define CTU_MESH_ADJ_SCAN_CHUNK 4096
#define CTU_MESH_SMOOTH_MAX_ITERATIONS 10000
size_t ctu_mesh_adjacency_ws_bytes(int64_t V, int64_t F);
int ctu_mesh_adjacency_build(const int32_t* faces, int64_t V, int64_t F, int32_t* offsets, void* ws, void* stream);
int ctu_mesh_adjacency_emit(int64_t V, int64_t F, int64_t E, const int32_t* offsets, int32_t* neighbours, void* ws,
                            void* stream);
size_t ctu_mesh_smooth_ws_bytes(int64_t V);
int ctu_mesh_smooth(const float* vertices, int64_t V, const int32_t* offsets, const int32_t* neighbours, int64_t E,
                    const uint8_t* fixed, int iterations, float lambda, int has_mu, float mu, float* out, void* ws,
                    void* stream);

size_t ctu_mesh_voxelize_ws_bytes(int D, int H, int W);
int ctu_mesh_voxelize(const float* vertices, int64_t V, const int32_t* faces, int64_t F, int D, int H, int W,
                      const float* spacing, const float* origin, int want_winding, void* out, void* ws, void* stream);

#define CTU_MESH_GRID_MAX_CELLS 16777216
size_t ctu_mesh_grid_ws_bytes(int64_t F, int64_t max_cells);
int ctu_mesh_grid_build(const float* vertices, int64_t V, const int32_t* faces, int64_t F, float cell_size, int64_t max_cells,
                        float* corners, void* ws, void* stream);
int ctu_mesh_grid_emit(const float* corners, int64_t F, int64_t max_cells, int64_t cells, int64_t pairs, int32_t* offsets,
                       int32_t* items, void* ws, void* stream);
int ctu_mesh_distance(const float* corners, int64_t F, const int32_t* offsets, const int32_t* items, int64_t pairs,
                      const double* frame, int nz, int ny, int nx, const float* points, int64_t Q, int D, int H, int W,
                      const float* spacing, const float* origin, float max_distance, float far_value, float* dist,
                      int32_t* face, float* closest, void* stream);

#define CTU_MESH_DECIMATE_MAX_CELLS 268435456
#define CTU_MESH_DECIMATE_MAX_BUCKET 4096
size_t ctu_mesh_decimate_ws_bytes(int64_t V, int64_t F, int64_t cells);
int ctu_mesh_decimate_bounds(const float* vertices, int64_t V, const int32_t* faces, int64_t F, void* ws, void* stream);
int ctu_mesh_decimate_build(const float* vertices, int64_t V, const int32_t* faces, int64_t F, const float* lo, const float* hi,
                            const float* cell_size, int64_t cells, int cancel, void* ws, void* stream);
int ctu_mesh_decimate_emit(const int32_t* faces, int64_t V, int64_t F, int64_t Vp, int64_t Fp, const float* lo, const float* hi,
                           float* out_vertices, int32_t* out_faces, int32_t* out_map, void* ws, void* stream);

#define CTU_GAUSS_NEAREST 0
#define CTU_GAUSS_REFLECT 1
#define CTU_GAUSS_CONSTANT 2
#define CTU_GAUSS_MAX_RADIUS 32
#define CTU_HISTOGRAM_MAX_BINS 4096
size_t ctu_gaussian_ws_bytes(int64_t N, int D, int H, int W, int rz);
int ctu_gaussian_filter(const void* in, int dtype, int64_t N, int D, int H, int W, const int* radius, const float* weights,
                        int mode, float cval, float* out, void* ws, void* stream);
size_t ctu_minmax_ws_bytes(int64_t n);
int ctu_finite_minmax(const void* in, int dtype, int64_t n, double* range, void* ws, void* stream);
int ctu_histogram(const void* in, int dtype, int64_t n, int bins, const double* range, double lo, double hi, int64_t* hist,
                  void* stream);
int ctu_threshold_otsu(const int64_t* hist, int bins, const double* range, double lo, double hi, double* threshold,
                       int64_t* index, void* stream);
int ctu_binarize(const void* in, int dtype, int64_t n, const double* lower_dev, double lower, const double* upper_dev,
                 double upper, uint8_t* out, void* stream);

int ctu_extract_patches(const float* vol, const int32_t* coords, int P, int C, int D, int H, int W, int pd, int ph,
                        int pw, float* out, void* stream);
int ctu_stitch_patches(const float* patches, const int32_t* coords, int P, int C, int D, int H, int W, int pd, int ph,
                       int pw, float* out, void* stream);

int ctu_window_accumulate(const float* patches, const int32_t* coords, const int32_t* valid, const int32_t* box, int B,
                          int K, int D, int H, int W, int pd, int ph, int pw, const float* wz, const float* wy,
                          const float* wx, float wmin, int bz, int by, int bx, float* num, float* wsum, void* stream);
int ctu_window_finalize(const float* num, const float* wsum, int K, int64_t V, float* probs, uint8_t* labels,
                        void* stream);

#define CTU_FLAP_CHUNK 8192
#define CTU_FLAP_RECORD 16
#define CTU_FLAP_HOLE 1
#define CTU_FLAP_NOISE 2
#define CTU_FLAP_SPHERE 0
#define CTU_FLAP_BOX 1
#define CTU_FLAP_FLAP 2
int ctu_flap_count(const void* skull, int u8, int N, int64_t V, int32_t* counts, void* stream);
// ... 160 lines not shown
```

Before: 685.2 million voxels/s.

## Add split-parity upconv kernels and MFMA weight pack/project for small grids

```diff
diff --git a/ct-unet_amd/csrc/upconv_fused.hip b/ct-unet_amd/csrc/upconv_fused.hip
--- a/ct-unet_amd/csrc/upconv_fused.hip
+++ b/ct-unet_amd/csrc/upconv_fused.hip
@@ -21,14 +21,15 @@
     ctu_bn_tail tail;
 };
 
-template <int PB, int NTP, bool PW = false>
-__global__ __launch_bounds__(256, 2) void upconv_fused_fwd_kernel(UpP p, int ntiles, int tiles_per_block) {
-    static_assert(PW ? (PB == 4 && NTP == 1) : ((PB * NTP == 8 || (PB == 4 && NTP == 1)) && (PB == 8 || PB == 4 || PB == 2)), "tile-parities per block");
+template <int PB, int NTP, bool PW, bool SPLIT>
+__device__ __forceinline__ void upconv_fused_fwd_body(const UpP& p, int ntiles, int tiles_per_block) {
+    static_assert(SPLIT ? (PB == 1 && NTP == 1 && !PW) :
+                  PW ? (PB == 4 && NTP == 1) : ((PB * NTP == 8 || (PB == 4 && NTP == 1)) && (PB == 8 || PB == 4 || PB == 2)), "tile-parities per block");
     constexpr int NTW = PW ? 3 : 2, TAPS = 4 * NTW;
     constexpr int MT = 4, TD = 4, TH = 4, TW = 16;
     constexpr int HD = TD + 2, HH = TH + 2, HW = TW + 2, HV = HD * HH * HW;
     constexpr int NTHR = 256;
-    constexpr int NTPT = NTP;
+    const int ntpt = SPLIT ? (p.nout_p + 15) >> 4 : NTP;
     constexpr int WFL = PB * TAPS * NTP * 128;
     constexpr int AITEMS = HV * 2, AITER = (AITEMS + NTHR - 1) / NTHR;
     constexpr int WITER = (WFL / 4 + NTHR - 1) / NTHR;
@@ -43,12 +44,14 @@
     const int tid = threadIdx.x, lane = tid & 63, wave = tid >> 6;
     const int m = lane & 15, kq = lane >> 4;
     const int by = blockIdx.y;
+    const int par0 = SPLIT ? by / ntpt : by * PB, tile0 = SPLIT ? by % ntpt : 0;
     const int nchunk = p.rin_p >> 3;
     const int half = tid & 1;
     const bool has_xf = p.in_scale != nullptr;
-    const int pd0 = PW ? 0 : ((by * PB) >> 2) & 1, ph0 = PW ? 0 : ((by * PB) >> 1) & 1;
-
-    lds_v2f_ptr vA = (lds_v2f_ptr)sA2 + (((wave + pd0) * HH + ph0) * HW + m) * VS2 + kq;
+    const int pd0 = PW ? 0 : (par0 >> 2) & 1, ph0 = PW ? 0 : (par0 >> 1) & 1;
+    const int pw0 = SPLIT ? par0 & 1 : 0;
+
+    lds_v2f_ptr vA = (lds_v2f_ptr)sA2 + (((wave + pd0) * HH + ph0) * HW + pw0 + m) * VS2 + kq;
     lds_v2f_ptr vW = (lds_v2f_ptr)sW2 + (kq * 16 + m);
 
     unsigned hoff[AITER];
@@ -84,7 +87,7 @@
     const int tile_end = min(ntiles, tile + tiles_per_block);
     int c = 0;
     float4 va[AITER];
-    typedef typename std::conditional<PW, f32x4, float4>::type wv_t;
+    typedef typename std::conditional<PW || SPLIT, f32x4, float4>::type wv_t;
     wv_t vw[WITER];
     float4 sc = make_float4(1.f, 1.f, 1.f, 1.f), sh = make_float4(0.f, 0.f, 0.f, 0.f);
     unsigned vmask = 0;
@@ -149,7 +152,12 @@
     };
     auto load_w = [&](int cc) {
         const char* wsrc = reinterpret_cast<const char*>(PW ? p.wp + (size_t)cc * 4 * TAPS * 128
-                                                            : p.wp + ((size_t)cc * 8 + (size_t)by * PB) * 8 * NTPT * 128);
+                                                            : p.wp + (((size_t)cc * 8 + (size_t)par0) * 8 * ntpt + tile0) * 128);
+        if constexpr (SPLIT) {
+            static_assert(WITER == 1, "one float4 per thread");
+            vw[0] = *reinterpret_cast<const wv_t*>(wsrc + (unsigned)((tid >> 5) * ntpt * 128 + (tid & 31) * 4) * 4u);
+            return;
+        }
 #pragma unroll
         for (int it = 0; it < WITER; ++it) vw[it] = *reinterpret_cast<const wv_t*>(wsrc + (unsigned)(tid + it * NTHR) * 16u);
     };
@@ -242,14 +250,14 @@
             const bool touches = d0 == 0 || h0 == 0 || w0 == 0 || d0 + TD >= p.D || h0 + TH >= p.H || w0 + TW >= p.W;
 #pragma unroll
             for (int nt = 0; nt < NTP; ++nt) {
-                const int co = PW ? (kq & 1) * 4 : nt * 16 + kq * 4;
+                const int co = PW ? (kq & 1) * 4 : (tile0 + nt) * 16 + kq * 4;
                 const bool cok = co < p.nout_p;
                 float4 b0 = make_float4(0.f, 0.f, 0.f, 0.f);
                 if (cok) b0 = *reinterpret_cast<const float4*>(p.beff + co);
 #pragma unroll
                 for (int pi = 0; pi < PB; ++pi) {
                     const int pd = PW ? (pi >> 1) : pd0 + ((PB == 8) ? (pi >> 2) : 0), ph = PW ? (pi & 1) : ph0 + ((PB >= 4) ? ((pi >> 1) & 1) : 0),
-                              pw = PW ? (kq >> 1) : (pi & 1);
+                              pw = PW ? (kq >> 1) : pw0 + (pi & 1);
                     const int fz = 2 * cd + pd, fx = 2 * cw + pw;
 #pragma unroll
                     for (int mt = 0; mt < MT; ++mt) {
@@ -297,16 +305,28 @@
         float* row = p.stats + ((size_t)blockIdx.y * gridDim.x + blockIdx.x) * 2 * p.nout_p;
         for (int ch = tid; ch < p.nout_p; ch += NTHR) {
             float a1 = 0.f, a2 = 0.f;
-#pragma unroll
-            for (int w = 0; w < 4; ++w) {
-                a1 += sRed[(w * NTP * 16 + ch) * 2 + 0];
-                a2 += sRed[(w * NTP * 16 + ch) * 2 + 1];
+            const int lc = ch - tile0 * 16;
+            if (!SPLIT || (unsigned)lc < 16u) {
+#pragma unroll
+                for (int w = 0; w < 4; ++w) {
+                    a1 += sRed[(w * NTP * 16 + lc) * 2 + 0];
+                    a2 += sRed[(w * NTP * 16 + lc) * 2 + 1];
+                }
             }
             st_row(p.tail.counter != nullptr, row + ch, a1);
             st_row(p.tail.counter != nullptr, row + p.nout_p + ch, a2);
         }
         if (p.tail.counter) bn_fwd_tail(p.tail, p.stats, gridDim.x * gridDim.y, p.nout_p, gridDim.x * gridDim.y);
     }
+}
+
+template <int PB, int NTP, bool PW = false>
+__global__ __launch_bounds__(256, 2) void upconv_fused_fwd_kernel(UpP p, int ntiles, int tiles_per_block) {
+    upconv_fused_fwd_body<PB, NTP, PW, false>(p, ntiles, tiles_per_block);
+}
+
+__global__ __launch_bounds__(256, 2) void upconv_fused_fwd_split_kernel(UpP p, int ntiles, int tiles_per_block) {
+    upconv_fused_fwd_body<1, 1, false, true>(p, ntiles, tiles_per_block);
 }
 
 struct UpDP {
@@ -318,9 +338,11 @@
     int tiles_d, tiles_h, tiles_w, n16;
 };
 
-template <int NT>
-__global__ __launch_bounds__(256, 2) void upconv_fused_bwd_data_kernel(UpDP p, int ntiles, int tiles_per_block) {
-    constexpr int MT = 4, TD = 4, TH = 4, TW = 16;
+template <int NT, int TD>
+__device__ __forceinline__ void upconv_fused_bwd_data_body(const UpDP& p, int ntiles, int tiles_per_block) {
+    static_assert(TD == 4 || TD == 2, "planes per box");
+    constexpr int MT = TD == 4 ? 4 : 2, TH = 4, TW = 16;
+    constexpr int AR = MT + 1;
     constexpr int HD = TD + 2, HH = TH + 2, HW = TW + 2, HV = HD * HH * HW;
     constexpr int NTHR = 256;
     constexpr int WFL = 8 * NT * 128;
@@ -341,7 +363,8 @@
     const int half = tid & 1;
     const int Hf = 2 * p.H, Wf = 2 * p.W;
 
-    lds_v2f_ptr vA0 = (lds_v2f_ptr)sA2 + ((wave * HH) * HW + m) * VS2 + kq;
+    const int wd = wave % TD, wh = (wave / TD) * MT;
+    lds_v2f_ptr vA0 = (lds_v2f_ptr)sA2 + ((wd * HH + wh) * HW + m) * VS2 + kq;
     lds_v2f_ptr vW = (lds_v2f_ptr)sW2 + (kq * 16 + m);
 
     unsigned hoff[AITER];
@@ -480,11 +503,11 @@
         }
         CTU_SETPRIO(0);
         {
-            v2f ar[2][5], br[2][2][NT];
-            auto load_group = [&](int g, v2f (&aa)[5], v2f (&bb)[2][NT]) {
+            v2f ar[2][AR], br[2][2][NT];
+            auto load_group = [&](int g, v2f (&aa)[AR], v2f (&bb)[2][NT]) {
                 const int ez = (g >> 1) & 1, ex = g & 1;
 #pragma unroll
-                for (int r = 0; r < 5; ++r) aa[r] = vA[((ez * HH + r) * HW + ex) * VS2];
+                for (int r = 0; r < AR; ++r) aa[r] = vA[((ez * HH + r) * HW + ex) * VS2];
 #pragma unroll
                 for (int ey = 0; ey < 2; ++ey)
 #pragma unroll
@@ -497,7 +520,7 @@
 #pragma unroll
             for (int g = 0; g < 4; ++g) {
                 if (g + 1 < 4) load_group(g + 1, ar[(g + 1) & 1], br[(g + 1) & 1]);
-                v2f (&aa)[5] = ar[g & 1];
+                v2f (&aa)[AR] = ar[g & 1];
                 v2f (&bb)[2][NT] = br[g & 1];
 #pragma unroll
                 for (int ey = 0; ey < 2; ++ey) {
@@ -516,7 +539,7 @@
 #pragma unroll
                 for (int q = 0; q < 4 * MT * NT; ++q) {
                     __builtin_amdgcn_sched_group_barrier(0x008, 1, 0);
-                    if (g + 1 < 4 && q < 5 + 2 * NT) __builtin_amdgcn_sched_group_barrier(0x100, 1, 0);
+                    if (g + 1 < 4 && q < AR + 2 * NT) __builtin_amdgcn_sched_group_barrier(0x100, 1, 0);
                 }
 #endif
             }
@@ -525,14 +548,14 @@
         if (c == nchunk - 1) {
             const int d0 = box.tz * TD, h0 = box.ty * TH, w0 = box.tx * TW;
             const int gw = w0 + m;
-            float* obase = p.out + ((((size_t)box.n * p.D + d0 + wave) * p.H + h0) * p.W + gw) * p.out_cs;
+            float* obase = p.out + ((((size_t)box.n * p.D + d0 + wd) * p.H + h0 + wh) * p.W + gw) * p.out_cs;
             const int orow = p.W * p.out_cs;
 #pragma unroll
             for (int nt = 0; nt < NT; ++nt) {
                 const int co = (by * NT + nt) * 16 + kq * 4;
 #pragma unroll
                 for (int mt = 0; mt < MT; ++mt) {
-                    if (co < p.cin_p && d0 + wave < p.D && h0 + mt < p.H && gw < p.W) {
+                    if (co < p.cin_p && d0 + wd < p.D && h0 + wh + mt < p.H && gw < p.W) {
                         float4 o;
                         o.x = acc[mt][nt][0]; o.y = acc[mt][nt][1]; o.z = acc[mt][nt][2]; o.w = acc[mt][nt][3];
                         *reinterpret_cast<float4*>(obase + mt * orow + co) = o;
@@ -544,6 +567,16 @@
         if (!has_next) break;
         tile = ntile; c = nc; box = nbox;
     }
+}
+
+template <int NT>
+__global__ __launch_bounds__(256, 2) void upconv_fused_bwd_data_kernel(UpDP p, int ntiles, int tiles_per_block) {
+    upconv_fused_bwd_data_body<NT, 4>(p, ntiles, tiles_per_block);
+}
+
+template <int NT>
+__global__ __launch_bounds__(256, 2) void upconv_fused_bwd_data_split_kernel(UpDP p, int ntiles, int tiles_per_block) {
+    upconv_fused_bwd_data_body<NT, 2>(p, ntiles, tiles_per_block);
 }
 
 __device__ __forceinline__ float upconv_pack_bwd_value(const float* __restrict__ wp, int idx, int cin_p, int nout_p) {
@@ -705,6 +738,78 @@
     upconv_pack_block(wtt, w3t, wp, C, nout_p, cinv, nchunk, ntpt, (int)blockIdx.x - nbeff, part);
 }
 
+__device__ __forceinline__ f32x4 mfma4(float a, float b, f32x4 c) { return __builtin_amdgcn_mfma_f32_16x16x4f32(a, b, c, 0, 0, 0); }
+
+constexpr int WSM_BLOCK = 256;
+__global__ __launch_bounds__(WSM_BLOCK) void upconv_pack_beff_mfma_kernel(const float* __restrict__ wtt, const float* __restrict__ w3t,
+                                                                          float* __restrict__ wp, int C, int cin_p, int nout_p,
+                                                                          const int32_t* __restrict__ cinv, int ntpt,
+                                                                          const float* __restrict__ bt, float* __restrict__ beff) {
+    __shared__ float4 part[WSM_BLOCK / 64][64];
+    static_assert(27 * BEFF_CO <= (WSM_BLOCK / 64) * 64 * 4, "b_eff's S fits the tile's LDS");
+    const int nbeff = nout_p / BEFF_CO;
+    if ((int)blockIdx.x < nbeff) {
+        upconv_beff_block(bt, w3t, beff, C, nout_p, (int)blockIdx.x * BEFF_CO, reinterpret_cast<float*>(part));
+        return;
+    }
+    const int wave = threadIdx.x >> 6, lane = threadIdx.x & 63, m = lane & 15, kq = lane >> 4;
+    const int nrt = (cin_p + 15) >> 4;
+    int r = (int)blockIdx.x - nbeff;
+    const int ct = r % ntpt; r /= ntpt;
+    const int rt = r % nrt; r /= nrt;
+    const int tap = r & 7, par = r >> 3;
+    const int rp = rt * 16 + m;
+    const int ci = rp < cin_p ? (cinv ? cinv[rp] : (rp < C ? rp : -1)) : -1;
+    const int co = ct * 16 + m;
+    const bool aok = ci >= 0, bok = co < nout_p;
+    int tz[2], az[2], ty[2], ay[2], tx[2], ax[2];
+    const int nz = axis_pairs((par >> 2) & 1, (tap >> 2) & 1, tz, az);
+    const int ny = axis_pairs((par >> 1) & 1, (tap >> 1) & 1, ty, ay);
+    const int nx = axis_pairs(par & 1, tap & 1, tx, ax);
+    f32x4 acc = {0.f, 0.f, 0.f, 0.f};
+    for (int pi = wave; pi < nz * ny * nx; pi += WSM_BLOCK / 64) {
+        const int ix = pi % nx, iy = (pi / nx) % ny, iz = pi / (nx * ny);
+        const float* a = wtt + ((size_t)((az[iz] * 2 + ay[iy]) * 2 + ax[ix]) * C + (aok ? ci : 0)) * C;
+        const float* b = w3t + (size_t)((tz[iz] * 3 + ty[iy]) * 3 + tx[ix]) * C * nout_p + (bok ? co : 0);
+        for (int cm0 = 0; cm0 < C; cm0 += 64) {
+            float4 av[4];
+            float bv[4][4];
+#pragma unroll
+            for (int u = 0; u < 4; ++u) {
+                const int k = cm0 + u * 16 + kq * 4;
+                const int kc = k < C ? k : 0;
+                av[u] = *reinterpret_cast<const float4*>(a + kc);
+#pragma unroll
+                for (int j = 0; j < 4; ++j) bv[u][j] = b[(size_t)(kc + j) * nout_p];
+            }
+            __builtin_amdgcn_sched_barrier(0);
+#pragma unroll
+            for (int u = 0; u < 4; ++u) {
+                const bool kok = cm0 + u * 16 + kq * 4 < C;
+                const bool ka = kok && aok, kb = kok && bok;
+                acc = mfma4(ka ? av[u].x : 0.f, kb ? bv[u][0] : 0.f, acc); acc = mfma4(ka ? av[u].y : 0.f, kb ? bv[u][1] : 0.f, acc);
+                acc = mfma4(ka ? av[u].z : 0.f, kb ? bv[u][2] : 0.f, acc); acc = mfma4(ka ? av[u].w : 0.f, kb ? bv[u][3] : 0.f, acc);
+            }
+        }
+    }
+    part[wave][lane] = make_float4(acc[0], acc[1], acc[2], acc[3]);
+    __syncthreads();
+    if (wave != 0) return;
+    float4 sum = part[0][lane];
+#pragma unroll
+    for (int w = 1; w < WSM_BLOCK / 64; ++w) {
+        const float4 q = part[w][lane];
+        sum.x += q.x; sum.y += q.y; sum.z += q.z; sum.w += q.w;
+    }
+    const float sv[4] = {sum.x, sum.y, sum.z, sum.w};
+#pragma unroll
+    for (int j = 0; j < 4; ++j) {
+        const int row = rt * 16 + kq * 4 + j;
+        if (row < cin_p)
+            wp[((((size_t)(row >> 3) * 8 + par) * 8 + tap) * ntpt + ct) * 128 + ((row & 7) >> 1) * 32 + m * 2 + (row & 1)] = sv[j];
+    }
+}
+
 constexpr int FS_SPLIT = 16;
 
 template <class T>
@@ -878,6 +983,120 @@
     if (sub == 0) *dst = v;
 }
 
+__global__ __launch_bounds__(WSM_BLOCK) void upconv_project_mfma_kernel(const float* __restrict__ dweff, const float* __restrict__ V,
+                                                                        const float* __restrict__ wtt, const float* __restrict__ w3t,
+                                                                        const float* __restrict__ bt, const int32_t* __restrict__ imap,
+                                                                        int C, int Co, int cin_p, int nout_p, int nbt, int nb3,
+                                                                        float* __restrict__ dwt, float* __restrict__ dw3,
+                                                                        float* __restrict__ dbt) {
+    __shared__ float4 part[WSM_BLOCK / 64][64];
+    const int wave = threadIdx.x >> 6, lane = threadIdx.x & 63, m = lane & 15, kq = lane >> 4;
+    const int nct = (C + 15) >> 4;
+    int b = blockIdx.x;
+    if (b >= nbt + nb3) {
+        const int gidx = (b - nbt - nb3) * WSM_BLOCK + threadIdx.x, sub = gidx & 7, cm = gidx >> 3;
+        if (cm >= C) return;
+        float v = 0.f;
+        for (int t = sub; t < 27; t += 8) {
+            const float* w = w3t + ((size_t)t * C + cm) * nout_p;
+#pragma unroll 8
+            for (int co = 0; co < Co; ++co) v = fmaf(V[t * nout_p + co], w[co], v);
+        }
+        v += __shfl_xor(v, 1); v += __shfl_xor(v, 2); v += __shfl_xor(v, 4);
+        if (sub == 0) dbt[cm] = v;
+        return;
+    }
+    f32x4 acc = {0.f, 0.f, 0.f, 0.f};
+    const bool is3 = b >= nbt;
+    int a = 0, t = 0, rt, cmt;
+    if (!is3) {
+        a = b & 7; b >>= 3;
+        cmt = b % nct; rt = b / nct;
+        const int ci = rt * 16 + m, cm = cmt * 16 + m;
+        const bool aok = ci < C, bok = cm < C;
+        const int pos = aok ? (imap ? imap[ci] : ci) : 0;
+        for (int c0 = 0; c0 < nout_p; c0 += 32) {
+            float4 gv[7][2], wv[7][2];
+#pragma unroll
+            for (int i = 0; i < 7; ++i) {
+                const int tt = wave + i * (WSM_BLOCK / 64);
+                const int tc = tt < 27 ? tt : 0;
+                const float* g = dweff + ((size_t)weff_index(tc, a) * cin_p + pos) * nout_p;
+                const float* w = w3t + ((size_t)tc * C + (bok ? cm : 0)) * nout_p;
+#pragma unroll
+                for (int u = 0; u < 2; ++u) {
+                    const int co = c0 + u * 16 + kq * 4;
+                    const int cc = co < nout_p ? co : 0;
+                    gv[i][u] = *reinterpret_cast<const float4*>(g + cc);
+                    wv[i][u] = *reinterpret_cast<const float4*>(w + cc);
+                }
+            }
+            __builtin_amdgcn_sched_barrier(0);
+#pragma unroll
+            for (int i = 0; i < 7; ++i) {
+                const bool ok = wave + i * (WSM_BLOCK / 64) < 27 && aok && bok;
+#pragma unroll
+                for (int u = 0; u < 2; ++u) {
+                    const int co = c0 + u * 16 + kq * 4;
+                    const float4 g4 = gv[i][u], w4 = wv[i][u];
+                    acc = mfma4(ok && co < Co ? g4.x : 0.f, w4.x, acc); acc = mfma4(ok && co + 1 < Co ? g4.y : 0.f, w4.y, acc);
+                    acc = mfma4(ok && co + 2 < Co ? g4.z : 0.f, w4.z, acc); acc = mfma4(ok && co + 3 < Co ? g4.w : 0.f, w4.w, acc);
+                }
+            }
+        }
+    } else {
+        b -= nbt;
+        const int nrt = (Co + 15) >> 4;
+        rt = b % nrt; b /= nrt;
+        cmt = b % nct; t = b / nct;
+        const int co = rt * 16 + m, cm = cmt * 16 + m;
+        const bool aok = co < Co, bok = cm < C;
+        const float* g0 = dweff + (size_t)weff_index(t, wave * 2) * cin_p * nout_p + (aok ? co : 0);
+        const float* g1 = dweff + (size_t)weff_index(t, wave * 2 + 1) * cin_p * nout_p + (aok ? co : 0);
+        const float* w0 = wtt + (size_t)(wave * 2) * C * C + (bok ? cm : 0);
+        for (int ci0 = 0; ci0 < C; ci0 += 64) {
+            float gv[2][16], wv[2][16];
+#pragma unroll
+            for (int u = 0; u < 16; ++u) {
+                const int ci = ci0 + u * 4 + kq;
+                const int cc = ci < C ? ci : 0;
+                const size_t row = (size_t)(imap ? imap[cc] : cc) * nout_p;
+                gv[0][u] = g0[row]; gv[1][u] = g1[row];
+                wv[0][u] = w0[(size_t)cc * C]; wv[1][u] = w0[(size_t)(C + cc) * C];
+            }
+            __builtin_amdgcn_sched_barrier(0);
+#pragma unroll
+            for (int q = 0; q < 2; ++q)
+#pragma unroll
+                for (int u = 0; u < 16; ++u) {
+                    const bool kok = ci0 + u * 4 + kq < C;
+                    acc = mfma4(kok && aok ? gv[q][u] : 0.f, kok && bok ? wv[q][u] : 0.f, acc);
+                }
+        }
+    }
+    part[wave][lane] = make_float4(acc[0], acc[1], acc[2], acc[3]);
+    __syncthreads();
+    if (wave != 0) return;
+    float4 s = part[0][lane];
+#pragma unroll
+    for (int w = 1; w < WSM_BLOCK / 64; ++w) {
+        const float4 q = part[w][lane];
+        s.x += q.x; s.y += q.y; s.z += q.z; s.w += q.w;
+    }
+    const float sv[4] = {s.x, s.y, s.z, s.w};
+    const int cm = cmt * 16 + m;
+    if (cm >= C) return;
+#pragma unroll
+    for (int j = 0; j < 4; ++j) {
+        const int row = rt * 16 + kq * 4 + j;
+        if (!is3) {
+            if (row < C) dwt[((size_t)row * C + cm) * 8 + a] = sv[j];
+        } else if (row < Co) {
+            dw3[((size_t)row * C + cm) * 27 + t] = fmaf(V[t * nout_p + row], bt[cm], sv[j]);
+        }
+    }
+}
+
 struct UpPlan { int tiles_d, tiles_h, tiles_w, ntiles, nt, ny; Grid grid; };
 static UpPlan up_plan(int N, int D, int H, int W, int nout_p, int bwd_n16) {
     UpPlan r;
@@ -894,12 +1113,30 @@
     r.grid = persist_grid(r.ntiles, 512 / r.ny);
     return r;
 }
+static UpPlan up_split_bwd_plan(int N, int D, int H, int W, int bwd_n16) {
+    UpPlan r;
+    r.tiles_d = ceil_div(D, 2); r.tiles_h = ceil_div(H, 4); r.tiles_w = ceil_div(W, 16);
+    r.ntiles = N * r.tiles_d * r.tiles_h * r.tiles_w;
+    r.nt = bwd_n16 >= 4 ? 4 : (bwd_n16 >= 2 ? 2 : 1);
+    while (r.nt > 1 && (long)r.ntiles * ceil_div(bwd_n16, r.nt) < 256) r.nt >>= 1;
+    r.ny = ceil_div(bwd_n16, r.nt);
+    r.grid = persist_grid(r.ntiles, 512 / r.ny);
+    return r;
+}
+static UpPlan up_split_plan(int N, int D, int H, int W, int nout_p) {
+    UpPlan r = up_plan(N, D, H, W, nout_p, 0);
+    r.ny = 8 * ceil_div(nout_p, 16);
+    r.grid = persist_grid(r.ntiles, 512 / r.ny);
+    return r;
+}
 
 }
 
 extern "C" int ctu_upconv_fused_supported(int k, int D, int H, int W, int cin_p, int nout_p) {
     return k == 3 && W >= 16 && D >= 1 && H >= 1 && cin_p % 8 == 0 && cin_p >= 8 && nout_p % 8 == 0 && nout_p >= 8 && nout_p <= 64;
 }
+
+static bool up_ws_mfma(int C, int cin_p) { return cin_p > 64 && C % 4 == 0; }
 
 static size_t up_std_packed(int cin_p, int nout_p) { return (size_t)(cin_p / 8) * 8 * 8 * ceil_div(nout_p, 16) * 128; }
 
@@ -936,9 +1173,15 @@
     const int ntr = 27 * C * nout_p + 8 * C * C;
     upconv_transpose_kernel<<<ceil_div(ntr, 256), 256, 0, st>>>(wt, w3, wtt, w3t, C, Co, nout_p);
     CTU_CHECK_LAUNCH("upconv_fused_transpose");
-    const int quads = (cin_p / 8) * 8 * 8 * 8 * ntpt * 4;
-    upconv_pack_beff_kernel<<<nout_p / BEFF_CO + ceil_div(quads, 8), WS_BLOCK, 0, st>>>(wtt, w3t, wp, C, nout_p, cinv, cin_p / 8,
-                                                                                         ntpt, bt, beff);
+    if (up_ws_mfma(C, cin_p)) {
+        const int tiles = 64 * ceil_div(cin_p, 16) * ntpt;
+        upconv_pack_beff_mfma_kernel<<<nout_p / BEFF_CO + tiles, WSM_BLOCK, 0, st>>>(
+            wtt, w3t, wp, C, cin_p, nout_p, cinv, ntpt, bt, beff);
+    } else {
+        const int quads = (cin_p / 8) * 8 * 8 * 8 * ntpt * 4;
+        upconv_pack_beff_kernel<<<nout_p / BEFF_CO + ceil_div(quads, 8), WS_BLOCK, 0, st>>>(wtt, w3t, wp, C, nout_p, cinv, cin_p / 8,
+                                                                                             ntpt, bt, beff);
+    }
     CTU_CHECK_LAUNCH("upconv_fused_pack");
     return upconv_pack_gather(wp, cin_p, nout_p, nout_p == 8 ? wp + up_std_packed(cin_p, nout_p) : nullptr, wpd, st);
 }
@@ -948,9 +1191,9 @@
     return ctu_upconv_fused_pack_all(wt, bt, w3, C, Co, cinv, cin_p, nout_p, wp, beff, ws, nullptr, stream);
 }
 
-extern "C" int ctu_upconv_fused_fwd(const float* in, int in_cs, int cin_p, const float* in_scale, const float* in_shift,
-                                    int in_relu, const float* wp, const float* beff, float* out, int out_cs, int nout_p,
-                                    float* stats, int N, int D, int H, int W, const ctu_bn_tail* tail, void* stream) {
+static int upconv_fwd_impl(bool split, const float* in, int in_cs, int cin_p, const float* in_scale, const float* in_shift,
+                           int in_relu, const float* wp, const float* beff, float* out, int out_cs, int nout_p,
+                           float* stats, int N, int D, int H, int W, const ctu_bn_tail* tail, void* stream) {
     CTU_REQUIRE(in && wp && beff && out, "upconv_fused_fwd: null pointer");
     CTU_REQUIRE(ctu_upconv_fused_supported(3, D, H, W, cin_p, nout_p), "upconv_fused_fwd: unsupported geometry (W=%d cin_p=%d nout_p=%d)",
                 W, cin_p, nout_p);
@@ -968,11 +1211,13 @@
     p.tail = tail_or_off(tail);
     p.in_cs = in_cs; p.rin_p = cin_p; p.in_relu = in_relu; p.out_cs = out_cs; p.nout_p = nout_p;
     p.N = N; p.D = D; p.H = H; p.W = W;
-    const UpPlan r = up_plan(N, D, H, W, nout_p, 0);
+    const UpPlan r = split ? up_split_plan(N, D, H, W, nout_p) : up_plan(N, D, H, W, nout_p, 0);
     p.tiles_d = r.tiles_d; p.tiles_h = r.tiles_h; p.tiles_w = r.tiles_w;
     const int ny = r.ny, gx = r.grid.gx, tpb = r.grid.tpb, ntiles = r.ntiles;
     hipStream_t st = (hipStream_t)stream;
-    if (nout_p == 16 && ny == 2) {
+    if (split) {
+        upconv_fused_fwd_split_kernel<<<dim3(gx, ny), 256, 0, st>>>(p, ntiles, tpb);
+    } else if (nout_p == 16 && ny == 2) {
         upconv_fused_fwd_kernel<4, 1><<<dim3(gx, 2), 256, 0, st>>>(p, ntiles, tpb);
     } else if (nout_p == 8) {
         p.wp = wp + up_std_packed(cin_p, nout_p);
@@ -982,6 +1227,25 @@
     else upconv_fused_fwd_kernel<2, 4><<<dim3(gx, 4), 256, 0, st>>>(p, ntiles, tpb);
     CTU_CHECK_LAUNCH("upconv_fused_fwd");
     return CTU_OK;
+}
+
+extern "C" int ctu_upconv_fused_fwd(const float* in, int in_cs, int cin_p, const float* in_scale, const float* in_shift,
+                                    int in_relu, const float* wp, const float* beff, float* out, int out_cs, int nout_p,
+                                    float* stats, int N, int D, int H, int W, const ctu_bn_tail* tail, void* stream) {
+    return upconv_fwd_impl(false, in, in_cs, cin_p, in_scale, in_shift, in_relu, wp, beff, out, out_cs, nout_p, stats, N, D, H, W,
+                           tail, stream);
+}
+
+extern "C" int ctu_upconv_fused_split_num_blocks(int N, int D, int H, int W, int nout_p) {
+    const UpPlan r = up_split_plan(N, D, H, W, nout_p);
+    return r.grid.gx * r.ny;
+}
+
+extern "C" int ctu_upconv_fused_fwd_split(const float* in, int in_cs, int cin_p, const float* in_scale, const float* in_shift,
+                                          int in_relu, const float* wp, const float* beff, float* out, int out_cs, int nout_p,
+                                          float* stats, int N, int D, int H, int W, void* stream) {
+    return upconv_fwd_impl(true, in, in_cs, cin_p, in_scale, in_shift, in_relu, wp, beff, out, out_cs, nout_p, stats, N, D, H, W,
+                           nullptr, stream);
 }
 
 extern "C" int ctu_channel_sum_num_blocks(int64_t nvox);
@@ -1015,6 +1279,13 @@
     CTU_CHECK_LAUNCH("upconv_tall_v");
     const float* w3t = pack_ws;
     const float* wtt = pack_ws + (size_t)27 * C * nout_p;
+    if (up_ws_mfma(C, cin_p)) {
+        const int nct = ceil_div(C, 16), nbt = 8 * nct * nct, nb3 = 27 * nct * ceil_div(Co, 16);
+        upconv_project_mfma_kernel<<<nbt + nb3 + ceil_div(C * 8, WSM_BLOCK), WSM_BLOCK, 0, st>>>(
+            dweff, V, wtt, w3t, bt, imap, C, Co, cin_p, nout_p, nbt, nb3, dwt, dw3, dbt);
+        CTU_CHECK_LAUNCH("upconv_project");
+        return CTU_OK;
+    }
     const int nb1 = ceil_div((C * C * 8 + C) * 8, WS_BLOCK);
     const int nb2 = ceil_div(((Co + 3) / 4) * C * 27, 8);
     upconv_project_kernel<<<nb1 + nb2, WS_BLOCK, 0, st>>>(dweff, V, wtt, w3t, bt, imap, C, Co, cin_p, nout_p, nb1, dwt, dw3, dbt);
@@ -1043,8 +1314,8 @@
     return upconv_pack_gather(wp, cin_p, nout_p, nullptr, wpd, (hipStream_t)stream);
 }
 
-extern "C" int ctu_upconv_fused_bwd_data(const float* gout, int g_cs, int nout_p, const float* wpd, float* gin, int gin_cs,
-                                         int cin_p, int N, int D, int H, int W, void* stream) {
+static int upconv_bwd_data_impl(bool split, const float* gout, int g_cs, int nout_p, const float* wpd, float* gin, int gin_cs,
+                                int cin_p, int N, int D, int H, int W, void* stream) {
     CTU_REQUIRE(gout && wpd && gin, "upconv_fused_bwd_data: null pointer");
     CTU_REQUIRE(ctu_upconv_fused_supported(3, D, H, W, cin_p, nout_p), "upconv_fused_bwd_data: unsupported geometry");
     CTU_REQUIRE(g_cs >= nout_p && g_cs % 4 == 0 && gin_cs >= cin_p && gin_cs % 4 == 0, "upconv_fused_bwd_data: bad stride");
@@ -1054,13 +1325,27 @@
     p.g = gout; p.wp = wpd; p.out = gin; p.g_cs = g_cs; p.nout_p = nout_p; p.out_cs = gin_cs; p.cin_p = cin_p;
     p.N = N; p.D = D; p.H = H; p.W = W;
     p.n16 = ceil_div(cin_p, 16);
-    const UpPlan r = up_plan(N, D, H, W, nout_p, p.n16);
+    const UpPlan r = split ? up_split_bwd_plan(N, D, H, W, p.n16) : up_plan(N, D, H, W, nout_p, p.n16);
     p.tiles_d = r.tiles_d; p.tiles_h = r.tiles_h; p.tiles_w = r.tiles_w;
     const int NT = r.nt, ny = r.ny, gx = r.grid.gx, tpb = r.grid.tpb, ntiles = r.ntiles;
     hipStream_t st = (hipStream_t)stream;
-    if (NT == 4) upconv_fused_bwd_data_kernel<4><<<dim3(gx, ny), 256, 0, st>>>(p, ntiles, tpb);
+    if (split) {
+        if (NT == 4) upconv_fused_bwd_data_split_kernel<4><<<dim3(gx, ny), 256, 0, st>>>(p, ntiles, tpb);
+        else if (NT == 2) upconv_fused_bwd_data_split_kernel<2><<<dim3(gx, ny), 256, 0, st>>>(p, ntiles, tpb);
+        else upconv_fused_bwd_data_split_kernel<1><<<dim3(gx, ny), 256, 0, st>>>(p, ntiles, tpb);
+    } else if (NT == 4) upconv_fused_bwd_data_kernel<4><<<dim3(gx, ny), 256, 0, st>>>(p, ntiles, tpb);
     else if (NT == 2) upconv_fused_bwd_data_kernel<2><<<dim3(gx, ny), 256, 0, st>>>(p, ntiles, tpb);
     else upconv_fused_bwd_data_kernel<1><<<dim3(gx, ny), 256, 0, st>>>(p, ntiles, tpb);
     CTU_CHECK_LAUNCH("upconv_fused_bwd_data");
     return CTU_OK;
 }
+
+extern "C" int ctu_upconv_fused_bwd_data(const float* gout, int g_cs, int nout_p, const float* wpd, float* gin, int gin_cs,
+                                         int cin_p, int N, int D, int H, int W, void* stream) {
+    return upconv_bwd_data_impl(false, gout, g_cs, nout_p, wpd, gin, gin_cs, cin_p, N, D, H, W, stream);
+}
+
+extern "C" int ctu_upconv_fused_bwd_data_split(const float* gout, int g_cs, int nout_p, const float* wpd, float* gin, int gin_cs,
+                                               int cin_p, int N, int D, int H, int W, void* stream) {
+    return upconv_bwd_data_impl(true, gout, g_cs, nout_p, wpd, gin, gin_cs, cin_p, N, D, H, W, stream);
+}
diff --git a/ct-unet_amd/ctunet_amd/_lib.py b/ct-unet_amd/ctunet_amd/_lib.py
--- a/ct-unet_amd/ctunet_amd/_lib.py
+++ b/ct-unet_amd/ctunet_amd/_lib.py
@@ -110,6 +110,8 @@
     "ctu_upconv_fused_pack": (I, [P, P, P, I, I, P, I, I, P, P, P, P]),
     "ctu_upconv_fused_pack_all": (I, [P, P, P, I, I, P, I, I, P, P, P, P, P]),
     "ctu_upconv_fused_fwd": (I, [P, I, I, P, P, I, P, P, P, I, I, P, I, I, I, I, P, P]),
+    "ctu_upconv_fused_split_num_blocks": (I, [I, I, I, I, I]),
+    "ctu_upconv_fused_fwd_split": (I, [P, I, I, P, P, I, P, P, P, I, I, P, I, I, I, I, P]),
     "ctu_upconv_fused_wgrad_ws_floats": (Z, [I, I, I, I, I, I]),
     "ctu_upconv_fused_wgrad": (I, [P, I, I, P, P, I, P, I, I, P, P, I, I, I, I, P]),
     "ctu_upconv_fused_wgrad_bn_supported": (I, [I, I, I, I, I, I]),
@@ -119,6 +121,7 @@
     "ctu_upconv_fused_bwd_packed_floats": (Z, [I, I]),
     "ctu_upconv_fused_pack_bwd": (I, [P, I, I, P, P]),
     "ctu_upconv_fused_bwd_data": (I, [P, I, I, P, P, I, I, I, I, I, I, P]),
+    "ctu_upconv_fused_bwd_data_split": (I, [P, I, I, P, P, I, I, I, I, I, I, P]),
     "ctu_hard_segm": (I, [P, I, I, L, P, P]),
     "ctu_one_hot": (I, [P, I, I, L, P, P]),
     "ctu_hard_dice_ws_doubles": (Z, [I]),
diff --git a/ct-unet_amd/ctunet_amd/engine.py b/ct-unet_amd/ctunet_amd/engine.py
--- a/ct-unet_amd/ctunet_amd/engine.py
+++ b/ct-unet_amd/ctunet_amd/engine.py
@@ -12,6 +12,7 @@
 BN_EPS = 1e-5
 FUSE_UP = os.environ.get("CTUNET_FUSE_UP", "1") != "0"
 FUSE_UP_MAX_CO = int(os.environ.get("CTUNET_FUSE_UP_MAXCO", "16"))
+FUSE_UP_SPLIT_BELOW = 256
 POOL_BN = os.environ.get("CTUNET_POOL_BN", "1") != "0"
 LP_FUSE_UP = os.environ.get("CTUNET_LP_FUSE_UP", "1") != "0"
 BN_MOMENTUM = 0.1
@@ -221,6 +222,10 @@
             return ops.upconv_fused_supported(x.dims, 3, x.cp, nout_p)
         return LP_FUSE_UP and ops.lp_upconv_fused_supported(x.dims, 3, x.cp, nout_p)
 
+    def _fuse_up_split(self, x: CL, nout_p: int) -> bool:
+        return (self.dtype == torch.float32 and nout_p > 16
+                and ops.upconv_fused_num_blocks(x.dims, nout_p) < FUSE_UP_SPLIT_BELOW)
+
     def _upconv_bn(self, P, x: CL, prefix: str, ct: int, cout: int, cinv, out: CL, vec4: torch.Tensor, training: bool,
                    n_upd: int, save: bool) -> Tuple[CL, Optional[_ConvRec]]:
         conv, bn = f"{prefix}.1", f"{prefix}.2"
@@ -239,13 +244,15 @@
             self._up_cache[prefix] = (ver, wp, beff, (x.cp, out.cp, self.dtype), pws, wpd)
         else:
             wp, beff, wpd = hit[1], hit[2], hit[5]
+        split = False
         if lp:
             nblk = ops.lp_upconv_fused_num_blocks(x.dims) if training else 0
             launch = lambda stats, tail: ops.lp_upconv_fused_fwd(x, wpd, beff, out, stats, (ct, cout))
         else:
-            nblk = ops.upconv_fused_num_blocks(x.dims, out.cp) if training else 0
-            launch = lambda stats, tail: ops.upconv_fused_fwd(x, wp, beff, out, stats, (ct, cout), tail)
-        y, stats = self._bn_stage(P, bn, out, vec4, 8 * x.nvox, cout, training, n_upd, nblk, launch, tail_ok=not lp)
+            split = self._fuse_up_split(x, out.cp)
+            nblk = (ops.upconv_fused_split_num_blocks if split else ops.upconv_fused_num_blocks)(x.dims, out.cp) if training else 0
+            launch = lambda stats, tail: ops.upconv_fused_fwd(x, wp, beff, out, stats, (ct, cout), tail, split)
+        y, stats = self._bn_stage(P, bn, out, vec4, 8 * x.nvox, cout, training, n_upd, nblk, launch, tail_ok=not (lp or split))
         rec = _ConvRec(None, out.raw(), vec4, stats, nblk, conv, bn, ct, cout, None, False) if save else None
         return y, rec
 
@@ -558,7 +565,8 @@
                 if g_u1.lp:
                     ops.lp_upconv_fused_bwd_data(gq, self._up_cache[blk.prefix][5], gin, (ct, blk.cout))
                 else:
-                    ops.upconv_fused_bwd_data(gq, self._up_cache[blk.prefix][5], gin, (ct, blk.cout))
+                    ops.upconv_fused_bwd_data(gq, self._up_cache[blk.prefix][5], gin, (ct, blk.cout),
+                                              self._fuse_up_split(x_in, gq.cp))
             else:
                 g_up = CL(torch.empty_like(up.buf), 0, up.cp)
                 self._conv_bn_bwd(P, r1, g_u1, g_up, grads, ws, part)
diff --git a/ct-unet_amd/ctunet_amd/ops.py b/ct-unet_amd/ctunet_amd/ops.py
--- a/ct-unet_amd/ctunet_amd/ops.py
+++ b/ct-unet_amd/ctunet_amd/ops.py
@@ -869,17 +869,27 @@
     return _lib.load().ctu_upconv_fused_num_blocks(n, d, h, w, nout_p)
 
 
+def upconv_fused_split_num_blocks(dims, nout_p: int) -> int:
+    n, d, h, w = dims
+    return _lib.load().ctu_upconv_fused_split_num_blocks(n, d, h, w, nout_p)
+
+
 def upconv_fused_fwd(x: CL, wp: torch.Tensor, beff: torch.Tensor, out: CL, stats: Optional[torch.Tensor],
-                     algo_ch: Optional[Tuple[int, int]] = None, tail=None) -> None:
+                     algo_ch: Optional[Tuple[int, int]] = None, tail=None, split: bool = False) -> None:
     n, d, h, w = x.dims
     assert out.dims == (n, 2 * d, 2 * h, 2 * w)
     ci, co = algo_ch if algo_ch is not None else (x.cp, out.cp)
     vox = n * d * h * w
-    with _timed(lambda: (f"upconv_fused_fwd_kernel<{out.cp}>", vox * (16.0 * ci * ci + 8 * 54.0 * ci * co),
+    assert not (split and tail is not None)
+    name = "upconv_fused_fwd_split_kernel" if split else "upconv_fused_fwd_kernel"
+    with _timed(lambda: (f"{name}<{out.cp}>", vox * (16.0 * ci * ci + 8 * 54.0 * ci * co),
                          4.0 * vox * (ci + 8 * co), (w, x.cp, out.cp))):
-        _lib.check(_lib.load().ctu_upconv_fused_fwd(x.ptr, x.cs, x.cp, _ptr(x.scale), _ptr(x.shift), int(x.relu),
-                                                    wp.data_ptr(), beff.data_ptr(), out.ptr, out.cs, out.cp, _ptr(stats),
-                                                    n, d, h, w, _tail_arg(tail), _stream()), "upconv_fused_fwd")
+        args = (x.ptr, x.cs, x.cp, _ptr(x.scale), _ptr(x.shift), int(x.relu), wp.data_ptr(), beff.data_ptr(), out.ptr, out.cs,
+                out.cp, _ptr(stats), n, d, h, w)
+        if split:
+            _lib.check(_lib.load().ctu_upconv_fused_fwd_split(*args, _stream()), "upconv_fused_fwd_split")
+        else:
+            _lib.check(_lib.load().ctu_upconv_fused_fwd(*args, _tail_arg(tail), _stream()), "upconv_fused_fwd")
 
 
 def upconv_fused_wgrad_bn_supported(dims, cin_p: int, nout_p: int, dtype=torch.float32) -> bool:
@@ -988,15 +998,17 @@
     return wpd
 
 
-def upconv_fused_bwd_data(g: CL, wpd: torch.Tensor, gin: CL, algo_ch: Optional[Tuple[int, int]] = None) -> None:
+def upconv_fused_bwd_data(g: CL, wpd: torch.Tensor, gin: CL, algo_ch: Optional[Tuple[int, int]] = None,
+                          split: bool = False) -> None:
     n, d, h, w = gin.dims
     assert g.dims == (n, 2 * d, 2 * h, 2 * w)
     ci, co = algo_ch if algo_ch is not None else (gin.cp, g.cp)
     vox = n * d * h * w
-    with _timed(lambda: (f"upconv_fused_bwd_data_kernel<{g.cp}>", vox * (16.0 * ci * ci + 8 * 54.0 * ci * co),
+    name = "upconv_fused_bwd_data_split_kernel" if split else "upconv_fused_bwd_data_kernel"
+    entry = _lib.load().ctu_upconv_fused_bwd_data_split if split else _lib.load().ctu_upconv_fused_bwd_data
+    with _timed(lambda: (f"{name}<{g.cp}>", vox * (16.0 * ci * ci + 8 * 54.0 * ci * co),
                          4.0 * vox * (ci + 8 * co), (w, gin.cp, g.cp))):
-        _lib.check(_lib.load().ctu_upconv_fused_bwd_data(g.ptr, g.cs, g.cp, wpd.data_ptr(), gin.ptr, gin.cs, gin.cp,
-                                                         n, d, h, w, _stream()), "upconv_fused_bwd_data")
+        _lib.check(entry(g.ptr, g.cs, g.cp, wpd.data_ptr(), gin.ptr, gin.cs, gin.cp, n, d, h, w, _stream()), name[:-7])
 
 
 def _ncv(t: torch.Tensor):
diff --git a/include/ctunet_hip.h b/include/ctunet_hip.h
--- a/include/ctunet_hip.h
+++ b/include/ctunet_hip.h
@@ -224,6 +224,10 @@
 int ctu_upconv_fused_fwd(const float* in, int in_cs, int cin_p, const float* in_scale, const float* in_shift,
                          int in_relu, const float* wp, const float* beff, float* out, int out_cs, int nout_p,
                          float* stats, int N, int D, int H, int W, const ctu_bn_tail* tail, void* stream);
+int ctu_upconv_fused_split_num_blocks(int N, int D, int H, int W, int nout_p);
+int ctu_upconv_fused_fwd_split(const float* in, int in_cs, int cin_p, const float* in_scale, const float* in_shift,
+                               int in_relu, const float* wp, const float* beff, float* out, int out_cs, int nout_p,
+                               float* stats, int N, int D, int H, int W, void* stream);
 
 size_t ctu_upconv_fused_wgrad_ws_floats(int N, int D, int H, int W, int cin_p, int nout_p);
 int ctu_upconv_fused_wgrad(const float* in, int in_cs, int cin_p, const float* in_scale, const float* in_shift,
@@ -243,6 +247,8 @@
 int ctu_upconv_fused_pack_bwd(const float* wp, int cin_p, int nout_p, float* wpd, void* stream);
 int ctu_upconv_fused_bwd_data(const float* gout, int g_cs, int nout_p, const float* wpd, float* gin, int gin_cs,
                               int cin_p, int N, int D, int H, int W, void* stream);
+int ctu_upconv_fused_bwd_data_split(const float* gout, int g_cs, int nout_p, const float* wpd, float* gin, int gin_cs,
+                                    int cin_p, int N, int D, int H, int W, void* stream);
 
 int ctu_hard_segm(const float* prob, int N, int C, int64_t nvox_per_item, float* seg, void* stream);
 int ctu_one_hot(const float* label, int N, int C, int64_t nvox_per_item, float* out, void* stream);
```

New measurement: 684.4 million voxels/s. No clear change (-0.1%).
